# jasperlinthorst/reveal

Hardware: AMD Instinct MI355X
Metric: Mbp/s indexed+MUM-anchored (reveal rem) (higher is better)
Workload: dtype int32

## Files before the change

### include/reveal_amd.h

```cpp
#ifndef REVEAL_AMD_H
#define REVEAL_AMD_H
#include <stdint.h>

#ifdef __cplusplus
extern "C" {
#endif

typedef struct rv_index rv_index;

const char *rv_last_error(void);
int  rv_abi_version(void);
int  rv_sa_bits(void);
int  rv_device_count(void);

rv_index *rv_new(int device);
void rv_free(rv_index *h);

int rv_add_sample(rv_index *h);
int rv_add_sequence(rv_index *h, const char *seq, int64_t len, int64_t *begin, int64_t *end);
int rv_reset(rv_index *h);
int rv_reserve_text(rv_index *h, int64_t bytes);
int64_t rv_n(const rv_index *h);
int rv_nsamples(const rv_index *h);
int rv_nnodes(const rv_index *h);
// ... 42 lines not shown
    int64_t steps;
    int64_t splits;
    int64_t anchored_bp;
    int32_t levels;
    int32_t maxdepth;
    int64_t scanned_ranks;
    double  t_scan, t_host, t_split, t_bubble;
} rv_align_stats;
int rv_align_builtin(rv_index *h, int minl, int minn, rv_align_stats *st);

int rv_align_builtin_until(rv_index *h, int minl, int minn, int stop_subs, rv_align_stats *st);
int rv_align_builtin_resume(rv_index *h, rv_align_stats *st);
int rv_align_builtin_continue(rv_index *h, int stop_subs, rv_align_stats *st);
int rv_frontier_counts(rv_index *h, int64_t *out);
int rv_frontier_export(rv_index *h, int64_t *meta, int64_t *node_first, int64_t *nodes);
int64_t rv_frontier_pack(rv_index *h, const int32_t *subs, int k, void *sa, void *lcp, void *bwt, int on_device);
int rv_frontier_import(rv_index *h, int minl, int minn, uint32_t maxlcp, int level, int nsubs, const int64_t *meta,
                       const int64_t *node_first, const int64_t *nodes, int64_t m,
                       const void *sa, const void *lcp, const void *bwt, int on_device);
int64_t rv_frontier_seeds_export(rv_index *h, const int32_t *subs, int k, int64_t *out, int64_t cap);
int rv_frontier_seeds_import(rv_index *h, int nsubs, const int64_t *words, int64_t nwords);
uint32_t rv_maxlcp(const rv_index *h);
int rv_cascade_info(const rv_index *h, int64_t *out);
int rv_capacity_events(const rv_index *h, int64_t *out);
const char *rv_cascade_why(const rv_index *h);
int64_t rv_anchor_count(rv_index *h, int64_t *members);
int rv_fetch_anchors(rv_index *h, uint32_t *l, int64_t *off, int64_t *pos);
int rv_set_result_buffers(rv_index *h, uint32_t *l, int64_t l_cap, int64_t *off, int64_t off_cap, int64_t *pos, int64_t pos_cap);
typedef struct {
    int64_t  key, n;
    int32_t  depth, nsamples, nnodes, picked;
    int64_t  nmums;
    uint32_t l; int32_t mn;
    int64_t  sp_min;
    uint64_t h_sa, h_lcp, h_mums;
} rv_trace;
int rv_set_trace(rv_index *h, int on);
int rv_set_preselect(rv_index *h, int64_t maxmums);
int rv_set_option(rv_index *h, const char *name, int64_t value);
int rv_get_option(rv_index *h, const char *name, int64_t *value);
int rv_set_launch_trace(int on);
int rv_option_count(void);
const char *rv_option_name(int k);
int64_t rv_trace_count(rv_index *h);
int rv_fetch_trace(rv_index *h, rv_trace *out, int64_t cap);

typedef struct rv_subindex rv_subindex;
rv_index *rv_clone(rv_index *h);
rv_subindex *rv_sx_main(rv_index *h);
rv_subindex *rv_sx_copy(rv_subindex *x);
void rv_sx_free(rv_subindex *x);
int rv_sx_info(const rv_subindex *x, rv_sub *out);
int rv_sx_nodes(const rv_subindex *x, int64_t *begin_end);
int64_t rv_sx_array(rv_subindex *x, int which, void *out, int64_t cap);
int64_t rv_sx_scan(rv_subindex *x, int minl, int minn, int64_t *members);
int rv_sx_fetch(rv_subindex *x, uint32_t *l, int32_t *n, int64_t *off, uint16_t *so, int64_t *pos);
int rv_sx_split(rv_subindex *x, const int64_t *lead, int nlead, const int64_t *trail, int ntrail,
                const int64_t *match, int nmatch, const int64_t *rest, int nrest, rv_subindex **out);
int rv_sx_extract(rv_subindex *x, int64_t *intervals, int niv);

int64_t rv_chain(int64_t m, int k, const uint32_t *len, const int32_t *nmem, const int64_t *crd, const int64_t *left,
                 const int64_t *right, int64_t wscore, int64_t wpen, int model, int64_t *out_idx, int64_t *out_score);

typedef struct { int64_t wscore, wpen, maxmums, seedsize; int gcmodel; int trim; double pcutoff; } rv_picker_args;
typedef struct {
    int picked; uint32_t pick_l; int32_t pick_n; int pick_members; uint16_t *pick_so; int64_t *pick_pos; int64_t member_cap;
    int64_t nleft, nright, nseed_members, seed_cap, seed_member_cap;
    uint32_t *seed_l; int32_t *seed_n; int64_t *seed_off; uint16_t *seed_so; int64_t *seed_pos; int64_t *seed_score; uint8_t *seed_right;
} rv_picker_out;
int rv_set_picker(rv_index *h, int kind, const rv_picker_args *args);
int rv_picker_info(const rv_index *h, int64_t *out);
int rv_pick_chain(const rv_picker_args *args, int nsub, int64_t m, const uint32_t *l, const int32_t *n, const int64_t *off, const uint16_t *so,
                  const int64_t *pos, int nsamples, const int64_t *seq_begin, const int64_t *iv_begin, const int64_t *iv_end, int minlength,
                  rv_picker_out *out);

typedef struct rv_graph rv_graph;
rv_graph *rv_graph_import(int64_t nnodes, const int64_t *node_b, const int64_t *node_e, const int8_t *node_aligned, const int8_t *node_sent,
                          const int64_t *off_ptr, const int32_t *off_sid, const int64_t *off_val,
                          int64_t nedges, const int32_t *edge_u, const int32_t *edge_v, const int64_t *edge_ptr, const int32_t *edge_paths,
                          const int64_t *pred_ptr, const int32_t *pred_edge, int npaths, const uint8_t *star, const int64_t *id2end,
                          int nstart, const int32_t *start_nodes, int literal_segments);
int rv_graph_pick(rv_graph *g, const rv_picker_args *args, int nsub, int64_t m, const uint32_t *l, const int32_t *n, const int64_t *off, const uint16_t *so, const int64_t *pos,
                  const int64_t *left, const int64_t *right, int minlength, rv_picker_out *out);
int rv_graph_align(rv_graph *g, const int64_t *nodes, int64_t nn, const int64_t *left, const int64_t *right, uint32_t l, const int64_t *pos, int npos,
                   int64_t *counts, int64_t *out6);
int rv_graph_align_fetch(rv_graph *g, int64_t *out);
int rv_set_graph_picker(rv_index *h, rv_graph *g, const rv_picker_args *args);
rv_graph *rv_graph_new(void);
int rv_graph_add_linear(rv_graph *g, int64_t b, int64_t e, int star);
int64_t rv_graph_read_gfa(rv_graph *g, rv_index *h, int64_t *text_n, const char *data, int64_t len, const char **names);
typedef struct GfaParsed rv_gfa_parsed;
rv_gfa_parsed *rv_gfa_parse(const char *data, int64_t len);
int64_t rv_graph_adopt(rv_graph *g, rv_index *h, int64_t *text_n, rv_gfa_parsed *parsed, const char **names);
void rv_gfa_parsed_free(rv_gfa_parsed *parsed);
int rv_graph_seal(rv_graph *g);
int rv_graph_paths(const rv_graph *g, int64_t *id2end);
int rv_graph_node_kinds(const rv_graph *g, int8_t *out);
int rv_graph_literal(const rv_graph *g);
int rv_graph_finish(rv_graph *g);
rv_graph *rv_graph_replay_begin(int nseq, const int64_t *begin, const int64_t *end);
int rv_set_replay_graph(rv_index *h, rv_graph *g);
rv_graph *rv_graph_replay(int nseq, const int64_t *begin, const int64_t *end, int64_t na, const uint32_t *an_l, const int64_t *an_off, const int64_t *an_pos);
const char *rv_graph_error(const rv_graph *g);
int rv_graph_sizes(const rv_graph *g, int64_t *out);
int rv_graph_export(const rv_graph *g, int64_t *node_b, int64_t *node_e, int8_t *node_aligned, int64_t *off_ptr, int32_t *off_sid, int64_t *off_val,
                    int64_t *succ_ptr, int32_t *succ_to, int32_t *succ_edge, int64_t *pred_ptr, int32_t *pred_from, int32_t *pred_edge, int64_t *edge_ptr, int32_t *edge_paths);
int rv_graph_prune(rv_graph *g, const char *T);
int64_t rv_graph_gfa(rv_graph *g, const char *T, int npaths, const char *const *names, const char *cmdline, const char **out);
void rv_graph_free(rv_graph *g);

enum { RV_K_SCAN_PAIR = 0, RV_K_SCAN_MULTI = 1, RV_K_SA_SORT = 2, RV_K_LCP = 3, RV_K_SPLIT = 4, RV_K_LABEL = 5,
       RV_K_BUBBLE = 6,
       RV_K_RADIX_SCATTER = 7, RV_K_RADIX_HIST = 8, RV_K_TEXT_ROUND = 9,
       RV_K_CASCADE = 10,
       RV_K_DIAG_TABLE = 11,
       RV_K_INIT_KEYS = 12,
       RV_K_PUBLISH = 13,
       RV_K_COUNT = 14 };
int rv_prof_enable(rv_index *h, int on);
int rv_prof_reset(rv_index *h);
int rv_prof_get(rv_index *h, int k, int64_t *launches, double *ms, double *bytes);
typedef struct rv_batch rv_batch;
rv_batch *rv_batch_new(void);
int rv_batch_add(rv_batch *b, rv_index *h);
int rv_batch_run(rv_batch *b, int minl, int minn, int construct, rv_align_stats *stats, int *status);
int rv_batch_info(const rv_batch *b, int64_t *out);
void rv_batch_free(rv_batch *b);
typedef struct rv_many rv_many;
rv_many *rv_many_new(int device);
void rv_many_free(rv_many *m);
int rv_many_option(rv_many *m, const char *name, int64_t value);
int64_t rv_many_add(rv_many *m, const char *const *seqs, const int64_t *lens, int k);
int rv_many_clear(rv_many *m);
int rv_many_run(rv_many *m, int minl, int minn, rv_align_stats *total);
int64_t rv_many_anchor_count(rv_many *m, int64_t *first, int64_t *members);
int rv_many_fetch(rv_many *m, uint32_t *l, int64_t *off, int64_t *pos);
int64_t rv_many_text(rv_many *m, int64_t job, char *out, int64_t cap);
int rv_many_info(const rv_many *m, int64_t *out);
int64_t rv_many_arrays(rv_many *m, int64_t job, int which, void *out, int64_t cap);
void *rv_dev_alloc(int device, int64_t bytes);
int rv_dev_free(int device, void *p);
int rv_ipc_export(int device, const void *p, uint8_t handle[64]);
void *rv_ipc_open(int device, const uint8_t handle[64]);
int rv_ipc_close(int device, void *p);
int rv_dev_copy(int device, void *dst, const void *src, int64_t bytes);
int rv_measure_bandwidth(int device, int64_t bytes, int iters, double *read_gbs, double *copy_gbs);
int rv_sa_stats(rv_index *h, int *sigma, int *bits, int *k0, int *rounds, int64_t *sorted_elems, int *radix_passes);
int rv_sa_diag_table(rv_index *h);
int rv_sa_tail(rv_index *h, int64_t *out);

int rv_test_exclusive_sum_u32(const uint32_t *in, uint32_t *out, int64_t n);
int rv_test_inclusive_max_u32(const uint32_t *in, uint32_t *out, int64_t n);
int rv_test_radix_sort(uint64_t *keys, uint32_t *vals, int64_t n, int bit_lo, int bit_hi);
int rv_test_radix_time(int64_t n, int bits, int dist, int flags, int iters, double *ms, int64_t *bad);

#ifdef __cplusplus
}
#endif
#endif
```

### reveal_amd/_index.py

```python
import ctypes
import mmap
import os
import sys
import numpy as np

from . import _lib
from ._lib import RV_T, RV_SA, RV_SAI, RV_LCP, RV_SO, RV_NSEP


def _page_array(count, dtype):
    nbytes = max(int(count), 1) * np.dtype(dtype).itemsize
    m = mmap.mmap(-1, (nbytes + mmap.PAGESIZE - 1) // mmap.PAGESIZE * mmap.PAGESIZE)
    return np.frombuffer(m, dtype=dtype, count=max(int(count), 1))


def _pairs(iv, sa64):
    a = np.ascontiguousarray(np.array([(int(b), int(e)) for b, e in iv], dtype=np.int64).reshape(-1, 2))
    return a, len(a)


_OPTION_DEFAULTS = {}


def make_index_type(sa64, error):

    class index(object):

        def __init__(self, sa="", lcp="", cache=0):
            self._lib = _lib.get(sa64)
            self._dll = self._lib.dll
            self._h = None
            self._safile, self._lcpfile, self._cache = sa or "", lcp or "", int(cache)
            self._samples, self._nodes, self.skipmums = [], set(), []
            self._leftnode = self._rightnode = None
            self._depth = 0
            self._constructed = False
            self._main = self
            self._slot = None
            self._sx = None
            self._n_sub = None
            self._nsamples_sub = None
            self._h = self._dll.rv_new(_lib.device())
            if not self._h:
                raise error(self._lib.err())
            self.options_from_env()

        def set_option(self, name, value=1):
            if self._dll.rv_set_option(self._main._h, name.encode(), int(value)) != 0:
                self._fail()

        def get_option(self, name):
            v = ctypes.c_int64(0)
            if self._dll.rv_get_option(self._main._h, name.encode(), ctypes.byref(v)) != 0:
                self._fail()
            return v.value

        def options_from_env(self):
            for k in range(self._dll.rv_option_count()):
                name = self._dll.rv_option_name(k).decode()
                v = os.environ.get(name)
                if v is None:
                    d = _OPTION_DEFAULTS.get((sa64, name))
                    if d is None:
                        d = _OPTION_DEFAULTS[(sa64, name)] = self.get_option(name)
                    elif self.get_option(name) != d:
                        self.set_option(name, d)
                    continue
                try:
                    iv = int(v) if v.strip() else 1
                except ValueError:
                    iv = 1
                _OPTION_DEFAULTS.setdefault((sa64, name), self.get_option(name))
                self.set_option(name, iv)

        @property
        def _main(self):
            m = self.__dict__.get("_main_ref")
            return self if m is None else m

        @_main.setter
        def _main(self, v):
            self.__dict__["_main_ref"] = None if v is self else v

        def __del__(self):
            try:
                if getattr(self, "_sx", None):
                    self._dll.rv_sx_free(self._sx)
                    self._sx = None
                if self._h and self._main is self:
                    self._dll.rv_free(self._h)
                    self._h = None
            except Exception:
                pass

        def _fail(self, exc=None):
            raise (exc or error)(self._lib.err())

        def addsample(self, *args):
            if len(args) < 1:
                raise error("Specify name of sample as argument.")
            if not isinstance(args[0], str):
                raise error("Sample name has to be a string.")
            self._samples.append(args[0])
            self._dll.rv_add_sample(self._h)
            self._constructed = False
            return None

        def addsequence(self, seq):
            if isinstance(seq, str):
                seq = seq.encode()
            elif not isinstance(seq, (bytes, bytearray)):
                raise TypeError("argument 1 must be str or bytes")
            b, e = ctypes.c_int64(0), ctypes.c_int64(0)
            if self._dll.rv_add_sequence(self._h, bytes(seq), len(seq), ctypes.byref(b), ctypes.byref(e)) != 0:
                self._fail()
            intv = (b.value, e.value)
            self._nodes.add(intv)
            self._constructed = False
            return intv

        def reset(self, reserve=0):
            if self._main is not self or self._slot is not None:
                raise error("reset() is for a main index outside align()")
            if self._sx:
                self._dll.rv_sx_free(self._sx)
                self._sx = None
            if self._dll.rv_reset(self._h) != 0:
                self._fail()
            if reserve and self._dll.rv_reserve_text(self._h, int(reserve)) != 0:
                self._fail()
            self._samples, self._nodes, self.skipmums = [], set(), []
            self._leftnode = self._rightnode = None
            self._depth = 0
            self._constructed = False
            self._pending = False
            self._n_sub = self._nsamples_sub = None

        def upload(self):
            if self._dll.rv_upload(self._h) != 0:
                self._fail()

        def upload_again(self):
            if self._dll.rv_upload_again(self._h) != 0:
                self._fail()

        def prof(self, enable=None, reset=False, only=None):
            ids = {"scan_pair": _lib.K_SCAN_PAIR, "scan_multi": _lib.K_SCAN_MULTI, "sa_build": _lib.K_SA_SORT, "lcp": _lib.K_LCP,
                   "split": _lib.K_SPLIT, "label": _lib.K_LABEL, "bubble": _lib.K_BUBBLE, "radix_scatter": _lib.K_RADIX_SCATTER,
                   "radix_hist": _lib.K_RADIX_HIST, "text_round": _lib.K_TEXT_ROUND, "cascade": _lib.K_CASCADE, "diag_table": _lib.K_DIAG_TABLE,
                   "init_keys": _lib.K_INIT_KEYS, "publish": _lib.K_PUBLISH}
            if enable is not None:
                on = 0
                if enable:
                    on = 1 if only is None else sum(2 << ids[k] for k in only)
                self._dll.rv_prof_enable(self._h, on)
            if reset:
                self._dll.rv_prof_reset(self._h)
            out = {}
            for name, k in ids.items():
                n, ms, by = ctypes.c_int64(0), ctypes.c_double(0), ctypes.c_double(0)
                self._dll.rv_prof_get(self._h, k, ctypes.byref(n), ctypes.byref(ms), ctypes.byref(by))
                out[name] = (n.value, ms.value, by.value)
            return out

        def sa_stats(self):
            v = [ctypes.c_int(0) for _ in range(4)]
            se, rp = ctypes.c_int64(0), ctypes.c_int(0)
            self._dll.rv_sa_stats(self._h, *[ctypes.byref(x) for x in v], ctypes.byref(se), ctypes.byref(rp))
            tail = (ctypes.c_int64 * 2)()
            self._dll.rv_sa_tail(self._h, tail)
            return dict(sigma=v[0].value, bits=v[1].value, k0=v[2].value, rounds=v[3].value, sorted_elems=se.value, radix_passes=rp.value,
                        diag_table=int(self._dll.rv_sa_diag_table(self._h)), far_pairs=int(tail[0]), lcp_list=int(tail[1]))

        def construct(self, rc=0):
            if self._sx:
                self._dll.rv_sx_free(self._sx)
                self._sx = None
            r = self._dll.rv_construct(self._h, int(rc), self._safile.encode(), self._lcpfile.encode(), self._cache)
            if r != 0:
                self._fail()
            self._constructed = True
            self._rc = 1 if int(rc) == 1 else 0
            self._depth = 0
            self._main = self
            return None

        def _sx_info(self):
            info = _lib.RvSub()
            self._dll.rv_sx_info(self._sx, ctypes.byref(info))
            return info

        @property
        def n(self):
            if self._sx:
                return self._sx_info().n
            return self._n_sub if self._n_sub is not None else self._dll.rv_n(self._h)

        @property
        def depth(self):
            return self._depth

        @property
        def nsamples(self):
            if self._sx and self._depth > 0:
                return self._sx_info().nsamples
            return self._nsamples_sub if self._nsamples_sub is not None else self._dll.rv_nsamples(self._h)

        @property
        def samples(self):
            return self._main._samples

        @property
        def nodes(self):
            if self.__dict__.get("_nodes_stale"):
                self._sync_nodes()
            return self._nodes

        @property
        def leftnode(self):
            return self._leftnode

        @property
        def rightnode(self):
            return self._rightnode

        @property
        def nsep(self):
            ns = self._dll.rv_nsamples(self._h)
            out = np.zeros(max(ns - 1, 1), dtype=np.int64)
            k = self._dll.rv_get_array(self._h, RV_NSEP, out.ctypes.data, len(out))
            return [int(x) for x in out[:max(k, 0)]]

        def _array(self, which, dtype, count, exc=TypeError):
            out = np.zeros(max(count, 1), dtype=dtype)
            if self._sx and which in (RV_SA, RV_LCP):
                k = self._dll.rv_sx_array(self._sx, which, out.ctypes.data, len(out))
            elif self._slot is not None and which in (RV_SA, RV_LCP):
                k = self._dll.rv_sub_array(self._h, self._slot, which, out.ctypes.data, len(out))
            else:
                k = self._dll.rv_get_array(self._h, which, out.ctypes.data, len(out))
            if k < 0:
                raise exc(self._lib.err())
            return out[:k]

        def _main_n(self):
            return self._dll.rv_n(self._h)

        @property
        def SA(self):
            return self._array(RV_SA, self._lib.sa_t, self.n).tolist()

        @property
        def LCP(self):
            return self._array(RV_LCP, self._lib.lcp_t, self.n).tolist()

        @property
        def SAi(self):
            return self._array(RV_SAI, self._lib.sa_t, self._main_n()).tolist()

        @property
        def SO(self):
            return self._array(RV_SO, np.uint16, self._main_n()).tolist()

        @property
        def T(self):
            return self._array(RV_T, np.uint8, self._main_n(), exc=error).tobytes().decode("latin-1")

        def array(self, name):
            which = {"SA": RV_SA, "LCP": RV_LCP, "SAi": RV_SAI, "SO": RV_SO, "T": RV_T}[name]
            dt = {RV_SA: self._lib.sa_t, RV_LCP: self._lib.lcp_t, RV_SAI: self._lib.sa_t, RV_SO: np.uint16, RV_T: np.uint8}[which]
            return self._array(which, dt, self.n if which in (RV_SA, RV_LCP) else self._main_n())

        def _sx_mums(self, minl, minn):
            mem = ctypes.c_int64(0)
            cnt = self._dll.rv_sx_scan(self._sx, int(minl), int(minn), ctypes.byref(mem))
            if cnt < 0:
                self._fail()
            l = np.zeros(max(cnt, 1), dtype=np.uint32); n = np.zeros(max(cnt, 1), dtype=np.int32)
            off = np.zeros(cnt + 1, dtype=np.int64)
            so = np.zeros(max(mem.value, 1), dtype=np.uint16); pos = np.zeros(max(mem.value, 1), dtype=np.int64)
            if self._dll.rv_sx_fetch(self._sx, l.ctypes.data, n.ctypes.data, off.ctypes.data, so.ctypes.data, pos.ctypes.data) != 0:
                self._fail()
            return _csr_to_tuples(cnt, l, n, off, so, pos)

        def getmums(self, minl=0):
            if self._sx:
                if self._dll.rv_nsamples(self._h) != 2:
                    raise error("getmums on a sub-index needs a two-sample main index")
                rc = 1 if getattr(self._main, "_rc", 0) else 0
                out = [(l, (spd[0][1], spd[1][1]), rc) for l, _, spd in self._sx_mums(minl, 0)]
                if rc:
                    nsep0, nT = self.nsep[0], self._main_n()
                    out = [(l, (a, nsep0 + (nT - b - l)), rc) for l, (a, b), _ in out]
                return out
            cnt = self._dll.rv_getmums(self._h, int(minl))
            if cnt < 0:
                self._fail(TypeError if cnt == -2 else error)
            l = np.zeros(max(cnt, 1), dtype=np.uint32)
            a = np.zeros(max(cnt, 1), dtype=np.int64)
            b = np.zeros(max(cnt, 1), dtype=np.int64)
            if self._dll.rv_fetch_mums(self._h, l.ctypes.data, a.ctypes.data, b.ctypes.data, len(l)) != 0:
                self._fail()
            rc = 1 if getattr(self, "_rc", 0) else 0
            return [(int(l[k]), (int(a[k]), int(b[k])), rc) for k in range(cnt)]

        def _multi(self, minlength, minn, mems):
            if self._sx:
                if mems or self._dll.rv_nsamples(self._h) <= 2:
                    raise error("only getmultimums of an index with more than two samples is available on a sub-index")
                return self._sx_mums(minlength, minn)
            members = ctypes.c_int64(0)
            cnt = self._dll.rv_getmultimums(self._h, int(minlength), int(minn), mems, ctypes.byref(members))
            if cnt < 0:
                self._fail(TypeError if cnt == -2 else error)
            l = np.zeros(max(cnt, 1), dtype=np.uint32); n = np.zeros(max(cnt, 1), dtype=np.int32)
            off = np.zeros(cnt + 1, dtype=np.int64)
            so = np.zeros(max(members.value, 1), dtype=np.uint16); pos = np.zeros(max(members.value, 1), dtype=np.int64)
            if self._dll.rv_fetch_multi(self._h, l.ctypes.data, n.ctypes.data, off.ctypes.data, so.ctypes.data, pos.ctypes.data) != 0:
                self._fail()
            return _csr_to_tuples(cnt, l, n, off, so, pos)

        def getmultimums(self, minlength=0, minn=2):
            return self._multi(minlength, minn, 0)

        def getmultimems(self, minlength=0, minn=2):
# ... 404 lines not shown
```

### reveal_amd/_lib.py

```python
import ctypes
import importlib.util
import os
import sys
import numpy as np

_HERE = os.path.dirname(os.path.abspath(__file__))

RV_T, RV_SA, RV_SAI, RV_LCP, RV_SO, RV_NSEP, RV_NODES = range(7)
K_SCAN_PAIR, K_SCAN_MULTI, K_SA_SORT, K_LCP, K_SPLIT, K_LABEL, K_BUBBLE, K_RADIX_SCATTER, K_RADIX_HIST, K_TEXT_ROUND, K_CASCADE, K_DIAG_TABLE, K_INIT_KEYS, K_PUBLISH = range(14)

CAPACITY_EVENTS = ("pair_ovf", "pair_out", "pair_pick_ovf", "pair_second_copy", "multi_rec", "multi_mem", "multi_cand",
                   "mems_rec", "mems_mem", "mems_long")
CAP_SITES = {"multi_cand": 1, "cas_wit": 2, "cas_tables": 4, "casm_matches": 8, "casm_wit": 16, "casm_tables": 32,
             "mems_rec": 64, "mems_mem": 128, "mems_long": 256}

c_i64p = ctypes.POINTER(ctypes.c_int64)
V = ctypes.c_void_p


class RvSub(ctypes.Structure):
    _fields_ = [("n", ctypes.c_int64), ("depth", ctypes.c_int32), ("nsamples", ctypes.c_int32),
                ("nnodes", ctypes.c_int32), ("parent", ctypes.c_int32), ("kind", ctypes.c_int32),
                ("reserved", ctypes.c_int32), ("nmums", ctypes.c_int64), ("nmembers", ctypes.c_int64)]


class RvAlignStats(ctypes.Structure):
    _fields_ = [("steps", ctypes.c_int64), ("splits", ctypes.c_int64), ("anchored_bp", ctypes.c_int64),
                ("levels", ctypes.c_int32), ("maxdepth", ctypes.c_int32), ("scanned_ranks", ctypes.c_int64),
                ("t_scan", ctypes.c_double), ("t_host", ctypes.c_double), ("t_split", ctypes.c_double),
                ("t_bubble", ctypes.c_double)]


TRACE_DTYPE = np.dtype([("key", np.int64), ("n", np.int64), ("depth", np.int32), ("nsamples", np.int32),
                        ("nnodes", np.int32), ("picked", np.int32), ("nmums", np.int64), ("l", np.uint32),
                        ("mn", np.int32), ("sp_min", np.int64), ("h_sa", np.uint64), ("h_lcp", np.uint64),
                        ("h_mums", np.uint64)], align=True)

_I, _L, _D = ctypes.c_int, ctypes.c_int64, ctypes.c_double
SYMBOLS = {
    "rv_last_error": (ctypes.c_char_p, []),
    "rv_abi_version": (_I, []),
    "rv_sa_bits": (_I, []),
    "rv_device_count": (_I, []),
    "rv_new": (V, [_I]),
    "rv_free": (None, [V]),
    "rv_add_sample": (_I, [V]),
    "rv_add_sequence": (_I, [V, ctypes.c_char_p, _L, c_i64p, c_i64p]),
    "rv_reset": (_I, [V]),
    "rv_reserve_text": (_I, [V, _L]),
    "rv_n": (_L, [V]),
    "rv_nsamples": (_I, [V]),
    "rv_nnodes": (_I, [V]),
    "rv_node_list": (_I, [V, V]),
    "rv_construct": (_I, [V, _I, ctypes.c_char_p, ctypes.c_char_p, _I]),
    "rv_upload": (_I, [V]),
    "rv_upload_again": (_I, [V]),
    "rv_get_array": (_L, [V, _I, V, _L]),
    "rv_getmums": (_L, [V, _I]),
    "rv_fetch_mums": (_I, [V, V, V, V, _L]),
    "rv_getmultimums": (_L, [V, _I, _I, _I, c_i64p]),
    "rv_fetch_multi": (_I, [V, V, V, V, V, V]),
    "rv_align_begin": (_I, [V, _I, _I]),
    "rv_frontier_size": (_I, [V]),
    "rv_frontier_scan": (_I, [V]),
    "rv_sub_skip_scan": (_I, [V, _I]),
    "rv_sub_info": (_I, [V, _I, ctypes.POINTER(RvSub)]),
    "rv_sub_nodes": (_I, [V, _I, V]),
    "rv_sub_mums": (_I, [V, _I, V, V, V, V, V]),
    "rv_sub_array": (_L, [V, _I, _I, V, _L]),
    "rv_sub_split": (_I, [V, _I, ctypes.c_uint32, _I, V, V, _I, V, _I, V, _I, V, _I]),
    "rv_frontier_commit": (_I, [V, V]),
    "rv_align_end": (_I, [V]),
    "rv_align_builtin": (_I, [V, _I, _I, ctypes.POINTER(RvAlignStats)]),
    "rv_align_builtin_until": (_I, [V, _I, _I, _I, ctypes.POINTER(RvAlignStats)]),
    "rv_align_builtin_resume": (_I, [V, ctypes.POINTER(RvAlignStats)]),
    "rv_align_builtin_continue": (_I, [V, _I, ctypes.POINTER(RvAlignStats)]),
    "rv_frontier_counts": (_I, [V, V]),
    "rv_frontier_export": (_I, [V, V, V, V]),
    "rv_frontier_pack": (_L, [V, V, _I, V, V, V, _I]),
    "rv_frontier_import": (_I, [V, _I, _I, ctypes.c_uint32, _I, _I, V, V, V, _L, V, V, V, _I]),
    "rv_frontier_seeds_export": (_L, [V, V, _I, V, _L]),
    "rv_frontier_seeds_import": (_I, [V, _I, V, _L]),
    "rv_maxlcp": (ctypes.c_uint32, [V]),
    "rv_cascade_info": (ctypes.c_int, [V, V]),
    "rv_cascade_why": (ctypes.c_char_p, [V]),
    "rv_capacity_events": (_I, [V, V]),
    "rv_anchor_count": (_L, [V, c_i64p]),
    "rv_fetch_anchors": (_I, [V, V, V, V]),
    "rv_set_result_buffers": (_I, [V, V, _L, V, _L, V, _L]),
    "rv_set_trace": (_I, [V, _I]),
    "rv_set_preselect": (_I, [V, _L]),
    "rv_set_option": (_I, [V, ctypes.c_char_p, _L]),
    "rv_set_launch_trace": (_I, [_I]),
    "rv_batch_new": (V, []),
    "rv_batch_add": (_I, [V, V]),
    "rv_batch_run": (_I, [V, _I, _I, _I, V, V]),
    "rv_batch_info": (_I, [V, V]),
    "rv_batch_free": (None, [V]),
    "rv_dev_alloc": (V, [_I, _L]),
    "rv_dev_free": (_I, [_I, V]),
    "rv_ipc_export": (_I, [_I, V, V]),
    "rv_ipc_open": (V, [_I, V]),
    "rv_ipc_close": (_I, [_I, V]),
    "rv_dev_copy": (_I, [_I, V, V, _L]),
    "rv_get_option": (_I, [V, ctypes.c_char_p, c_i64p]),
    "rv_option_count": (_I, []),
    "rv_option_name": (ctypes.c_char_p, [_I]),
    "rv_trace_count": (_L, [V]),
    "rv_fetch_trace": (_I, [V, V, _L]),
    "rv_clone": (V, [V]),
    "rv_sx_main": (V, [V]),
    "rv_sx_copy": (V, [V]),
    "rv_sx_free": (None, [V]),
    "rv_sx_info": (_I, [V, ctypes.POINTER(RvSub)]),
    "rv_sx_nodes": (_I, [V, V]),
    "rv_sx_array": (_L, [V, _I, V, _L]),
    "rv_sx_scan": (_L, [V, _I, _I, c_i64p]),
    "rv_sx_fetch": (_I, [V, V, V, V, V, V]),
    "rv_sx_split": (_I, [V, V, _I, V, _I, V, _I, V, _I, V]),
    "rv_sx_extract": (_I, [V, V, _I]),
    "rv_chain": (_L, [_L, _I, V, V, V, V, V, _L, _L, _I, V, V]),
    "rv_prof_enable": (_I, [V, _I]),
    "rv_prof_reset": (_I, [V]),
    "rv_prof_get": (_I, [V, _I, c_i64p, ctypes.POINTER(_D), ctypes.POINTER(_D)]),
    "rv_measure_bandwidth": (_I, [_I, _L, _I, ctypes.POINTER(_D), ctypes.POINTER(_D)]),
    "rv_sa_stats": (_I, [V] + [ctypes.POINTER(_I)] * 4 + [c_i64p, ctypes.POINTER(_I)]),
    "rv_sa_diag_table": (_I, [V]),
    "rv_sa_tail": (_I, [V, c_i64p]),
    "rv_set_picker": (_I, [V, _I, V]),
    "rv_picker_info": (_I, [V, c_i64p]),
    "rv_pick_chain": (_I, [V, _I, _L, V, V, V, V, V, _I, V, V, V, _I, V]),
    "rv_graph_import": (V, [_L, V, V, V, V, V, V, V, _L, V, V, V, V, V, V, _I, V, V, _I, V, _I]),
    "rv_graph_pick": (_I, [V, V, _I, _L, V, V, V, V, V, V, V, _I, V]),
    "rv_graph_align": (_I, [V, V, _L, V, V, ctypes.c_uint32, V, _I, V, V]),
    "rv_graph_align_fetch": (_I, [V, V]),
    "rv_graph_finish": (_I, [V]),
    "rv_set_graph_picker": (_I, [V, V, V]),
    "rv_graph_new": (V, []),
    "rv_graph_replay_begin": (V, [_I, V, V]),
    "rv_set_replay_graph": (_I, [V, V]),
    "rv_graph_add_linear": (_I, [V, _L, _L, _I]),
    "rv_graph_read_gfa": (_L, [V, V, V, V, _L, V]),
    "rv_graph_paths": (_I, [V, V]),
    "rv_graph_seal": (_I, [V]),
    "rv_gfa_parse": (V, [V, _L]),
    "rv_graph_adopt": (_L, [V, V, V, V, V]),
    "rv_gfa_parsed_free": (None, [V]),
    "rv_add_sequences": (_I, [V, V, _L, V, _L]),
    "rv_graph_node_kinds": (_I, [V, V]),
    "rv_graph_literal": (_I, [V]),
    "rv_graph_replay": (V, [_I, V, V, _L, V, V, V]),
    "rv_graph_error": (ctypes.c_char_p, [V]),
    "rv_graph_sizes": (_I, [V, c_i64p]),
    "rv_graph_export": (_I, [V] * 15),
    "rv_graph_prune": (_I, [V, V]),
    "rv_graph_gfa": (_L, [V, V, _I, V, V, V]),
    "rv_graph_free": (None, [V]),
    "rv_many_new": (V, [_I]),
    "rv_many_free": (None, [V]),
    "rv_many_option": (_I, [V, ctypes.c_char_p, _L]),
    "rv_many_add": (_L, [V, V, V, _I]),
    "rv_many_clear": (_I, [V]),
    "rv_many_run": (_I, [V, _I, _I, ctypes.POINTER(RvAlignStats)]),
    "rv_many_anchor_count": (_L, [V, V, c_i64p]),
    "rv_many_fetch": (_I, [V, V, V, V]),
    "rv_many_text": (_L, [V, _L, V, _L]),
    "rv_many_info": (_I, [V, V]),
    "rv_many_arrays": (_L, [V, _L, _I, V, _L]),
    "rv_test_exclusive_sum_u32": (_I, [V, V, _L]),
    "rv_test_inclusive_max_u32": (_I, [V, V, _L]),
    "rv_test_radix_sort": (_I, [V, V, _L, _I, _I]),
    "rv_test_radix_time": (_I, [_L, _I, _I, _I, _I, ctypes.POINTER(_D), c_i64p]),
}


def _share_torch_runtime():
    if os.environ.get("RV_SYSTEM_HIP") or "torch" in sys.modules:
        return
    try:
        spec = importlib.util.find_spec("torch")
    except (ImportError, ValueError):
        spec = None
    if spec is None or not spec.origin:
        return
    path = os.path.join(os.path.dirname(spec.origin), "lib", "libamdhip64.so")
    if os.path.exists(path):
        ctypes.CDLL(path, mode=ctypes.RTLD_GLOBAL)


class Lib:
    def __init__(self, sa64=False):
        self.sa64 = sa64
        _share_torch_runtime()
        name = "libreveal_amd64.so" if sa64 else "libreveal_amd.so"
        self.path = os.path.join(os.environ.get("RV_LIB_DIR") or _HERE, name)
        if not os.path.exists(self.path):
            raise ImportError("%s is missing: build it with `python -c 'import __graft_entry__ as g; g.build()'` "
                              "(hipcc --offload-arch=gfx950); reveal_amd has no CPU fallback" % self.path)
        self.dll = ctypes.CDLL(self.path)
        for sym, (res, args) in SYMBOLS.items():
            fn = getattr(self.dll, sym)
            fn.restype, fn.argtypes = res, args
        self.sa_t = np.int64 if sa64 else np.int32
        self.lcp_t = np.uint32 if sa64 else np.int32
        assert self.dll.rv_sa_bits() == (64 if sa64 else 32)
        v = os.environ.get("RV_LAUNCH_TRACE")
        if v is not None and v.strip() not in ("", "0"):
            self.dll.rv_set_launch_trace(1)

    def err(self):
        return (self.dll.rv_last_error() or b"").decode(errors="replace")


_libs = {}
_device = 0


def set_device(i):
    global _device
    _device = int(i)


def device():
    return _device


def measure_bandwidth(nbytes=1 << 30, iters=10):
    lib = get(False)
    r, c = _D(0), _D(0)
    if lib.dll.rv_measure_bandwidth(device(), int(nbytes), int(iters), ctypes.byref(r), ctypes.byref(c)) != 0:
        raise RuntimeError(lib.err())
    return r.value, c.value


def set_launch_trace(on=True):
    return [bool(get(w).dll.rv_set_launch_trace(1 if on else 0)) for w in (False, True)]


def get(sa64=False):
    if sa64 not in _libs:
        _libs[sa64] = Lib(sa64)
    return _libs[sa64]
```

### reveal_amd/csrc/rv_api.hip

```cpp
#include "rv_index.h"
#include "rv_cascade.h"
#include <limits>
#include <stdarg.h>
#include <stdio.h>
#include <string.h>
#include <limits.h>
#include <algorithm>
#include <thread>

static thread_local char g_err[1024] = "";

void rv_set_error(const char *fmt, ...) {
    va_list ap;
    va_start(ap, fmt);
    vsnprintf(g_err, sizeof g_err, fmt, ap);
    va_end(ap);
}

static std::vector<rv_index *> &live_handles() { static std::vector<rv_index *> v; return v; }
std::mutex &rv_trim_mutex() { static std::mutex *m = new std::mutex(); return *m; }
bool rv_oom_trim() {
    size_t got = 0;
    bool log = false;
    int caller_dev = 0;
// ... 988 lines not shown
            h->batch = in ? b->g : nullptr; h->batch_settled = false;
            members += in ? 1 : 0;
        }
        rv_batch_group_begin(b->g, members);
        std::vector<int> rc((size_t)n, 0);
        auto work = [&](int i) {
            rv_index *h = b->hs[(size_t)i];
            int r = 0;
            if (hipSetDevice(h->device) != hipSuccess) { rv_set_error("hipSetDevice failed"); r = -1; }
            if (r == 0 && construct) r = rv_construct(h, 0, "", "", 0);
            if (r == 0) r = rv_align_builtin(h, minl, minn, stats ? &stats[i] : nullptr);
            if (h->batch && !h->batch_settled) { h->batch_settled = true; rv_batch_group_leave(h->batch); }
            if (r != 0) b->errs[(size_t)i] = rv_last_error();
            rc[(size_t)i] = r;
        };
        std::vector<std::thread> th;
        int started = n;
        for (int i = 1; i < n; i++) {
            try { th.emplace_back(work, i); }
            catch (...) { started = i; break; }
        }
        if (started < n) for (int i = started; i < n; i++) { rv_index *h = b->hs[(size_t)i]; if (h->batch) { h->batch_settled = true; rv_batch_group_leave(h->batch); h->batch = nullptr; } }
        work(0);
        for (auto &t : th) t.join();
        for (int i = started; i < n; i++) work(i);
        int bad = -1;
        for (int i = 0; i < n; i++) { b->hs[(size_t)i]->batch = nullptr; if (status) status[i] = rc[(size_t)i]; if (rc[(size_t)i] != 0 && bad < 0) bad = i; }
        if (bad >= 0) { rv_set_error("rv_batch_run: job %d: %s", bad, b->errs[(size_t)bad].c_str()); return -1; }
        return 0;
    } catch (const std::exception &e) {
        for (rv_index *h : b->hs) h->batch = nullptr;
        rv_set_error("rv_batch_run: %s", e.what());
        return -1;
    }
}

void *rv_dev_alloc(int device, int64_t bytes) {
    void *p = nullptr;
    if (bytes < 0 || hipSetDevice(device) != hipSuccess) { rv_set_error("rv_dev_alloc: bad device or size"); return nullptr; }
    const hipError_t e = hipMalloc(&p, (size_t)std::max<int64_t>(bytes, 256));
    if (e != hipSuccess) { (void)hipGetLastError(); rv_set_error("rv_dev_alloc(%lld bytes): %s", (long long)bytes, hipGetErrorString(e)); return nullptr; }
    return p;
}
int rv_dev_free(int device, void *p) {
    if (!p) return 0;
    RV_HIP(hipSetDevice(device));
    RV_HIP(hipFree(p));
    return 0;
}
int rv_ipc_export(int device, const void *p, uint8_t handle[64]) {
    static_assert(sizeof(hipIpcMemHandle_t) == 64, "hipIpcMemHandle_t is 64 bytes");
    RV_HIP(hipSetDevice(device));
    hipIpcMemHandle_t hd;
    RV_HIP(hipIpcGetMemHandle(&hd, const_cast<void *>(p)));
    memcpy(handle, &hd, 64);
    return 0;
}
void *rv_ipc_open(int device, const uint8_t handle[64]) {
    if (hipSetDevice(device) != hipSuccess) { rv_set_error("rv_ipc_open: bad device"); return nullptr; }
    hipIpcMemHandle_t hd;
    memcpy(&hd, handle, 64);
    void *p = nullptr;
    const hipError_t e = hipIpcOpenMemHandle(&p, hd, hipIpcMemLazyEnablePeerAccess);
    if (e != hipSuccess) { (void)hipGetLastError(); rv_set_error("rv_ipc_open: %s", hipGetErrorString(e)); return nullptr; }
    return p;
}
int rv_ipc_close(int device, void *p) {
    if (!p) return 0;
    RV_HIP(hipSetDevice(device));
    RV_HIP(hipIpcCloseMemHandle(p));
    return 0;
}
int rv_dev_copy(int device, void *dst, const void *src, int64_t bytes) {
    if (bytes <= 0) return 0;
    RV_HIP(hipSetDevice(device));
    RV_HIP(hipMemcpy(dst, src, (size_t)bytes, hipMemcpyDefault));
    RV_HIP(hipStreamSynchronize(nullptr));
    return 0;
}

int rv_measure_bandwidth(int device, int64_t bytes, int iters, double *read_gbs, double *copy_gbs) {
    if (bytes < (1 << 20) || iters < 1) { rv_set_error("rv_measure_bandwidth: bytes >= 1 MiB and iters >= 1 needed"); return -1; }
    RV_HIP(hipSetDevice(device));
    const int64_t n16 = bytes / 16;
    void *a = nullptr, *b = nullptr; unsigned *sink = nullptr;
    hipStream_t q = nullptr; hipEvent_t e0 = nullptr, e1 = nullptr;
    RV_HIP(hipMalloc(&a, (size_t)n16 * 16)); RV_HIP(hipMalloc(&b, (size_t)n16 * 16)); RV_HIP(hipMalloc((void **)&sink, 64));
    RV_HIP(hipStreamCreateWithFlags(&q, hipStreamNonBlocking));
    RV_HIP(hipEventCreate(&e0)); RV_HIP(hipEventCreate(&e1));
    RV_HIP(hipMemsetAsync(a, 1, (size_t)n16 * 16, q)); RV_HIP(hipMemsetAsync(b, 2, (size_t)n16 * 16, q));
    const unsigned grid = 256 * 16;
    double out[2] = {0, 0};
    for (int pass = 0; pass < 2; pass++) {
        for (int r = -1; r < iters; r++) {
            if (r == 0) RV_HIP(hipEventRecord(e0, q));
            if (pass == 0) hipLaunchKernelGGL(k_bw_read, dim3(grid), dim3(256), 0, q, (const bw_v4 *)a, n16, sink);
            else hipLaunchKernelGGL(k_bw_copy, dim3(grid), dim3(256), 0, q, (const bw_v4 *)a, (bw_v4 *)b, n16);
        }
        RV_HIP(hipEventRecord(e1, q));
        RV_HIP(hipEventSynchronize(e1));
        float ms = 0.f;
        RV_HIP(hipEventElapsedTime(&ms, e0, e1));
        out[pass] = (double)n16 * 16 * (pass ? 2 : 1) * iters / ((double)ms * 1e6);
    }
    if (read_gbs) *read_gbs = out[0];
    if (copy_gbs) *copy_gbs = out[1];
    (void)hipEventDestroy(e0); (void)hipEventDestroy(e1); (void)hipStreamDestroy(q);
    (void)hipFree(a); (void)hipFree(b); (void)hipFree(sink);
    return 0;
}

static int test_ws(Workspace &ws) {
    if (rv_device_count() <= 0) { rv_set_error("no HIP device"); return -1; }
    RV_HIP(hipSetDevice(0));
    RV_HIP(hipStreamCreateWithFlags(&ws.stream, hipStreamNonBlocking));
    return 0;
}
static void test_ws_done(Workspace &ws) { ws.release(); (void)hipStreamDestroy(ws.stream); }

static int test_scan(const uint32_t *in, uint32_t *out, int64_t n, bool maxscan) {
    Workspace ws;
    RV_TRY(test_ws(ws));
    DBuf a, b;
    int r = 0;
    if (a.reserve((size_t)n * 4 + 64) || b.reserve((size_t)n * 4 + 64)) r = -1;
    if (!r && hipMemcpy(a.p, in, (size_t)n * 4, hipMemcpyHostToDevice) != hipSuccess) r = -1;
    if (!r) r = maxscan ? rv_inclusive_max_u32(ws, a.as<u32>(), b.as<u32>(), n) : rv_exclusive_sum_u32(ws, a.as<u32>(), b.as<u32>(), n);
    if (!r && hipStreamSynchronize(ws.stream) != hipSuccess) { rv_set_error("sync failed: %s", hipGetErrorString(hipGetLastError())); r = -1; }
    if (!r && hipMemcpy(out, b.p, (size_t)n * 4, hipMemcpyDeviceToHost) != hipSuccess) r = -1;
    a.release(); b.release();
    test_ws_done(ws);
    return r;
}
int rv_test_exclusive_sum_u32(const uint32_t *in, uint32_t *out, int64_t n) { return test_scan(in, out, n, false); }
int rv_test_inclusive_max_u32(const uint32_t *in, uint32_t *out, int64_t n) { return test_scan(in, out, n, true); }

int rv_test_radix_sort(uint64_t *keys, uint32_t *vals, int64_t n, int bit_lo, int bit_hi) {
    Workspace ws;
    RV_TRY(test_ws(ws));
    DBuf k0, k1, v0, v1;
    int r = 0, in1 = 0;
    if (k0.reserve((size_t)n * 8 + 64) || k1.reserve((size_t)n * 8 + 64) || v0.reserve((size_t)n * 4 + 64) || v1.reserve((size_t)n * 4 + 64)) r = -1;
    if (!r && hipMemcpy(k0.p, keys, (size_t)n * 8, hipMemcpyHostToDevice) != hipSuccess) r = -1;
    if (!r && hipMemcpy(v0.p, vals, (size_t)n * 4, hipMemcpyHostToDevice) != hipSuccess) r = -1;
    if (!r) r = rv_radix_sort_pairs<u32>(ws, k0.as<u64>(), v0.as<u32>(), k1.as<u64>(), v1.as<u32>(), n, bit_lo, bit_hi, &in1);
    if (!r && hipStreamSynchronize(ws.stream) != hipSuccess) { rv_set_error("sync failed: %s", hipGetErrorString(hipGetLastError())); r = -1; }
    if (!r && hipMemcpy(keys, in1 ? k1.p : k0.p, (size_t)n * 8, hipMemcpyDeviceToHost) != hipSuccess) r = -1;
    if (!r && hipMemcpy(vals, in1 ? v1.p : v0.p, (size_t)n * 4, hipMemcpyDeviceToHost) != hipSuccess) r = -1;
    k0.release(); k1.release(); v0.release(); v1.release();
    test_ws_done(ws);
    return r;
}

}
namespace {
__device__ inline u64 rt_mix(u64 x) { x ^= x >> 33; x *= 0xff51afd7ed558ccdull; x ^= x >> 33; x *= 0xc4ceb9fe1a85ec53ull; x ^= x >> 33; return x; }
__global__ __launch_bounds__(256) void k_rt_fill(u64 *keys, u32 *vals, int64_t n, int bits, int dist) {
    const int64_t i = (int64_t)blockIdx.x * 256 + threadIdx.x;
    if (i >= n) return;
    u64 r = rt_mix((u64)i * 0x9E3779B97F4A7C15ull + 12345);
    u64 k = 0;
    if (dist == 0) k = r;
    else if (dist == 1) { u64 r2 = rt_mix(r); for (int j = 0; j < 17; j++) { k = k * 5 + 1 + (r2 & 3); r2 >>= 2; } }
    const u64 mask = bits >= 64 ? ~0ull : (1ull << bits) - 1;
    keys[i] = (k & mask) | (r & ~mask & 0x00ffffffffffffffull);
    vals[i] = (u32)i;
}
__global__ __launch_bounds__(256) void k_rt_check(const u64 *keys, const u32 *vals, int64_t n, int bits, unsigned long long *bad) {
    const int64_t i = (int64_t)blockIdx.x * 256 + threadIdx.x;
    if (i + 1 >= n) return;
    const u64 mask = bits >= 64 ? ~0ull : (1ull << bits) - 1;
    const u64 a = keys[i] & mask, b = keys[i + 1] & mask;
    if (a > b || (a == b && vals[i] > vals[i + 1])) atomicAdd(bad, 1ull);
}
}
extern "C" {
int rv_test_radix_time(int64_t n, int bits, int dist, int flags, int iters, double *ms, int64_t *bad) {
    Workspace ws;
    RV_TRY(test_ws(ws));
    ws.opt.rs_bits = (flags & 1) ? 10 : 8; ws.opt.rs_xcd = (flags & 2) ? 1 : 0; ws.opt.rs_cnt16 = (flags & 4) ? 1 : 0; ws.opt.rs_no_digit_bytes = (flags & 8) ? 1 : 0;
    DBuf k0, k1, v0, v1, db;
    int r = 0, in1 = 0;
    hipEvent_t e0 = nullptr, e1 = nullptr;
    if (k0.reserve((size_t)n * 8 + 64) || k1.reserve((size_t)n * 8 + 64) || v0.reserve((size_t)n * 4 + 64) || v1.reserve((size_t)n * 4 + 64) || db.reserve(64)) r = -1;
    if (!r && (hipEventCreate(&e0) != hipSuccess || hipEventCreate(&e1) != hipSuccess)) r = -1;
    for (int it = 0; !r && it < iters; it++) {
        hipLaunchKernelGGL(k_rt_fill, dim3((unsigned)ceil_div(n, 256)), dim3(256), 0, ws.stream, k0.as<u64>(), v0.as<u32>(), n, bits, dist);
        (void)hipEventRecord(e0, ws.stream);
        r = rv_radix_sort_pairs<u32>(ws, k0.as<u64>(), v0.as<u32>(), k1.as<u64>(), v1.as<u32>(), n, 0, bits, &in1);
        (void)hipEventRecord(e1, ws.stream);
        if (!r && hipEventSynchronize(e1) != hipSuccess) { rv_set_error("sync failed: %s", hipGetErrorString(hipGetLastError())); r = -1; }
        float t = 0;
        if (!r) { (void)hipEventElapsedTime(&t, e0, e1); ms[it] = t; }
    }
    if (!r) {
        (void)hipMemsetAsync(db.p, 0, 8, ws.stream);
        hipLaunchKernelGGL(k_rt_check, dim3((unsigned)ceil_div(n, 256)), dim3(256), 0, ws.stream, (const u64 *)(in1 ? k1.p : k0.p), (const u32 *)(in1 ? v1.p : v0.p), n, bits,
                           db.as<unsigned long long>());
        unsigned long long b = 0;
        if (hipMemcpyAsync(&b, db.p, 8, hipMemcpyDeviceToHost, ws.stream) != hipSuccess || hipStreamSynchronize(ws.stream) != hipSuccess) r = -1;
        *bad = (int64_t)b;
    }
    if (e0) (void)hipEventDestroy(e0);
    if (e1) (void)hipEventDestroy(e1);
    k0.release(); k1.release(); v0.release(); v1.release(); db.release();
    test_ws_done(ws);
    return r;
}

}
```

### reveal_amd/csrc/rv_common.h

```cpp
#pragma once
#include <algorithm>
#include <mutex>
#include <thread>
#include <vector>
#include <utility>
#include <hip/hip_runtime.h>
#include <stdint.h>
#include <string.h>
#include <stddef.h>
#include <vector>
#include <string>

#ifdef RV_SA64
typedef int64_t  sa_t;
typedef uint32_t lcp_t;
#else
typedef int32_t  sa_t;
typedef int32_t  lcp_t;
#endif

typedef unsigned long long u64;
typedef unsigned int       u32;

void rv_set_error(const char *fmt, ...);

#define RV_HIP(x)                                                                              \
    do {                                                                                       \
        hipError_t e_ = (x);                                                                   \
        if (e_ != hipSuccess) {                                                                \
            rv_set_error("%s:%d %s: %s", __FILE__, __LINE__, #x, hipGetErrorString(e_));       \
            return -1;                                                                         \
        }                                                                                      \
    } while (0)
#define RV_TRY(x)                                                                              \
    do {                                                                                       \
        int r_ = (x);                                                                          \
        if (r_ != 0) return r_;                                                                \
    } while (0)
#define RV_OPTION_LIST(X) \
    X(bubble_par_min, "RV_BUBBLE_PAR_MIN", -1) \
    X(presel_log, "RV_PRESEL_LOG", 0) \
    X(presel_host, "RV_PRESEL_HOST", 0) \
    X(leaf_acap, "RV_LEAF_ACAP", 256) \
    X(bubble_lds_always, "RV_BUBBLE_LDS_ALWAYS", 0) \
    X(no_early_bubble, "RV_NO_EARLY_BUBBLE", 0) \
    X(early_bubble_many, "RV_EARLY_BUBBLE_MANY", 0) \
    X(no_early_split, "RV_NO_EARLY_SPLIT", 0) \
    X(keep_dead, "RV_KEEP_DEAD", 0) \
    X(bubble_no_lds, "RV_BUBBLE_NO_LDS", 0) \
    X(bubble_no_join, "RV_BUBBLE_NO_JOIN", 0) \
    X(bubble_no_merge, "RV_BUBBLE_NO_MERGE", 0) \
    X(tables_memcpy, "RV_TABLES_MEMCPY", 0) \
    X(bubble_parent_scratch, "RV_BUBBLE_PARENT_SCRATCH", 0) \
    X(level_log, "RV_LEVEL_LOG", 0) \
    X(pb_two_pass, "RV_PB_TWO_PASS", 0) \
    X(no_leaf, "RV_NO_LEAF", 0) \
    X(leaf_prof, "RV_LEAF_PROF", 0) \
    X(no_cascade, "RV_NO_CASCADE", 0) \
    X(cascade_second, "RV_CASCADE_SECOND", 0) \
    X(cascade_danger, "RV_CASCADE_DANGER", 1) \
    X(cascade_second_off, "RV_CASCADE_SECOND_OFF", 0) \
    X(sync_block, "RV_SYNC_BLOCK", 0) \
    X(pb_refresh_tmin, "RV_PB_REFRESH_TMIN", 0) \
    X(cascade_log, "RV_CASCADE_LOG", 0) \
    X(cascade_danger_min, "RV_CASCADE_DANGER_MIN", 0) \
    X(cascade_batch, "RV_CASCADE_BATCH", 8) \
    X(lcp_by_rank, "RV_LCP_BY_RANK", 0) \
    X(no_tiny_sa, "RV_NO_TINY_SA", 0) \
    X(no_short_alphabet, "RV_NO_SHORT_ALPHABET", 0) \
    X(no_fused_lcp, "RV_NO_FUSED_LCP", 0) \
    X(no_diag, "RV_NO_DIAG", 0) \
    X(no_packed_text, "RV_NO_PACKED_TEXT", 0) \
    X(no_heads_fusion, "RV_NO_HEADS_FUSION", 0) \
    X(no_twin_collapse, "RV_NO_TWIN_COLLAPSE", 0) \
    X(no_far_twins, "RV_NO_FAR_TWINS", 0) \
    X(no_lcp_list, "RV_NO_LCP_LIST", 0) \
    X(no_text_jump, "RV_NO_TEXT_JUMP", 0) \
    X(far_table, "RV_FAR_TABLE", 0) \
    X(no_slow_class, "RV_NO_SLOW_CLASS", 0) \
    X(no_dwalk_blocks, "RV_NO_DWALK_BLOCKS", 0) \
    X(no_pub_twins, "RV_NO_PUB_TWINS", 0) \
    X(sa_no_text, "RV_SA_NO_TEXT", 0) \
    X(text_mode, "RV_TEXT_MODE", -1) \
    X(carry_ch, "RV_CARRY_CH", -1) \
    X(rs_bits, "RV_RS_BITS", 8) \
    X(rs_xcd, "RV_RS_XCD", 1) \
    X(rs_cnt16, "RV_RS_CNT16", 1) \
    X(rs_no_digit_bytes, "RV_RS_NO_DIGIT_BYTES", 0) \
    X(diag_table, "RV_DIAG_TABLE", -1) \
    X(no_cascade_chain, "RV_NO_CASCADE_CHAIN", 0) \
    X(casm_rank_count, "RV_CASM_RANK_COUNT", 0) \
    X(casm_big_min, "RV_CASM_BIG_MIN", -1) \
    X(casm_no_big, "RV_CASM_NO_BIG", 0) \
    X(casm_big_root, "RV_CASM_BIG_ROOT", 1 << 22) \
    X(casm_big_total, "RV_CASM_BIG_TOTAL", 1 << 26) \
    X(lock_any, "RV_LOCK_ANY", 0) \
    X(presel_dev_min, "RV_PRESEL_DEV_MIN", 65536) \
    X(scan_v1, "RV_SCAN_V1", 0) \
    X(pick_threads, "RV_PICK_THREADS", 0) \
    X(cascade_prio, "RV_CASCADE_PRIO", 0) \
    X(cas_witness_pass, "RV_CAS_WITNESS_PASS", 0) \
    X(cap_limit, "RV_CAP_LIMIT", 0) \
    X(cap_sites, "RV_CAP_SITES", -1)
struct RvOptions {
#define RV_X_(f, name, def) int64_t f = def;
    RV_OPTION_LIST(RV_X_)
#undef RV_X_
    int64_t *find(const char *name) {
#define RV_X_(f, nm, def) if (strcmp(name, nm) == 0) return &f;
        RV_OPTION_LIST(RV_X_)
#undef RV_X_
        return nullptr;
    }
};
extern int g_rv_launch_trace;
static inline bool rv_launch_trace_on() { return g_rv_launch_trace != 0; }
#define RV_LAUNCH_CHECK()                                                                      \
    do {                                                                                       \
        RV_HIP(hipGetLastError());                                                             \
        if (rv_launch_trace_on()) {                                                            \
            fprintf(stderr, "launch %s:%d\n", __FILE__, __LINE__);                             \
            fflush(stderr);                                                                    \
            RV_HIP(hipDeviceSynchronize());                                                    \
        }                                                                                      \
    } while (0)

static inline int64_t ceil_div(int64_t a, int64_t b) { return (a + b - 1) / b; }

#define RV_BWT_SIDE 0x80u
#define RV_BWT_CHAR 0x7fu

#ifdef __HIPCC__
__device__ inline u32 rv_wave_min_u32(u32 v) {
    const int inf = -1;
    int x = (int)v, y;
#define RV_DPP_MIN(ctrl, rmask)                                                        \
    y = __builtin_amdgcn_update_dpp(inf, x, ctrl, rmask, 0xf, false);                  \
    x = (int)(((u32)y < (u32)x) ? (u32)y : (u32)x);
    RV_DPP_MIN(0xB1, 0xf)
    RV_DPP_MIN(0x4E, 0xf)
    RV_DPP_MIN(0x141, 0xf)
    RV_DPP_MIN(0x140, 0xf)
    RV_DPP_MIN(0x142, 0xa)
    RV_DPP_MIN(0x143, 0xc)
#undef RV_DPP_MIN
    return (u32)__builtin_amdgcn_readlane(x, 63);
}
#endif

#ifdef __HIPCC__
template <int CTRL, int ROWMASK> __device__ inline u32 rv_dpp_u32(u32 x) { return (u32)__builtin_amdgcn_update_dpp(0, (int)x, CTRL, ROWMASK, 0xf, false); }
#define RV_WAVE_SCAN_STEPS(STEP)                                                     \
    STEP(0x111, 0xf, (lane & 15) >= 1)                                               \
    STEP(0x112, 0xf, (lane & 15) >= 2)                                               \
    STEP(0x114, 0xf, (lane & 15) >= 4)                                               \
    STEP(0x118, 0xf, (lane & 15) >= 8)                                               \
    STEP(0x142, 0xa, (lane & 31) >= 16)                                              \
    STEP(0x143, 0xc, lane >= 32)
__device__ inline u64 rv_wave_max_u64(u64 v) {
#define RV_STEP_(CTRL, RM, TAKE) { const u64 t = ((u64)rv_dpp_u32<CTRL, RM>((u32)(v >> 32)) << 32) | rv_dpp_u32<CTRL, RM>((u32)v); v = t > v ? t : v; }
    RV_WAVE_SCAN_STEPS(RV_STEP_)
#undef RV_STEP_
    return ((u64)(u32)__builtin_amdgcn_readlane((int)(u32)(v >> 32), 63) << 32) | (u32)__builtin_amdgcn_readlane((int)(u32)v, 63);
}
__device__ inline u64 rv_wave_seg_max_u64(u32 seg, u64 v) {
    const int lane = threadIdx.x & 63;
    u32 lo = (u32)v, hi = (u32)(v >> 32);
#define RV_STEP_(CTRL, RM, TAKE) { const u32 os = rv_dpp_u32<CTRL, RM>(seg), ol = rv_dpp_u32<CTRL, RM>(lo), oh = rv_dpp_u32<CTRL, RM>(hi); \
                                   const bool up = (TAKE) && os == seg && (oh > hi || (oh == hi && ol > lo)); lo = up ? ol : lo; hi = up ? oh : hi; }
    RV_WAVE_SCAN_STEPS(RV_STEP_)
#undef RV_STEP_
    return ((u64)hi << 32) | lo;
}
__device__ inline u32 rv_wave_seg_max_u32(u32 seg, u32 v) {
    const int lane = threadIdx.x & 63;
#define RV_STEP_(CTRL, RM, TAKE) { const u32 os = rv_dpp_u32<CTRL, RM>(seg), ov = rv_dpp_u32<CTRL, RM>(v); v = ((TAKE) && os == seg && ov > v) ? ov : v; }
    RV_WAVE_SCAN_STEPS(RV_STEP_)
#undef RV_STEP_
    return v;
}
__device__ inline u32 rv_wave_incl_sum_u32(u32 v) {
    const int lane = threadIdx.x & 63;
#define RV_STEP_(CTRL, RM, TAKE) { const u32 t = rv_dpp_u32<CTRL, RM>(v); v += (TAKE) ? t : 0u; }
    RV_WAVE_SCAN_STEPS(RV_STEP_)
#undef RV_STEP_
    return v;
}
#endif

bool rv_oom_trim();

inline hipError_t rv_event_wait(hipEvent_t ev) {
    hipError_t e;
    for (int spins = 0; (e = hipEventQuery(ev)) == hipErrorNotReady; spins++) {
        if (spins < 64) { __builtin_ia32_pause(); continue; }
        if (spins < 640) { std::this_thread::yield(); continue; }
        return hipEventSynchronize(ev);
    }
    return e;
}

struct DBuf {
    void  *p = nullptr;
    size_t cap = 0;
    int reserve(size_t bytes) {
        if (bytes <= cap) return 0;
        if (p) { (void)hipFree(p); p = nullptr; cap = 0; }
        size_t want = bytes + (bytes >= ((size_t)256 << 20) ? bytes / 64 : bytes / 8) + 256;
        hipError_t e = hipMalloc(&p, want);
        if (e == hipErrorOutOfMemory) {
            (void)hipGetLastError();
            if (rv_oom_trim()) e = hipMalloc(&p, want);
            if (e == hipErrorOutOfMemory) { (void)hipGetLastError(); want = bytes + 256; e = hipMalloc(&p, want); }
        }
        if (e != hipSuccess) { p = nullptr; rv_set_error("%s:%d hipMalloc(%zu bytes): %s", __FILE__, __LINE__, want, hipGetErrorString(e)); return -1; }
        cap = want;
        return 0;
    }
    void release() { if (p) (void)hipFree(p); p = nullptr; cap = 0; }
    template <class T> T *as() const { return (T *)p; }
};

struct RvPools {
    std::mutex mu;
    std::vector<std::pair<int, hipStream_t>> streams;
    struct Pin { int dev; void *p; size_t cap; };
    std::vector<Pin> pinned;
    size_t pinned_bytes = 0;
};
inline RvPools &rv_pools() { static RvPools *p = new RvPools(); return *p; }
inline hipError_t rv_stream_get(hipStream_t *s) {
    int dev = 0; (void)hipGetDevice(&dev);
    {
        RvPools &P = rv_pools();
        std::lock_guard<std::mutex> g(P.mu);
        for (size_t k = P.streams.size(); k-- > 0;)
            if (P.streams[k].first == dev) { *s = P.streams[k].second; P.streams.erase(P.streams.begin() + (ptrdiff_t)k); return hipSuccess; }
    }
    return hipStreamCreateWithFlags(s, hipStreamNonBlocking);
}
inline void rv_stream_put(hipStream_t s) {
    if (!s) return;
    (void)hipStreamSynchronize(s);
    int dev = 0; (void)hipGetDevice(&dev);
    RvPools &P = rv_pools();
    {
        std::lock_guard<std::mutex> g(P.mu);
        if (P.streams.size() < 64) { P.streams.push_back({dev, s}); return; }
    }
    (void)hipStreamDestroy(s);
}
inline hipError_t rv_pinned_get(size_t bytes, void **p, size_t *cap) {
    int dev = 0; (void)hipGetDevice(&dev);
    {
        RvPools &P = rv_pools();
        std::lock_guard<std::mutex> g(P.mu);
        size_t best = (size_t)-1;
        for (size_t k = 0; k < P.pinned.size(); k++)
            if (P.pinned[k].dev == dev && P.pinned[k].cap >= bytes && P.pinned[k].cap <= 4 * bytes + (1u << 20) && (best == (size_t)-1 || P.pinned[k].cap < P.pinned[best].cap)) best = k;
        if (best != (size_t)-1) { *p = P.pinned[best].p; *cap = P.pinned[best].cap; P.pinned_bytes -= *cap; P.pinned.erase(P.pinned.begin() + (ptrdiff_t)best); return hipSuccess; }
    }
    const hipError_t e = hipHostMalloc(p, bytes, hipHostMallocDefault);
    if (e == hipSuccess) *cap = bytes;
    return e;
}
inline void rv_pinned_put(void *p, size_t cap) {
    if (!p) return;
    int dev = 0; (void)hipGetDevice(&dev);
    RvPools &P = rv_pools();
    {
        std::lock_guard<std::mutex> g(P.mu);
        if (cap <= ((size_t)64 << 20) && P.pinned_bytes + cap <= ((size_t)512 << 20) && P.pinned.size() < 256) { P.pinned.push_back({dev, p, cap}); P.pinned_bytes += cap; return; }
    }
    (void)hipHostFree(p);
}

struct HBuf {
    void  *p = nullptr;
    size_t cap = 0;
    int reserve(size_t bytes) {
        if (bytes <= cap) return 0;
        if (p) { (void)hipDeviceSynchronize(); rv_pinned_put(p, cap); p = nullptr; cap = 0; }
        size_t want = bytes + bytes / 2 + 4096;
        RV_HIP(rv_pinned_get(want, &p, &cap));
        return 0;
    }
    void release() { if (p) rv_pinned_put(p, cap); p = nullptr; cap = 0; }
    template <class T> T *as() const { return (T *)p; }
};

enum RvCapEvent { RV_CE_PAIR_OVF = 0, RV_CE_PAIR_OUT, RV_CE_PAIR_PICK_OVF, RV_CE_PAIR_SECOND_COPY, RV_CE_MULTI_REC, RV_CE_MULTI_MEM, RV_CE_MULTI_CAND,
                  RV_CE_MEMS_REC, RV_CE_MEMS_MEM, RV_CE_MEMS_LONG, RV_CE_COUNT };
enum RvCapSite { RV_CS_MULTI_CAND = 1, RV_CS_CAS_WIT = 2, RV_CS_CAS_TABLES = 4, RV_CS_CASM_MATCHES = 8, RV_CS_CASM_WIT = 16, RV_CS_CASM_TABLES = 32,
                 RV_CS_MEMS_REC = 64, RV_CS_MEMS_MEM = 128, RV_CS_MEMS_LONG = 256 };
struct Workspace {
    hipStream_t stream = nullptr;
    RvOptions opt;
    int64_t cap_events[RV_CE_COUNT] = {0};
    u32 pair_ovf_cap = 0, multi_cand_cap = 0;
    template <class T> T cap_first(int site, T cap, T least = 1) const {
        if (opt.cap_limit <= 0 || !(opt.cap_sites & (int64_t)site)) return cap;
        const T lim = (T)std::max<int64_t>(opt.cap_limit, (int64_t)least);
        return cap < lim ? cap : lim;
    }
    DBuf scan_tmp[4];
    DBuf rs_hist;
    DBuf rs_digits;
    DBuf misc[20];
    DBuf sa[32];
    HBuf hpin;
    hipEvent_t ev_rb = nullptr;
    void *prof_ctx = nullptr;
    int (*prof_begin_fn)(void *, hipStream_t, int, double) = nullptr;
    void (*prof_end_fn)(void *, hipStream_t, int) = nullptr;
    int prof_begin(int k, double bytes) { return prof_begin_fn ? prof_begin_fn(prof_ctx, stream, k, bytes) : -1; }
    void prof_end(int id) { if (prof_end_fn && id >= 0) prof_end_fn(prof_ctx, stream, id); }
    bool sa_in_use = false;
    size_t trim_sa() {
        size_t got = 0;
        for (auto &b : sa) { got += b.cap; b.release(); }
        return got;
    }
    void release() {
        hpin.release();
        if (ev_rb) { (void)hipEventDestroy(ev_rb); ev_rb = nullptr; }
        for (auto &b : scan_tmp) b.release();
        rs_hist.release(); rs_digits.release();
        for (auto &b : misc) b.release();
        for (auto &b : sa) b.release();
    }
};

std::mutex &rv_trim_mutex();
struct SaScratchInUse {
    Workspace &w; bool was;
    SaScratchInUse(Workspace &x) : w(x) { std::lock_guard<std::mutex> g(rv_trim_mutex()); was = w.sa_in_use; w.sa_in_use = true; }
    ~SaScratchInUse() { std::lock_guard<std::mutex> g(rv_trim_mutex()); w.sa_in_use = was; }
};

int rv_exclusive_sum_u32(Workspace &ws, const u32 *in, u32 *out, int64_t n);
int rv_exclusive_sum_u64(Workspace &ws, const u64 *in, u64 *out, int64_t n);
int rv_inclusive_max_u32(Workspace &ws, const u32 *in, u32 *out, int64_t n);
int rv_inclusive_max_u64(Workspace &ws, const u64 *in, u64 *out, int64_t n);

int rv_radix_passes(const Workspace &ws, int nbits);
template <class V>
int rv_radix_sort_pairs(Workspace &ws, u64 *k0, V *v0, u64 *k1, V *v1, int64_t n,
                        int bit_lo, int bit_hi, int *result_in_1, bool first_digits = false);
uint8_t *rv_radix_first_digits(Workspace &ws, int64_t n, int bit_lo, int bit_hi);

int rv_read_back(Workspace &ws, void *dst, const void *dsrc, size_t bytes);
int rv_read_back2(Workspace &ws, void *dst_a, const void *dsrc_a, size_t bytes_a, void *dst_b, const void *dsrc_b, size_t bytes_b);

int rv_h2d_copy(Workspace &ws, const void *pinned_src, void *dst, size_t bytes);

struct RvSaStats {
    int    sigma, bits, k0;
    int    rounds;
    int64_t sorted_elems;
    int    radix_passes;
    int    diag_table;
    int64_t far_pairs;
    int64_t lcp_list;
};
int rv_build_sa(Workspace &ws, const uint8_t *T, int64_t n, sa_t *SA, RvSaStats *st,
                lcp_t *LCP = nullptr, uint8_t *BWT = nullptr, sa_t side_sep = 0, u32 *d_maxlcp = nullptr, bool *fused_done = nullptr,
                const int64_t *seps = nullptr, int nseps = 0);
int rv_build_inverse(Workspace &ws, const sa_t *SA, sa_t *SAi, int64_t n);
int rv_build_inverse_checked(Workspace &ws, const sa_t *SA, sa_t *SAi, int64_t n);
int rv_build_lcp(Workspace &ws, const uint8_t *T, const sa_t *SA, bool by_rank, lcp_t *LCP, int64_t n, u32 *d_maxlcp, uint8_t *BWT, sa_t side_sep);
int rv_build_bwt(Workspace &ws, const uint8_t *T, const sa_t *SA, int64_t n, uint8_t *BWT, sa_t side_sep);
```

### reveal_amd/csrc/rv_construct.hip

```cpp
#include "rv_common.h"
#include <string.h>
#include <stdlib.h>
#include <algorithm>
#include <limits>

#ifdef RV_SA64
typedef u64 sav_t;
#else
typedef u32 sav_t;
#endif

namespace {

constexpr int TB = 256;

__device__ inline u64 swar_eq(u64 v, uint8_t c) {
    const u64 t = v ^ (0x0101010101010101ull * c);
    return ~(((t & 0x7f7f7f7f7f7f7f7full) + 0x7f7f7f7f7f7f7f7full) | t) & 0x8080808080808080ull;
}
__device__ inline u64 swar_acgt(u64 v) { return swar_eq(v, 'A') | swar_eq(v, 'C') | swar_eq(v, 'G') | swar_eq(v, 'T'); }
__device__ inline u32 swar_code2(u64 v) {
    u64 y = ((v >> 1) ^ (v >> 2)) & 0x0303030303030303ull;
    y = (y | (y >> 6)) & 0x000f000f000f000full;
    y = (y | (y >> 12)) & 0x000000ff000000ffull;
// ... 182 lines not shown
        const int64_t z0 = ys < dt.S2 ? ys + dt.D + (int64_t)dd : ys - dt.D - (int64_t)dd;
        const bool other_side = ys < dt.S2 ? z0 >= dt.S2 : z0 + DT_TILE - 1 < dt.S2 - 1;
        if (dd == DT_NONE) { ms = me = 0xffffu; prev = DT_NONE; }
        else if (one_side && ys + DT_TILE <= n && z0 >= 0 && z0 + DT_TILE <= n && other_side) {
            const int off = (int)(z0 & (DT_TILE - 1));
            const bool v0 = dt.dtab[z0 >> DT_SHIFT] == dd, v1 = off ? dt.dtab[(z0 >> DT_SHIFT) + 1] == dd : v0;
            const u32 lowm = off ? ((1u << (DT_TILE - off)) - 1u) : 0xffffu;
            const u32 valid = (v0 ? lowm : 0u) | (v1 ? (~lowm & 0xffffu) : 0u);
            u64 a[2], b[2];
            __builtin_memcpy(a, T + ys, 16);
            __builtin_memcpy(b, T + z0, 16);
#pragma unroll
            for (int k = 0; k < 2; k++)
#pragma unroll
                for (int j = 0; j < 8; j++) {
                    const u32 ca = (u32)(a[k] >> (8 * j)) & 0xffu, cb = (u32)(b[k] >> (8 * j)) & 0xffu;
                    const bool ea = !((ca == 'A') | (ca == 'C') | (ca == 'G') | (ca == 'T')), eb = !((cb == 'A') | (cb == 'C') | (cb == 'G') | (cb == 'T'));
                    const int bit = 8 * k + j;
                    me |= (u32)(ea | eb) << bit; ms |= (u32)((ca != cb) | ea | eb) << bit; ml |= (u32)(ca < cb) << bit;
                }
            u32 forced = 0;
            if ((valid & 1u) && prev != dd) forced |= 1u;
            if (off && !v0 && v1) forced |= 1u << (DT_TILE - off);
            ms |= (~valid & 0xffffu) | forced; me |= (~valid & 0xffffu) | forced; ml &= valid & ~forced;
            prev = (valid >> (DT_TILE - 1)) & 1u ? dd : DT_NONE;
        } else {
            for (int bit = 0; bit < DT_TILE; bit++) {
                const int64_t y = ys + bit;
                int64_t z = 0;
                const int32_t l = dtab_link(dt, y, n, &z);
                if (l == DT_NONE || l != prev) { me |= 1u << bit; ms |= 1u << bit; prev = l; continue; }
                const u32 ca = T[y], cb = T[z];
                const bool ea = !((ca == 'A') | (ca == 'C') | (ca == 'G') | (ca == 'T')), eb = !((cb == 'A') | (cb == 'C') | (cb == 'G') | (cb == 'T'));
                me |= (u32)(ea | eb) << bit; ms |= (u32)((ca != cb) | ea | eb) << bit; ml |= (u32)((ca < cb) & !(ea | eb)) << bit;
            }
        }
        ws |= (u64)ms << (sub * DT_TILE); we |= (u64)me << (sub * DT_TILE); wl |= (u64)ml << (sub * DT_TILE);
    }
    stop[w] = ws; exc[w] = we; lt[w] = wl;
}
constexpr sav_t TW_FLAG = (sav_t)1 << (sizeof(sav_t) * 8 - 1);
__device__ inline u64 tw_window_clear(u64 prev, u64 lo, u64 hi, int K) {
    u64 a = lo, b = hi;
    int m = 1;
    while (2 * m <= K) { a |= (a >> m) | (b << (64 - m)); b |= b >> m; m *= 2; }
    if (m < K) { const int d = K - m; a |= (a >> d) | (b << (64 - d)); }
    return ~(a | (lo << 1) | (prev >> 63));
}
__device__ inline u64 tw_range(int64_t w, int64_t a, int64_t b) {
    const int64_t lo = a - 64 * w, hi = b - 64 * w;
    if (hi <= 0 || lo >= 64) return 0ull;
    const u64 from = lo <= 0 ? ~0ull : (~0ull << lo), to = hi >= 64 ? ~0ull : ((1ull << hi) - 1ull);
    return from & to;
}
__device__ inline u64 tw_mask(u64 prev, u64 lo, u64 hi, int64_t w, int K, int64_t D, int64_t n, int tab) {
    const int64_t e = 2 * D - 1 < n ? 2 * D - 1 : n;
    return tw_window_clear(prev, lo, hi, K) & (tab ? (tw_range(w, 0, D - 1) | tw_range(w, D, n)) : (tw_range(w, 1, D - 1) | tw_range(w, D + 1, e)));
}
__global__ __launch_bounds__(TB) void k_tw_count(const u64 *__restrict__ stop, int64_t nwords, int K, int64_t D, int64_t n, u32 *__restrict__ tilecnt, int64_t ntiles, int tab) {
    const int64_t w = (int64_t)blockIdx.x * TB + threadIdx.x;
    u32 c = 0;
    if (w < nwords) {
        const u64 prev = w > 0 ? stop[w - 1] : ~0ull, lo = stop[w], hi = w + 1 < nwords ? stop[w + 1] : ~0ull;
        c = (u32)__popcll(tw_range(w, D, n) & ~tw_mask(prev, lo, hi, w, K, D, n, tab));
    }
#pragma unroll
    for (int d = 8; d >= 1; d >>= 1) c += __shfl_down(c, d, 16);
    const int64_t tile = w >> 4;
    if ((threadIdx.x & 15) == 0 && tile < ntiles) tilecnt[tile] = c;
    if (w == 0) tilecnt[ntiles] = 0;
}
struct KeyLayout { int at_shift, at_bits, nd_shift, nd_bits; u64 sortmask; };
struct KeyPack { int g, fb, nf, gl, fbl, bits; u32 rad, fmask, lmask, lscale , fdiv ;
                 u32 lastmul , dmul[4]; };
constexpr int KP_MAXG = 5;
constexpr u32 KP_MAXFIELD = 4096;
__device__ inline u32 key_common_digits(u64 x, u64 y, const KeyPack &kp) {
    const u64 d = x ^ y;
    if (d == 0ull) return (u32)((kp.nf - 1) * kp.g + kp.gl);
    const int top = 63 - __builtin_clzll(d);
    const bool last = top < kp.fbl;
    const u32 f = last ? (u32)(kp.nf - 1) : ((u32)(kp.bits - 1 - top) * kp.fdiv) >> 16;
    const int sh = last ? 0 : kp.bits - (int)(f + 1u) * kp.fb;
    const u32 fm = last ? kp.lmask : kp.fmask, sc = last ? kp.lscale : 1u;
    const u32 a = __umul24((u32)(x >> sh) & fm, sc), b = __umul24((u32)(y >> sh) & fm, sc);
    u32 c = f * (u32)kp.g;
#pragma unroll
    for (int i = 1; i < KP_MAXG; i++)
        if (i < kp.g) c += ((a * kp.dmul[i - 1]) >> 20) == ((b * kp.dmul[i - 1]) >> 20) ? 1u : 0u;
    return c;
}
constexpr int ND_WORDS = 40;
constexpr int IK_AHEAD = 96;
constexpr int IK_WORDS = (KEY_TILE + IK_AHEAD) / 4;
constexpr int IK_FPOS = KEY_TILE + 64;
__device__ inline u32 ik_first_stop(const u32 *s_sc, int k, int K, u32 at_none) {
    const int w = k >> 5, sh = k & 31;
    if (K <= 32) {
        const u32 win = __funnelshift_r(s_sc[w], s_sc[w + 1], (u32)sh) & (K >= 32 ? ~0u : (1u << K) - 1u);
        return win ? (u32)__builtin_ctz(win) : at_none;
    }
    u64 win = (((u64)s_sc[w + 1] << 32) | s_sc[w]) >> sh;
    if (sh) win |= (u64)s_sc[w + 2] << (64 - sh);
    win &= K >= 64 ? ~0ull : (1ull << K) - 1ull;
    return win ? (u32)__builtin_ctzll(win) : at_none;
}
template <int G, int N> __device__ inline void ik_fields(const volatile uint16_t *s_tf, int p, const KeyPack &kp, u32 (&lo)[N], u32 (&hi)[N]) {
#pragma unroll
    for (int r = 0; r < N; r++) lo[r] = hi[r] = 0u;
    int sh = kp.bits;
    for (int f = 0; f + 1 < kp.nf; f++, p += G) {
        sh -= kp.fb;
        u32 v[N];
#pragma unroll
        for (int r = 0; r < N; r++) v[r] = s_tf[p + r];
        if (sh >= 32) {
#pragma unroll
            for (int r = 0; r < N; r++) hi[r] |= v[r] << (sh - 32);
        } else {
#pragma unroll
            for (int r = 0; r < N; r++) lo[r] |= v[r] << sh;
            if (sh + kp.fb > 32) {
#pragma unroll
                for (int r = 0; r < N; r++) hi[r] |= v[r] >> (32 - sh);
            }
        }
    }
#pragma unroll
    for (int r = 0; r < N; r++) lo[r] |= ((u32)s_tf[p + r] * kp.lastmul) >> 20;
}
struct IkFetch { u32 raw0, raw1, pb; u64 ds, de, dl; };
__device__ inline u32 ik_text_word(const uint8_t *__restrict__ T, int64_t n, int64_t i, bool whole) {
    if (whole) return *reinterpret_cast<const u32 *>(T + i);
    u32 raw = 0;
    for (int r = 0; r < 4; r++) if (i + r < n) raw |= (u32)T[i + r] << (8 * r);
    return raw;
}
__device__ inline void ik_fetch(IkFetch &f, const uint8_t *__restrict__ T, int64_t n, const DiagBits &dg, bool hint, int64_t tile, bool aligned) {
    const int64_t base = tile * KEY_TILE;
    const bool whole = aligned && base + KEY_TILE + IK_AHEAD <= n;
    f.raw0 = ik_text_word(T, n, base + 4 * (int64_t)threadIdx.x, whole);
    f.raw1 = (int)threadIdx.x < IK_WORDS - TB ? ik_text_word(T, n, base + 4 * (int64_t)(TB + threadIdx.x), whole) : 0u;
    f.pb = (threadIdx.x == 0 && base > 0) ? (u32)T[base - 1] : (u32)'$';
    f.ds = ~0ull; f.de = ~0ull; f.dl = 0ull;
    if (hint && (int)threadIdx.x <= ND_WORDS) {
        const int64_t w = base / 64 - 1 + threadIdx.x, nwords = (n + 63) / 64;
        if (w >= 0 && w < nwords) { f.ds = dg.stop[w]; if (threadIdx.x) { f.de = dg.exc[w]; f.dl = dg.lt[w]; } }
    }
}
template <int G>
__global__ __launch_bounds__(TB) void k_init_keys(const uint8_t *__restrict__ T, int64_t n, const uint8_t *__restrict__ lut, int K, KeyPack kp,
                                                  u64 *__restrict__ keys, sav_t *__restrict__ vals, int pay, u32 stop0, u32 stop1,
                                                  KeyLayout ly, DiagBits dg, const u32 *__restrict__ tw_off , int64_t ntiles,
                                                  uint8_t *__restrict__ dig0 ) {
    __shared__ u32 code32[IK_WORDS + 2];
    __shared__ u32 s_sc[IK_WORDS / 8 + 3];
    __shared__ uint8_t slut[256], sstop[256];
    __shared__ __align__(8) uint16_t s_tf[IK_FPOS];
    __shared__ u64 s_stop0[ND_WORDS + 1], s_exc[ND_WORDS], s_lt[ND_WORDS];
    __shared__ u64 s_tw[KEY_TILE / 64], s_keep[KEY_TILE / 64];
    __shared__ u32 s_kpre[KEY_TILE / 64 + 1];
    __shared__ uint16_t s_list[KEY_TILE];
    __shared__ u32 s_nm[64];
    __shared__ u32 s_raw32[KEY_TILE / 4 + 1];
    u64 *const s_stop = s_stop0 + 1;
    uint8_t *const s_raw = reinterpret_cast<uint8_t *>(s_raw32);
    const bool hint = ly.nd_bits > 0;
    const bool aligned = (reinterpret_cast<uintptr_t>(T) & 3u) == 0;
    auto tile_of = [&](int64_t x) { return x; };
    IkFetch fx;
    int64_t x = blockIdx.x;
    if (x < ntiles) ik_fetch(fx, T, n, dg, hint, tile_of(x), aligned);
    {
        const u32 c = lut[threadIdx.x];
        slut[threadIdx.x] = (uint8_t)c;
        sstop[threadIdx.x] = ((c == stop0) | (c == stop1) | (c == 0u)) ? 1 : 0;
        if (threadIdx.x < 2) code32[IK_WORDS + threadIdx.x] = 0u;
        if (threadIdx.x < 3) s_sc[IK_WORDS / 8 + threadIdx.x] = ~0u;
    }
    __syncthreads();
    const u32 at_none = (1u << ly.at_bits) - 1u;
    const int nd_none = hint ? (int)((1u << ly.nd_bits) - 1u) : 0;
    for (; x < ntiles; x += gridDim.x) {
    const int64_t tile = tile_of(x);
    const int64_t base = tile * KEY_TILE;
#pragma unroll
    for (int turn = 0; turn < 2; turn++) {
        const int wq = (int)threadIdx.x + turn * TB;
        if (wq >= IK_WORDS) break;
        const u32 raw = turn ? fx.raw1 : fx.raw0;
        u32 c4 = 0, sb = 0;
#pragma unroll
        for (int r = 0; r < 4; r++) {
            const u32 b = (raw >> (8 * r)) & 0xffu;
            c4 |= (u32)slut[b] << (8 * r);
            sb |= (u32)sstop[b] << r;
        }
        code32[wq] = c4;
        if (turn == 0) s_raw32[1 + wq] = raw;
        int v = (int)(sb << (4 * (wq & 7)));
        v |= __builtin_amdgcn_update_dpp(0, v, 0xB1, 0xf, 0xf, false);
        v |= __builtin_amdgcn_update_dpp(0, v, 0x4E, 0xf, 0xf, false);
        v |= __builtin_amdgcn_update_dpp(0, v, 0x141, 0xf, 0xf, false);
        if ((wq & 7) == 0) s_sc[wq >> 3] = (u32)v;
    }
    if (threadIdx.x == 0) s_raw[3] = (uint8_t)fx.pb;
    if (hint && (int)threadIdx.x <= ND_WORDS) {
        s_stop0[threadIdx.x] = fx.ds;
        if (threadIdx.x) { s_exc[threadIdx.x - 1] = fx.de; s_lt[threadIdx.x - 1] = fx.dl; }
    }
    if (x + gridDim.x < ntiles) ik_fetch(fx, T, n, dg, hint, tile_of(x + gridDim.x), aligned);
    __syncthreads();
    for (int wq = threadIdx.x; wq < IK_FPOS / 4; wq += TB) {
        const u64 cw = ((u64)code32[wq + 1] << 32) | code32[wq];
        u32 f4[4];
#pragma unroll
        for (int j = 0; j < 4; j++) {
            u32 h = 0;
#pragma unroll
            for (int e = 0; e < G; e++) h = __umul24(h, kp.rad) + ((u32)(cw >> (8 * (j + e))) & 0xffu);
            f4[j] = h;
        }
        *reinterpret_cast<uint2 *>(s_tf + 4 * wq) = make_uint2(f4[0] | (f4[1] << 16), f4[2] | (f4[3] << 16));
    }
    if (hint && (threadIdx.x >> 6) == 1) {
        const int w = (int)threadIdx.x - 64;
        u32 v = ~0u;
        if (w < ND_WORDS && s_stop[w] != 0ull) {
            const int b = __builtin_ctzll(s_stop[w]);
            v = ((u32)(64 * w + b) << 2) | ((u32)((s_lt[w] >> b) & 1ull) << 1) | (u32)((s_exc[w] >> b) & 1ull);
        }
#pragma unroll
        for (int d = 1; d < 64; d <<= 1) { const u32 o = __shfl_down(v, d, 64); if (w + d < 64 && o < v) v = o; }
        s_nm[w] = v;
    }
    if (tw_off && threadIdx.x < KEY_TILE / 64) {
        const int xw = threadIdx.x;
        const int64_t w = base / 64 + xw;
        const u64 t = tw_mask(s_stop0[xw], s_stop[xw], s_stop[xw + 1], w, K, dg.D, n, dg.tab);
        const u64 keep = tw_range(w, dg.D, n) & ~t;
        s_tw[xw] = t; s_keep[xw] = keep;
        const u32 c = (u32)__popcll(keep);
        u32 inc = c;
#pragma unroll
        for (int d = 1; d < KEY_TILE / 64; d <<= 1) { const u32 up = __shfl_up(inc, d, KEY_TILE / 64); if (xw >= d) inc += up; }
        s_kpre[xw] = inc - c;
        if (xw == KEY_TILE / 64 - 1) s_kpre[KEY_TILE / 64] = inc;
    }
    __syncthreads();
    if (tw_off && base >= dg.D) {
        {
            const int t = (int)threadIdx.x, xw = t >> 4, b = (t & 15) * 4;
            const u64 kw = s_keep[xw];
            u32 nib = (u32)(kw >> b) & 15u;
            if (nib) {
                u32 at = s_kpre[xw] + (u32)__popcll(kw & ((1ull << b) - 1ull));
                while (nib) { s_list[at++] = (uint16_t)(4 * t + __builtin_ctz(nib)); nib &= nib - 1u; }
            }
        }
        __syncthreads();
        const u32 total = s_kpre[KEY_TILE / 64];
        const int64_t obase = dg.D + (int64_t)tw_off[tile];
        for (u32 j = threadIdx.x; j < total; j += TB) {
            const int k = (int)s_list[j];
            const int64_t i = base + k;
            u32 lo[1], hi[1];
            ik_fields<G, 1>(s_tf, k, kp, lo, hi);
            u64 key = ((u64)hi[0] << 32) | lo[0];
            if (pay) key |= ((u64)s_raw[k + 3] << 56) | ((u64)ik_first_stop(s_sc, k, K, at_none) << ly.at_shift);
            if (hint) {
                const int wi = k >> 6, sft = k & 63;
                const u64 A = s_stop[wi] >> sft;
                const u32 nx = s_nm[wi + 1];
                const bool has = A != 0ull;
                const int d = has ? __builtin_ctzll(A) : (int)(nx >> 2) - k;
                const int at = (sft + d) & 63;
                const u32 f = has ? ((u32)((s_lt[wi] >> at) & 1ull) << 1) | (u32)((s_exc[wi] >> at) & 1ull) : nx & 3u;
                const bool known = (d < nd_none) & !(f & 1u);
                key |= (u64)(known ? (u32)d | ((f >> 1) << ly.nd_bits) : (u32)nd_none) << ly.nd_shift;
            }
            keys[obase + j] = key; vals[obase + j] = (sav_t)i;
            if (dig0) dig0[obase + j] = (uint8_t)key;
        }
    } else {
    constexpr int PER = KEY_TILE / TB;
    static_assert(PER == 4, "four bytes in front of four positions");
    const int k0 = (int)threadIdx.x * PER;
    const int64_t i0 = base + k0;
    u64 okey[PER];
    {
        u32 lo[PER], hi[PER];
        ik_fields<G, PER>(s_tf, k0, kp, lo, hi);
#pragma unroll
        for (int r = 0; r < PER; r++) okey[r] = ((u64)hi[r] << 32) | lo[r];
    }
    if (pay) {
        const u32 prevb = (u32)s_raw[k0 + 3] | (s_raw32[threadIdx.x + 1] << 8);
        const bool clear = K <= 29 && (__funnelshift_r(s_sc[k0 >> 5], s_sc[(k0 >> 5) + 1], (u32)(k0 & 31)) & ((1u << (K + 3)) - 1u)) == 0u;
#pragma unroll
        for (int r = 0; r < PER; r++)
            okey[r] |= ((u64)((prevb >> (8 * r)) & 0xffu) << 56) | ((u64)(clear ? at_none : ik_first_stop(s_sc, k0 + r, K, at_none)) << ly.at_shift);
    }
    if (hint) {
        const int wi = k0 >> 6, sft = k0 & 63;
        const u64 A = s_stop[wi] >> sft, E = s_exc[wi] >> sft, Lt = s_lt[wi] >> sft;
        const u32 nx = s_nm[wi + 1];
        const u64 Ah = A >> 3;
        const bool hh = Ah != 0ull;
        const int dh = hh ? 3 + __builtin_ctzll(Ah) : (int)(nx >> 2) - k0;
        const u32 fh = hh ? ((u32)((Lt >> (dh & 63)) & 1ull) << 1) | (u32)((E >> (dh & 63)) & 1ull) : nx & 3u;
        const u32 a3 = (u32)A & 7u, e3 = (u32)E & 7u, l3 = (u32)Lt & 7u;
#pragma unroll
        for (int r = 0; r < PER; r++) {
            const u32 t = a3 >> r;
            const int m = t ? r + __builtin_ctz(t) : dh;
            const u32 f = t ? (((l3 >> m) & 1u) << 1) | ((e3 >> m) & 1u) : fh;
            const int nd = m - r;
            const bool known = (nd < nd_none) & !(f & 1u);
            okey[r] |= (u64)(known ? (u32)nd | ((f >> 1) << ly.nd_bits) : (u32)nd_none) << ly.nd_shift;
        }
    }
    if (!tw_off || i0 + PER <= dg.D) {
        const u32 twn = tw_off ? (u32)(s_tw[k0 >> 6] >> (k0 & 63)) & 15u : 0u;
        sav_t oval[PER];
#pragma unroll
        for (int r = 0; r < PER; r++) oval[r] = (sav_t)(i0 + r) | (((twn >> r) & 1u) ? TW_FLAG : (sav_t)0);
        if (i0 + PER <= n) {
            ulonglong2 *kd2 = reinterpret_cast<ulonglong2 *>(keys + i0);
            kd2[0] = make_ulonglong2(okey[0], okey[1]); kd2[1] = make_ulonglong2(okey[2], okey[3]);
            if constexpr (sizeof(sav_t) == 4) *reinterpret_cast<uint4 *>(vals + i0) = make_uint4((u32)oval[0], (u32)oval[1], (u32)oval[2], (u32)oval[3]);
            else {
                ulonglong2 *vd2 = reinterpret_cast<ulonglong2 *>(vals + i0);
                vd2[0] = make_ulonglong2((u64)oval[0], (u64)oval[1]); vd2[1] = make_ulonglong2((u64)oval[2], (u64)oval[3]);
            }
            if (dig0) *reinterpret_cast<u32 *>(dig0 + i0) = ((u32)okey[0] & 0xffu) | (((u32)okey[1] & 0xffu) << 8) | (((u32)okey[2] & 0xffu) << 16) | ((u32)okey[3] << 24);
        } else {
#pragma unroll
            for (int r = 0; r < PER; r++) if (i0 + r < n) { keys[i0 + r] = okey[r]; vals[i0 + r] = oval[r]; if (dig0) dig0[i0 + r] = (uint8_t)okey[r]; }
        }
    } else {
#pragma unroll
        for (int r = 0; r < PER; r++) {
            const int k = k0 + r;
            const int64_t i = base + k;
            if (i >= n) continue;
            const int xw = k >> 6, b = k & 63;
            const bool twin = (s_tw[xw] >> b) & 1ull;
            if (i < dg.D) { keys[i] = okey[r]; vals[i] = (sav_t)i | (twin ? TW_FLAG : (sav_t)0); if (dig0) dig0[i] = (uint8_t)okey[r]; }
            else if (!twin) {
                const int64_t o = dg.D + (int64_t)tw_off[tile] + s_kpre[xw] + (u32)__popcll(s_keep[xw] & ((b == 0) ? 0ull : (~0ull >> (64 - b))));
                keys[o] = okey[r]; vals[o] = (sav_t)i;
                if (dig0) dig0[o] = (uint8_t)okey[r];
            }
        }
    }
    }
    __syncthreads();
    }
}

constexpr int HINT_K = 16;
struct KeyDigits { int K; u32 stop0, stop1; KeyPack kp; KeyLayout ly; int64_t D; int ns; int64_t sep[HINT_K - 1], Ds[HINT_K];
                   const int32_t *dtab; };
__device__ inline u32 key_first_stop(u64 key, const KeyDigits &kd) {
    const u32 none = (1u << kd.ly.at_bits) - 1u;
    const u32 at = (u32)(key >> kd.ly.at_shift) & none;
    return at == none ? 0xFFFFFFFFu : at;
}
__device__ inline bool key_hint(u64 key, const KeyDigits &kd, u32 *nd, bool *lt) {
    const u32 none = (1u << kd.ly.nd_bits) - 1u;
    const u32 v = (u32)(key >> kd.ly.nd_shift) & none;
    *nd = v; *lt = (key >> (kd.ly.nd_shift + kd.ly.nd_bits)) & 1ull;
    return kd.ly.nd_bits > 0 && v != none;
}
__device__ inline int hint_sample(const KeyDigits &kd, int64_t p) {
    int s = 0;
    for (int q = 0; q < kd.ns - 1; q++) s += kd.sep[q] < p ? 1 : 0;
    return s;
}
__device__ inline bool hint_cmp(const KeyDigits &kd, int64_t u, u64 key_u, int64_t v, u64 key_v, int *c, u32 *l, bool linked = false) {
    if (kd.ly.nd_bits <= 0) return false;
    const int su = hint_sample(kd, u), sv = hint_sample(kd, v);
    if (su >= HINT_K || sv >= HINT_K) return false;
    if (kd.dtab) {
        if (su == sv) return false;
        if (!linked) {
            const int64_t a = su == 0 ? u : v, b = su == 0 ? v : u;
            const int32_t dd = kd.dtab[b >> DT_SHIFT];
            if (dd == DT_NONE || b - kd.D - (int64_t)dd != a) return false;
        }
    } else {
    const int64_t bu = u - (su ? kd.Ds[su] : 0), bv = v - (sv ? kd.Ds[sv] : 0);
    if (bu != bv || su == sv) return false;
    }
    u32 au = 0, av = 0; bool ltu = false, ltv = false;
    const bool ku = su ? key_hint(key_u, kd, &au, &ltu) : false, kv = sv ? key_hint(key_v, kd, &av, &ltv) : false;
    if (su == 0) { if (!kv) return false; *c = ltv ? 1 : -1; *l = av; return true; }
    if (sv == 0) { if (!ku) return false; *c = ltu ? -1 : 1; *l = au; return true; }
    if (!ku || !kv) return false;
    if (ltu != ltv) { *c = ltu ? -1 : 1; *l = au < av ? au : av; return true; }
    if (au == av) return false;
    *l = au < av ? au : av;
    *c = ((au < av) == ltu) ? -1 : 1;
    return true;
}

__device__ inline bool hint_cmp2(const KeyDigits &kd, int64_t u, u64 key_u, int64_t v, u64 key_v, int *c, u32 *l) {
    const bool su = u > kd.sep[0], sv = v > kd.sep[0];
    if (su == sv) return false;
    const int64_t a = su ? v : u, b = su ? u : v;
    if (kd.dtab) {
        const int32_t dd = kd.dtab[b >> DT_SHIFT];
        if (dd == DT_NONE || b - kd.D - (int64_t)dd != a) return false;
    } else if (b - kd.D != a) return false;
    u32 nd = 0; bool lt = false;
    if (!key_hint(su ? key_u : key_v, kd, &nd, &lt)) return false;
    *c = (lt == su) ? -1 : 1; *l = nd;
    return true;
}

__global__ __launch_bounds__(TB) void k_heads(const u64 *__restrict__ keys, int64_t n, uint8_t *__restrict__ head, u32 *__restrict__ seed,
                                              lcp_t *__restrict__ LCP, KeyDigits kd, u32 *__restrict__ d_maxlcp) {
    const int64_t j = (int64_t)blockIdx.x * TB + threadIdx.x;
    const u64 mask = LCP ? kd.ly.sortmask : ~0ull;
    const bool in = j < n;
    const u64 kb = in ? keys[j] & mask : 0ull, ka = (in && j > 0) ? keys[j - 1] & mask : 0ull;
    const bool hd = in && ((j == 0) || ka != kb);
    if (in) { head[j] = hd; seed[j] = hd ? (u32)j : 0u; }
    u32 l = 0;
    if (LCP && hd) {
        if (j > 0) {
            const u64 dm = kd.ly.sortmask;
            l = key_common_digits(ka & dm, kb & dm, kd.kp);
            const u32 st = key_first_stop(keys[j], kd);
            l = l < st ? l : st;
        }
        LCP[j] = (lcp_t)l;
    }
    if (LCP && d_maxlcp) {
        const u32 wm = (u32)rv_wave_max_u64((u64)l);
        if ((threadIdx.x & 63) == 0 && wm > *reinterpret_cast<volatile u32 *>(d_maxlcp)) atomicMax(d_maxlcp, wm);
    }
}

__global__ __launch_bounds__(TB) void k_publish0(const sav_t *__restrict__ vals, int64_t n, sa_t *__restrict__ SA,
                                                 const u64 *__restrict__ keys, uint8_t *__restrict__ BWT, sa_t side_sep,
                                                 KeyDigits kd, lcp_t *__restrict__ LCP, uint8_t *__restrict__ head, u32 *__restrict__ d_maxlcp, u32 *__restrict__ grp) {
    const int64_t j = (int64_t)blockIdx.x * TB + threadIdx.x;
    u32 lmax = 0;
    __shared__ u64 s_key[TB + 4];
    __shared__ sav_t s_val[TB + 2];
    const bool hint = BWT && kd.ly.nd_bits > 0;
    if (hint) {
        const int64_t j0 = (int64_t)blockIdx.x * TB;
        for (int k = threadIdx.x; k < TB + 4; k += TB) { const int64_t i = j0 - 2 + k; s_key[k] = (i >= 0 && i < n) ? keys[i] : 0ull; }
        for (int k = threadIdx.x; k < TB + 2; k += TB) { const int64_t i = j0 - 1 + k; s_val[k] = (i >= 0 && i < n) ? vals[i] : (sav_t)0; }
        __syncthreads();
    }
    if (j < n) {
        const int t = threadIdx.x;
        const sav_t s = hint ? s_val[t + 1] : vals[j];
        int64_t rank = j;
        const u64 key = hint ? s_key[t + 2] : (BWT ? keys[j] : 0ull);
        if (hint) {
            const u64 mk = kd.ly.sortmask;
            const u64 k0 = key & mk;
            const u64 km2 = j >= 2 ? s_key[t] & mk : ~k0, km1 = j >= 1 ? s_key[t + 1] & mk : ~k0;
            const u64 kp1r = j + 1 < n ? s_key[t + 3] : ~key, kp2 = j + 2 < n ? s_key[t + 4] & mk : ~k0;
            const u64 km1r = j >= 1 ? s_key[t + 1] : ~key;
            const u64 kp1 = j + 1 < n ? kp1r & mk : ~k0;
            const bool first = (km1 != k0) & (kp1 == k0) & (kp2 != k0);
            const bool second = (km1 == k0) & (kp1 != k0) & (km2 != k0);
            if (first | second) {
                const sav_t ps = first ? s_val[t + 2] : s_val[t];
                const u64 pkey = first ? kp1r : km1r;
                int c; u32 nd;
                if (hint_cmp(kd, (int64_t)s, key, (int64_t)ps, pkey, &c, &nd)) {
                    const bool i_smaller = c < 0;
                    const int64_t base = first ? j : j - 1;
                    rank = base + (i_smaller ? 0 : 1);
                    if (rank != base) {
                        const u32 st = key_first_stop(key, kd);
                        const u32 l = nd < st ? nd : st;
                        LCP[rank] = (lcp_t)l;
                        lmax = l;
                        grp[rank] = (u32)rank;
                    }
                    if (second) head[j] = 1;
                }
            }
        }
        SA[rank] = (sa_t)s;
        if (BWT) BWT[rank] = (uint8_t)((u32)(key >> 56) | ((sa_t)s > side_sep ? RV_BWT_SIDE : 0u));
    }
    if (BWT && kd.ly.nd_bits > 0) {
        const u32 wm = (u32)rv_wave_max_u64((u64)lmax);
        if ((threadIdx.x & 63) == 0 && wm > __atomic_load_n(d_maxlcp, __ATOMIC_RELAXED)) atomicMax(d_maxlcp, wm);
    }
}
constexpr int HP_ITEMS = 4;
__global__ __launch_bounds__(TB) void k_heads_publish(const u64 *__restrict__ keys, const sav_t *__restrict__ vals, int64_t n, uint8_t *__restrict__ head,
                                                      u32 *__restrict__ seed, lcp_t *__restrict__ LCP, sa_t *__restrict__ SA, uint8_t *__restrict__ BWT, sa_t side_sep,
                                                      KeyDigits kd, u32 *__restrict__ d_maxlcp, int twins) {
    __shared__ u64 s_key[HP_ITEMS * TB + 4];
    __shared__ sav_t s_val[HP_ITEMS * TB + 2];
// ... 1477 lines not shown
    if (sigma >= 255) radix = 256;
    if (sigma >= 255) for (int c = 0; c < 256; c++) lut[c] = (uint8_t)c;
    const bool short_alphabet = sigma >= 2 && sigma < 255 && T != nullptr && hist[(uint8_t)'$'] > 0 && lut[(uint8_t)'$'] == 1 && hist[256] == 0 && !ws.opt.no_short_alphabet;
    bool ends_with_sep = false;
    if (short_alphabet) ends_with_sep = hist[257] == (u32)(uint8_t)'$';
    if (short_alphabet && ends_with_sep) {
        for (int c = 0; c < 256; c++) lut[c] = hist[c] ? (uint8_t)(lut[c] - 1) : (uint8_t)0;
        radix = (u32)sigma;
    }
    int K = 1;
    int bits = 0;
    KeyPack kp;
    {
        const double base = sigma > 2 ? (double)(sigma - 1) : 2.0;
        const double want = (double)n * ((seps && nseps > 1) ? 16.0 : 1.0);
        int best_g = 0, best_K = 0, best_bits = 0;
        u64 rg = 1;
        for (int g = 1; g <= KP_MAXG; g++) {
            rg *= radix;
            if (rg > KP_MAXFIELD && g > 1) break;
            const int fb = bitlen(rg - 1);
            auto bits_of = [&](int k) { u64 rl = 1; for (int e = 0; e < k % g; e++) rl *= radix; return (k / g) * fb + (k % g ? bitlen(rl - 1) : 0); };
            bool exact = true;
            for (int i = 1; i < g && exact; i++) {
                u64 d = 1; for (int e = 0; e < g - i; e++) d *= radix;
                const u32 m = (u32)(((1ull << 20) + d - 1) / d);
                for (u64 f = 0; f < rg && exact; f++) exact = ((f * m) >> 20) == f / d && f * m < (1ull << 32);
            }
            if (!exact) continue;
            int k = 1; double cap = base;
            while (cap < want && bits_of(k + 1) <= 62) { cap *= base; k++; }
            const int passes = rv_radix_passes(ws, bits_of(k));
            while (bits_of(k + 1) <= 62 && rv_radix_passes(ws, bits_of(k + 1)) == passes) k++;
            const int b = bits_of(k);
            if (k > best_K || (k == best_K && b < best_bits)) { best_g = g; best_K = k; best_bits = b; }
        }
        K = best_K; bits = best_bits;
        u64 rgb = 1; for (int e = 0; e < best_g; e++) rgb *= radix;
        kp.g = best_g; kp.fb = bitlen(rgb - 1); kp.nf = (K + best_g - 1) / best_g; kp.gl = K - (kp.nf - 1) * best_g;
        u64 rl = 1; for (int e = 0; e < kp.gl; e++) rl *= radix;
        kp.fbl = bitlen(rl - 1); kp.bits = bits; kp.rad = radix; kp.fmask = (1u << kp.fb) - 1u; kp.lmask = (1u << kp.fbl) - 1u;
        kp.lscale = (u32)(rgb / rl); kp.fdiv = (1u << 16) / (u32)kp.fb + 1u;
        kp.lastmul = kp.gl == best_g ? (1u << 20) : (u32)(((1ull << 20) + kp.lscale - 1) / kp.lscale);
        for (int i = 1; i < KP_MAXG; i++) {
            u64 d = 1; for (int e = 0; e < best_g - i; e++) d *= radix;
            kp.dmul[i - 1] = i < best_g ? (u32)(((1ull << 20) + d - 1) / d) : 0u;
        }
    }
    s.sigma = sigma; s.bits = bits; s.k0 = K;
    RV_HIP(hipMemcpyAsync(d_lut.p, lut, 256, hipMemcpyHostToDevice, q));
    bool fused = LCP && BWT && d_maxlcp && bits <= 48 && !ws.opt.no_fused_lcp;
    KeyDigits kd;
    kd.ly.sortmask = bits >= 64 ? ~0ull : (1ull << bits) - 1;
    kd.ly.at_bits = K <= 30 ? 5 : 8; kd.ly.at_shift = 56 - kd.ly.at_bits;
    kd.ly.nd_shift = (bits + 7) / 8 * 8; kd.ly.nd_bits = 0;
    kd.D = (side_sep > 0 && (int64_t)side_sep < n - 1) ? (int64_t)side_sep + 1 : 0;
    kd.ns = 0;
    for (int q2 = 0; q2 < HINT_K - 1; q2++) kd.sep[q2] = std::numeric_limits<int64_t>::max();
    for (int q2 = 0; q2 < HINT_K; q2++) kd.Ds[q2] = 0;
    if (seps && nseps > 0 && kd.D > 0) {
        kd.ns = (nseps + 1 < HINT_K + 1) ? nseps + 1 : HINT_K + 1;
        if (kd.ns > HINT_K) kd.ns = HINT_K;
        for (int q2 = 0; q2 < kd.ns - 1; q2++) kd.sep[q2] = seps[q2];
        for (int q2 = 1; q2 < kd.ns; q2++) kd.Ds[q2] = seps[q2 - 1] + 1;
        if (nseps + 1 > HINT_K) kd.ns = 0;
    }
    const bool want_hint = fused && kd.D > 0 && kd.ns >= 2 && kd.ly.at_shift - kd.ly.nd_shift >= 8 && !ws.opt.no_diag && !ws.opt.no_packed_text;
    if (want_hint) kd.ly.nd_bits = std::min(kd.ly.at_shift - kd.ly.nd_shift - 1, 11);
    kd.K = K; kd.kp = kp; kd.stop0 = lut[(uint8_t)'$']; kd.stop1 = lut[(uint8_t)'N'];
    if (fused) RV_HIP(hipMemsetAsync(d_maxlcp, 0, sizeof(u32), q));

    DBuf &bk0 = ws.sa[0], &bk1 = ws.sa[1], &bv0 = ws.sa[2], &bv1 = ws.sa[3], &bhead = ws.sa[4], &bseed = ws.sa[5], &bgrp = ws.sa[6], &bisa = ws.sa[7],
         &bP0 = ws.sa[8], &bP1 = ws.sa[9], &bG0 = ws.sa[10], &bG1 = ws.sa[11], &btile = ws.sa[12], &bbig = ws.sa[13], &bQb = ws.sa[14], &bPb = ws.sa[15];
    auto freeall = [&]() {};
#define SA_TRY(x) do { int r__ = (x); if (r__) { freeall(); return r__; } } while (0)
#define SA_HIP(x) do { hipError_t e__ = (x); if (e__ != hipSuccess) { rv_set_error("%s:%d %s", __FILE__, __LINE__, hipGetErrorString(e__)); freeall(); return -1; } } while (0)
    SA_TRY(bk0.reserve((size_t)n * 8)); SA_TRY(bk1.reserve((size_t)n * 8));
    SA_TRY(bv0.reserve((size_t)n * sizeof(sav_t))); SA_TRY(bv1.reserve((size_t)n * sizeof(sav_t)));
    SA_TRY(bhead.reserve((size_t)n + 16));
    auto need_seed_grp = [&](int64_t cnt) -> int {
        RV_TRY(bseed.reserve((size_t)std::max<int64_t>(cnt, 1) * (sizeof(sav_t) > 4 ? sizeof(sav_t) : 4)));
        return bgrp.reserve((size_t)std::max<int64_t>(cnt, 1) * 4);
    };
    SA_TRY(bisa.reserve((size_t)n * 4));
    const unsigned nblk = (unsigned)ceil_div(n, TB);

    DiagBits dg; dg.stop = dg.exc = dg.lt = nullptr; dg.D = kd.D; dg.tab = 0;
    kd.dtab = nullptr;
    const int64_t nw = (n + 63) / 64;
    DiagSamples dsm; dsm.ns = kd.ns;
    for (int q2 = 0; q2 < HINT_K - 1; q2++) dsm.sep[q2] = kd.sep[q2];
    for (int q2 = 0; q2 < HINT_K; q2++) dsm.Ds[q2] = kd.Ds[q2];
    if (kd.ly.nd_bits > 0) {
        DBuf &bds = ws.sa[20], &bde = ws.sa[21], &bdl = ws.sa[22];
        SA_TRY(bds.reserve((size_t)nw * 8)); SA_TRY(bde.reserve((size_t)nw * 8)); SA_TRY(bdl.reserve((size_t)nw * 8));
        hipLaunchKernelGGL(k_diag_bits, dim3((unsigned)ceil_div(nw, TB)), dim3(TB), 0, q, T, n, dsm, bds.as<u64>(), bde.as<u64>(), bdl.as<u64>(), nw);
        SA_HIP(hipGetLastError());
        dg.stop = bds.as<u64>(); dg.exc = bde.as<u64>(); dg.lt = bdl.as<u64>();
    }
    const bool collapse = fused && kd.ly.nd_bits > 0 && kd.ns == 2 && K < 64 && kd.D > 1 && n > kd.D + 1 && !ws.opt.no_heads_fusion && !ws.opt.no_twin_collapse
                          && (sizeof(sav_t) > 4 || n < ((int64_t)1 << 31));
    int64_t nsort = n;
    const u32 *tw_off = nullptr;
    if (collapse) {
        const int64_t ntiles = ceil_div(n, KEY_TILE);
        DBuf &btw = ws.sa[23];
        SA_TRY(btw.reserve((size_t)(std::max<int64_t>(ntiles, ceil_div(n, TB)) + 1) * 4 + 64));
        u32 *tc = btw.as<u32>();
        auto count_kept = [&](int tab, u32 *kept_out) -> int {
            hipLaunchKernelGGL(k_tw_count, dim3((unsigned)ceil_div(nw, TB)), dim3(TB), 0, q, (const u64 *)dg.stop, nw, K, kd.D, n, tc, ntiles, tab);
            RV_LAUNCH_CHECK();
            RV_TRY(rv_exclusive_sum_u32(ws, tc, tc, ntiles + 1));
            return rv_read_back(ws, kept_out, tc + ntiles, 4);
        };
        u32 kept = 0;
        SA_TRY(count_kept(0, &kept));
        const int dt_mode = (int)ws.opt.diag_table;
        const int64_t n2 = n - kd.D;
        if (dt_mode != 0 && n >= 4096 && (dt_mode == 1 || (int64_t)kept * 10 > n2 * 3)) {
            const int64_t mseeds = nw * SEED_SLOTS;
            DBuf &bdt = ws.sa[25];
            const int64_t ndt = (n >> DT_SHIFT) + 1;
            SA_TRY(bdt.reserve((size_t)ndt * 8 + 64));
            int32_t *raw = bdt.as<int32_t>(), *tab = raw + ndt;
            const int did = ws.prof_begin(11 , (double)n + (double)mseeds * 12.0);
            hipLaunchKernelGGL(k_seed_sample, dim3((unsigned)ceil_div(nw, TB)), dim3(TB), 0, q, T, n, bk0.as<u64>(), bv0.as<sav_t>(), nw);
            SA_HIP(hipGetLastError());
            int sin1 = 0;
            SA_TRY(rv_radix_sort_pairs<sav_t>(ws, bk0.as<u64>(), bv0.as<sav_t>(), bk1.as<u64>(), bv1.as<sav_t>(), mseeds, 0, 40, &sin1));
            SA_HIP(hipMemsetAsync(raw, 0x7f, (size_t)ndt * 4, q));
            hipLaunchKernelGGL(k_seed_pairs, dim3((unsigned)ceil_div(mseeds, TB)), dim3(TB), 0, q, (const u64 *)(sin1 ? bk1.as<u64>() : bk0.as<u64>()),
                               (const sav_t *)(sin1 ? bv1.as<sav_t>() : bv0.as<sav_t>()), mseeds, kd.D, kd.D, raw);
            SA_HIP(hipGetLastError());
            hipLaunchKernelGGL(k_dtab_fill, dim3((unsigned)ceil_div(ndt, TB)), dim3(TB), 0, q, T, n, kd.D, kd.D, (const int32_t *)raw, tab, ndt);
            SA_HIP(hipGetLastError());
            DiagTab dt; dt.dtab = tab; dt.S2 = kd.D; dt.D = kd.D;
            hipLaunchKernelGGL(k_diag_bits_tab, dim3((unsigned)ceil_div(nw, TB)), dim3(TB), 0, q, T, n, dt, ws.sa[20].as<u64>(), ws.sa[21].as<u64>(), ws.sa[22].as<u64>(), nw);
            SA_HIP(hipGetLastError());
            ws.prof_end(did);
            u32 kept_tab = 0;
            SA_TRY(count_kept(1, &kept_tab));
            if (dt_mode == 1 || (int64_t)kept_tab * 5 < (int64_t)kept * 4) { kept = kept_tab; kd.dtab = tab; dg.tab = 1; }
            else {
                hipLaunchKernelGGL(k_diag_bits, dim3((unsigned)ceil_div(nw, TB)), dim3(TB), 0, q, T, n, dsm, ws.sa[20].as<u64>(), ws.sa[21].as<u64>(), ws.sa[22].as<u64>(), nw);
                SA_HIP(hipGetLastError());
                SA_TRY(count_kept(0, &kept));
            }
        }
        nsort = kd.D + (int64_t)kept;
        tw_off = tc;
        s.diag_table = dg.tab;
    }
    uint8_t *dig0 = nullptr;
    {
        const int64_t iktiles = ceil_div(n, KEY_TILE);
        const dim3 ig((unsigned)std::min<int64_t>(iktiles, 256 * 8));
        dig0 = rv_radix_first_digits(ws, nsort, 0, bits);
#define RV_IK_(G) hipLaunchKernelGGL(k_init_keys<G>, ig, dim3(TB), 0, q, T, n, d_lut.as<uint8_t>(), K, kp, bk0.as<u64>(), bv0.as<sav_t>(), fused ? 1 : 0, \
                                     kd.stop0, kd.stop1, kd.ly, dg, tw_off, iktiles, dig0)
        const int ikid = ws.prof_begin(12 , (double)n + (double)nsort * (8.0 + sizeof(sav_t) + 1.0));
        switch (kp.g) { case 1: RV_IK_(1); break; case 2: RV_IK_(2); break; case 3: RV_IK_(3); break; case 4: RV_IK_(4); break; default: RV_IK_(5); break; }
        ws.prof_end(ikid);
#undef RV_IK_
    }
    SA_HIP(hipGetLastError());
    int in1 = 0;
    SA_TRY(rv_radix_sort_pairs<sav_t>(ws, bk0.as<u64>(), bv0.as<sav_t>(), bk1.as<u64>(), bv1.as<sav_t>(), nsort, 0, bits, &in1, dig0 != nullptr));
    s.radix_passes += rv_radix_passes(ws, bits); s.sorted_elems += nsort;
    u64 *ks = in1 ? bk1.as<u64>() : bk0.as<u64>();
    sav_t *vs = in1 ? bv1.as<sav_t>() : bv0.as<sav_t>();
    u64 *kt = in1 ? bk0.as<u64>() : bk1.as<u64>();
    sav_t *vt = in1 ? bv0.as<sav_t>() : bv1.as<sav_t>();

    uint8_t *head = bhead.as<uint8_t>();
    if (!collapse) SA_TRY(need_seed_grp(n));
    u32 *seed = bseed.as<u32>(), *grp = bgrp.as<u32>(), *ISA = bisa.as<u32>();
    const u64 *keys_by_rank = ks;
    const sav_t *vals_by_rank = vs;
    if (collapse) {
        const int64_t nb = ceil_div(nsort, TC_TILE);
        u32 *bc = ws.sa[23].as<u32>();
        hipLaunchKernelGGL(k_tw_flags, dim3((unsigned)nb), dim3(TB), 0, q, (const sav_t *)vs, nsort, bc);
        SA_HIP(hipGetLastError());
        SA_TRY(rv_exclusive_sum_u32(ws, bc, bc, nb));
        sav_t *vexp = reinterpret_cast<sav_t *>(bisa.p);
        if (sizeof(sav_t) > 4) { SA_TRY(ws.sa[24].reserve((size_t)n * sizeof(sav_t))); vexp = ws.sa[24].as<sav_t>(); }
        const int pbid = ws.prof_begin(13 , (double)nsort * 2.0 * (8.0 + sizeof(sav_t)) + (double)n * (1.0 + sizeof(sa_t) + sizeof(lcp_t) + 1.0));
        hipLaunchKernelGGL(k_heads_publish_tc, dim3((unsigned)nb), dim3(TB), 0, q, (const u64 *)ks, (const sav_t *)vs, nsort, (const u32 *)bc, head, LCP, SA, BWT,
                           side_sep, kd, d_maxlcp, ws.opt.no_pub_twins ? 0 : 1, kt, vexp);
        ws.prof_end(pbid);
        SA_HIP(hipGetLastError());
        keys_by_rank = kt; vals_by_rank = vexp;
    } else if (fused && kd.ly.nd_bits > 0 && !ws.opt.no_heads_fusion) {
        hipLaunchKernelGGL(k_heads_publish, dim3((unsigned)ceil_div(n, (int64_t)HP_ITEMS * TB)), dim3(TB), 0, q, (const u64 *)ks, (const sav_t *)vs, n, head, seed, LCP, SA, BWT, side_sep, kd, d_maxlcp,
                           ws.opt.no_pub_twins ? 0 : 1);
        SA_HIP(hipGetLastError());
        SA_TRY(rv_inclusive_max_u32(ws, seed, grp, n));
    } else {
        hipLaunchKernelGGL(k_heads, dim3(nblk), dim3(TB), 0, q, (const u64 *)ks, n, head, seed, fused ? LCP : (lcp_t *)nullptr, kd, fused ? d_maxlcp : (u32 *)nullptr);
        SA_HIP(hipGetLastError());
        SA_TRY(rv_inclusive_max_u32(ws, seed, grp, n));
        {
            KeyDigits kp = kd;
            if (ws.opt.no_pub_twins) kp.ly.nd_bits = 0;
            hipLaunchKernelGGL(k_publish0, dim3(nblk), dim3(TB), 0, q, (const sav_t *)vs, n, SA, (const u64 *)ks, fused ? BWT : (uint8_t *)nullptr, side_sep,
                               kp, fused ? LCP : (lcp_t *)nullptr, head, d_maxlcp, grp);
        }
        SA_HIP(hipGetLastError());
    }
    bool isa_built = false;
    const sav_t *cur_S = nullptr; const u32 *cur_G = nullptr; int64_t cur_m = 0;
    auto need_isa = [&]() -> int {
        if (isa_built) return 0;
        hipLaunchKernelGGL(k_isa_identity, dim3(nblk), dim3(TB), 0, q, (const sa_t *)SA, n, ISA);
        RV_LAUNCH_CHECK();
        if (cur_m > 0) {
            hipLaunchKernelGGL(k_round_isa, dim3((unsigned)ceil_div(cur_m, TB)), dim3(TB), 0, q, cur_S, cur_G, cur_m, ISA);
            RV_LAUNCH_CHECK();
        }
        isa_built = true;
        return 0;
    };

    int64_t ntile = ceil_div(n, CP_TILE);
    SA_TRY(btile.reserve(std::max((size_t)(ntile + 1) * 8 + 64, (size_t)RT_REGIONS * 4)));
    u32 *tile = btile.as<u32>();
    auto count_unsorted = [&](const uint8_t *hd, int64_t len, int64_t *m_out) -> int {
        const int64_t nt = ceil_div(len, CP_TILE);
        hipLaunchKernelGGL(k_cp_count, dim3((unsigned)nt), dim3(TB), 0, q, hd, len, tile);
        RV_LAUNCH_CHECK();
        RV_TRY(rv_exclusive_sum_u32(ws, tile, tile, nt + 1));
        u32 tot = 0;
        RV_TRY(rv_read_back(ws, &tot, tile + nt, 4));
        *m_out = tot;
        return 0;
    };
    auto emit_unsorted = [&](const uint8_t *hd, int64_t len, const u32 *pos_in, const sav_t *suf_in, const u32 *grp_in, u32 *P, sav_t *S, u32 *G,
                             const uint8_t *cls_in = nullptr, uint8_t *cls_out = nullptr, int cls_is = 0) -> int {
        const int64_t nt = ceil_div(len, CP_TILE);
        hipLaunchKernelGGL(k_cp_emit, dim3((unsigned)nt), dim3(TB), 0, q, hd, len, (const u32 *)tile, pos_in, suf_in, grp_in, P, S, G, cls_in, cls_out, cls_is);
        RV_LAUNCH_CHECK();
        return 0;
    };
    int64_t m = 0;
    if (collapse) {
        u32 *tlast = tile + (ntile + 1);
        hipLaunchKernelGGL(k_cp_count_g, dim3((unsigned)ntile), dim3(TB), 0, q, (const uint8_t *)head, n, tile, tlast);
        SA_HIP(hipGetLastError());
        SA_TRY(rv_exclusive_sum_u32(ws, tile, tile, ntile + 1));
        SA_TRY(rv_inclusive_max_u32(ws, tlast, tlast, ntile));
        u32 tot = 0;
        SA_TRY(rv_read_back(ws, &tot, tile + ntile, 4));
        m = tot;
        SA_TRY(bP0.reserve((size_t)std::max<int64_t>(m, 1) * 4)); SA_TRY(bG0.reserve((size_t)std::max<int64_t>(m, 1) * 4));
        SA_TRY(need_seed_grp(m));
        seed = bseed.as<u32>(); grp = bgrp.as<u32>();
        if (m > 0) {
            hipLaunchKernelGGL(k_cp_emit_g, dim3((unsigned)ntile), dim3(TB), 0, q, (const uint8_t *)head, n, (const u32 *)tile, (const u32 *)tlast, vals_by_rank,
                               bP0.as<u32>(), vt, bG0.as<u32>());
            SA_HIP(hipGetLastError());
        }
    } else {
        SA_TRY(count_unsorted(head, n, &m));
        SA_TRY(bP0.reserve((size_t)std::max<int64_t>(m, 1) * 4)); SA_TRY(bG0.reserve((size_t)std::max<int64_t>(m, 1) * 4));
        if (m > 0) SA_TRY(emit_unsorted(head, n, nullptr, vals_by_rank, grp, bP0.as<u32>(), vt, bG0.as<u32>()));
    }
    const int64_t m_list0 = m;
    u32 *P = bP0.as<u32>(), *G = bG0.as<u32>(), *Pn = nullptr, *Gn = nullptr;
    sav_t *S = vt;
    sav_t *Sfree = vs;
    u64 *kA = ks, *kB = kt;
    if (m > 0) { SA_TRY(bbig.reserve((size_t)m + 16)); SA_TRY(bQb.reserve((size_t)m * 4)); SA_TRY(bPb.reserve((size_t)m * 4)); }

    const int lowbits = bitlen((u64)n), highbits = bitlen((u64)(n > 1 ? n - 1 : 1));
    int64_t h = K;
    const bool can_far = fused && kd.ly.nd_bits > 0 && kd.ns == 2 && dg.stop != nullptr && !ws.opt.no_far_twins;
    const bool can_list = fused && !ws.opt.no_lcp_list;
    bool text_round_ran = false, far_ran = false, partial = false;
    DBuf &btodo = ws.sa[26];
    int64_t ntodo = 0;
    auto todo_add = [&](const u32 *ranks, int64_t cnt) -> int {
        if (cnt <= 0) return 0;
        if ((size_t)(ntodo + cnt) * 4 > btodo.cap) {
            DBuf nb;
            RV_TRY(nb.reserve((size_t)(ntodo + cnt) * 4 * 2 + 1024));
            if (ntodo) RV_HIP(hipMemcpyAsync(nb.p, btodo.p, (size_t)ntodo * 4, hipMemcpyDeviceToDevice, q));
            RV_HIP(hipStreamSynchronize(q));
            btodo.release();
            btodo = nb;
        }
        RV_HIP(hipMemcpyAsync(btodo.as<u32>() + ntodo, ranks, (size_t)cnt * 4, hipMemcpyDeviceToDevice, q));
        ntodo += cnt;
        return 0;
    };
    auto leave_fused = [&](const u32 *ranks, int64_t cnt) -> int {
        if (!fused) return 0;
        if (!can_list) { fused = false; return 0; }
        partial = true;
        return todo_add(ranks, cnt);
    };
    bool list_in_todo = false;
    DBuf &bcls0 = ws.sa[30], &bcls1 = ws.sa[31];
    uint8_t *cls = nullptr, *cls_next = nullptr;
    while (m > 0) {
        if (h >= 2 * n + 2 + 2 * TEXT_LIM) { rv_set_error("SA build: did not converge"); freeall(); return -1; }
        s.rounds++;
        const unsigned mb = (unsigned)ceil_div(m, TB);
        uint8_t *bigflag = bbig.as<uint8_t>();
        cur_S = S; cur_G = G; cur_m = m;
        const bool far_round = text_round_ran && !far_ran && can_far;
        const bool text_round = !far_round && s.rounds == 1 && h <= 64 && !ws.opt.sa_no_text;
        bool text_big = false;
        if (far_round) {
            far_ran = true;
            DBuf &bR = ws.sa[27], &bM = ws.sa[28];
            const int64_t nw1 = ceil_div(kd.D - 1, (int64_t)64);
            SA_TRY(bR.reserve(std::max((size_t)nw * 4 + 64, (size_t)(nw1 * 64 + 64) * 4))); SA_TRY(bM.reserve((size_t)nw * 4 + 64));
            hipLaunchKernelGGL(k_far_rev, dim3((unsigned)ceil_div(nw, TB)), dim3(TB), 0, q, (const u64 *)dg.stop, nw, bR.as<u32>());
            SA_HIP(hipGetLastError());
            SA_TRY(rv_inclusive_max_u32(ws, bR.as<u32>(), bM.as<u32>(), nw));
            FarTwins ft; ft.stop = dg.stop; ft.exc = dg.exc; ft.lt = dg.lt; ft.M = bM.as<u32>(); ft.nw = nw; ft.n = n; ft.S2 = kd.D; ft.D = kd.D; ft.dtab = kd.dtab;
// ... 136 lines not shown
```

### reveal_amd/csrc/rv_prims.hip

```cpp
#include "rv_common.h"
#include <string.h>

namespace {

constexpr int SCAN_THREADS = 256;
constexpr int SCAN_ITEMS   = 8;
constexpr int SCAN_TILE    = SCAN_THREADS * SCAN_ITEMS;

template <class T> struct OpSum {
    __device__ static T id() { return (T)0; }
    __device__ static T f(T a, T b) { return a + b; }
};
template <class T> struct OpMax {
    __device__ static T id() { return (T)0; }
    __device__ static T f(T a, T b) { return a > b ? a : b; }
};

template <class T> __device__ inline T shfl_up_t(T v, int d) { return __shfl_up(v, d, 64); }
template <> __device__ inline u64 shfl_up_t<u64>(u64 v, int d) {
    u32 lo = __shfl_up((u32)v, d, 64), hi = __shfl_up((u32)(v >> 32), d, 64);
    return ((u64)hi << 32) | lo;
}

template <class T, class Op>
__device__ inline T block_exclusive(T x, T *lds , T *total) {
    const int lane = threadIdx.x & 63, w = threadIdx.x >> 6;
    T inc = x;
#pragma unroll
    for (int d = 1; d < 64; d <<= 1) {
        T t = shfl_up_t<T>(inc, d);
        if (lane >= d) inc = Op::f(t, inc);
    }
    T exc = shfl_up_t<T>(inc, 1);
    if (lane == 0) exc = Op::id();
    if (lane == 63) lds[w] = inc;
    __syncthreads();
    T base = Op::id(), tot = Op::id();
#pragma unroll
    for (int k = 0; k < SCAN_THREADS / 64; k++) {
        T v = lds[k];
        if (k < w) base = Op::f(base, v);
        tot = Op::f(tot, v);
    }
    __syncthreads();
    *total = tot;
    return Op::f(base, exc);
}

template <class T, class Op>
__global__ __launch_bounds__(SCAN_THREADS) void k_tile_reduce(const T *__restrict__ in, T *__restrict__ totals, int64_t n) {
    __shared__ T lds[4];
    const int64_t base = (int64_t)blockIdx.x * SCAN_TILE + (int64_t)threadIdx.x * SCAN_ITEMS;
    T acc = Op::id();
    if (base + SCAN_ITEMS <= n) {
        T v[SCAN_ITEMS];
        __builtin_memcpy(v, in + base, sizeof v);
#pragma unroll
        for (int i = 0; i < SCAN_ITEMS; i++) acc = Op::f(acc, v[i]);
    } else {
#pragma unroll
        for (int i = 0; i < SCAN_ITEMS; i++)
            if (base + i < n) acc = Op::f(acc, in[base + i]);
    }
    T tot;
    (void)block_exclusive<T, Op>(acc, lds, &tot);
    if (threadIdx.x == 0) totals[blockIdx.x] = tot;
}

template <class T, class Op, bool INCL>
__global__ __launch_bounds__(SCAN_THREADS) void k_tile_scan(const T *in, T *out, const T *__restrict__ tile_prefix, int64_t n) {
    __shared__ T lds[4];
    const int64_t base = (int64_t)blockIdx.x * SCAN_TILE + (int64_t)threadIdx.x * SCAN_ITEMS;
    T v[SCAN_ITEMS];
    const bool whole = base + SCAN_ITEMS <= n;
    if (whole) __builtin_memcpy(v, in + base, sizeof v);
    else {
#pragma unroll
        for (int i = 0; i < SCAN_ITEMS; i++) v[i] = (base + i < n) ? in[base + i] : Op::id();
    }
    T acc = Op::id();
#pragma unroll
    for (int i = 0; i < SCAN_ITEMS; i++) acc = Op::f(acc, v[i]);
    T tot;
    T pre = block_exclusive<T, Op>(acc, lds, &tot);
    if (tile_prefix) pre = Op::f(tile_prefix[blockIdx.x], pre);
    if (whole) {
        T o[SCAN_ITEMS];
#pragma unroll
        for (int i = 0; i < SCAN_ITEMS; i++) { const T nx = Op::f(pre, v[i]); o[i] = INCL ? nx : pre; pre = nx; }
        __builtin_memcpy(out + base, o, sizeof o);
        return;
    }
#pragma unroll
    for (int i = 0; i < SCAN_ITEMS; i++) {
        T nx = Op::f(pre, v[i]);
        if (base + i < n) out[base + i] = INCL ? nx : pre;
        pre = nx;
    }
}

template <class T, class Op, bool INCL>
int scan_rec(Workspace &ws, const T *in, T *out, int64_t n, int level) {
    if (n <= 0) return 0;
    const int64_t nt = ceil_div(n, SCAN_TILE);
    if (nt == 1) {
        hipLaunchKernelGGL((k_tile_scan<T, Op, INCL>), dim3(1), dim3(SCAN_THREADS), 0, ws.stream, in, out, (const T *)nullptr, n);
        RV_LAUNCH_CHECK();
        return 0;
    }
    if (level >= 4) { rv_set_error("scan: too many levels"); return -1; }
    RV_TRY(ws.scan_tmp[level].reserve((size_t)nt * sizeof(T)));
    T *tot = ws.scan_tmp[level].as<T>();
    hipLaunchKernelGGL((k_tile_reduce<T, Op>), dim3((unsigned)nt), dim3(SCAN_THREADS), 0, ws.stream, in, tot, n);
    RV_LAUNCH_CHECK();
    RV_TRY((scan_rec<T, Op, false>(ws, tot, tot, nt, level + 1)));
    hipLaunchKernelGGL((k_tile_scan<T, Op, INCL>), dim3((unsigned)nt), dim3(SCAN_THREADS), 0, ws.stream, in, out, (const T *)tot, n);
    RV_LAUNCH_CHECK();
    return 0;
}

}

int rv_exclusive_sum_u32(Workspace &ws, const u32 *in, u32 *out, int64_t n) { return scan_rec<u32, OpSum<u32>, false>(ws, in, out, n, 0); }
int rv_exclusive_sum_u64(Workspace &ws, const u64 *in, u64 *out, int64_t n) { return scan_rec<u64, OpSum<u64>, false>(ws, in, out, n, 0); }
int rv_inclusive_max_u32(Workspace &ws, const u32 *in, u32 *out, int64_t n) { return scan_rec<u32, OpMax<u32>, true>(ws, in, out, n, 0); }
int rv_inclusive_max_u64(Workspace &ws, const u64 *in, u64 *out, int64_t n) { return scan_rec<u64, OpMax<u64>, true>(ws, in, out, n, 0); }

namespace {

#ifndef RV_RS_THREADS
#define RV_RS_THREADS 256
#endif
constexpr int RS_THREADS = RV_RS_THREADS;
#ifndef RV_RS_ITEMS
#define RV_RS_ITEMS 16
#endif
constexpr int RS_ITEMS   = RV_RS_ITEMS;
constexpr int RS_TILE    = RS_THREADS * RS_ITEMS;
constexpr int RS_WAVES   = RS_THREADS / 64;

constexpr unsigned RS_XCDS = 8;
template <bool XCD> __device__ inline u32 rs_tile_of(u32 nb) {
    if (!XCD) return blockIdx.x;
    const u32 chunk = (nb + RS_XCDS - 1) / RS_XCDS;
    return (blockIdx.x % RS_XCDS) * chunk + blockIdx.x / RS_XCDS;
}

template <int BITS, bool XCD>
__global__ __launch_bounds__(RS_THREADS) void k_rs_hist(const u64 *__restrict__ keys, int64_t n, int shift, u32 dmask, u32 *__restrict__ blockhist, u32 nblocks) {
    constexpr int NB = 1 << BITS;
    __shared__ u32 h[NB];
    const u32 tile = rs_tile_of<XCD>(nblocks);
    if (tile >= nblocks) return;
    for (int k = threadIdx.x; k < NB; k += RS_THREADS) h[k] = 0;
    __syncthreads();
    const int64_t base = (int64_t)tile * RS_TILE;
    u64 key[RS_ITEMS];
#pragma unroll
    for (int r = 0; r < RS_ITEMS; r++) {
        const int64_t i = base + (int64_t)r * RS_THREADS + threadIdx.x;
        key[r] = i < n ? keys[i] : 0ull;
    }
#pragma unroll
    for (int r = 0; r < RS_ITEMS; r++) {
        const int64_t i = base + (int64_t)r * RS_THREADS + threadIdx.x;
        if (i < n) atomicAdd(&h[(u32)(key[r] >> shift) & dmask], 1u);
    }
    __syncthreads();
    for (int k = threadIdx.x; k < NB; k += RS_THREADS) blockhist[(size_t)k * nblocks + tile] = h[k];
}

template <bool XCD>
__global__ __launch_bounds__(RS_THREADS) void k_rs_hist_bytes(const uint8_t *__restrict__ digits, int64_t n, u32 *__restrict__ blockhist, u32 nblocks) {
    static_assert(RS_ITEMS == 16, "sixteen digit bytes per thread");
    __shared__ u32 h[256];
    const u32 tile = rs_tile_of<XCD>(nblocks);
    if (tile >= nblocks) return;
    h[threadIdx.x] = 0;
    __syncthreads();
    const int64_t i0 = (int64_t)tile * RS_TILE + (int64_t)threadIdx.x * 16;
    if (i0 + 16 <= n) {
        const uint4 v = *reinterpret_cast<const uint4 *>(digits + i0);
        const u32 w[4] = {v.x, v.y, v.z, v.w};
#pragma unroll
        for (int k = 0; k < 4; k++)
#pragma unroll
            for (int b = 0; b < 4; b++) atomicAdd(&h[(w[k] >> (8 * b)) & 255u], 1u);
    } else {
        for (int64_t i = i0; i < n && i < i0 + 16; i++) atomicAdd(&h[digits[i]], 1u);
    }
    __syncthreads();
    blockhist[(size_t)threadIdx.x * nblocks + tile] = h[threadIdx.x];
}

template <class V, int BITS, bool XCD, class CNT>
__global__ __launch_bounds__(RS_THREADS) void k_rs_scatter(const u64 *__restrict__ kin, const V *__restrict__ vin,
                                                            u64 *__restrict__ kout, V *__restrict__ vout, int64_t n, int shift, u32 dmask,
                                                            const u32 *__restrict__ blockoff, u32 nblocks, uint8_t *__restrict__ dnext, int nshift, u32 nmask) {
    constexpr int NB = 1 << BITS;
    constexpr int BPT = NB / RS_THREADS;
    static_assert(NB % RS_THREADS == 0 && RS_TILE < 65536, "bins per thread, 16-bit counters");
    __shared__ CNT cnt[RS_WAVES][NB];
    __shared__ u32 gbase[NB];
    __shared__ CNT dstart[NB];
    __shared__ u32 wtot[RS_WAVES];
    __shared__ u64 skey[RS_TILE];
    __shared__ V sval[RS_TILE];
    const u32 tile = rs_tile_of<XCD>(nblocks);
    if (tile >= nblocks) return;
    const int lane = threadIdx.x & 63, w = threadIdx.x >> 6;
    for (int k = threadIdx.x; k < RS_WAVES * NB; k += RS_THREADS) (&cnt[0][0])[k] = 0;
    for (int k = threadIdx.x; k < NB; k += RS_THREADS) gbase[k] = blockoff[(size_t)k * nblocks + tile];
    __syncthreads();

    const int64_t wbase = (int64_t)tile * RS_TILE + (int64_t)w * (64 * RS_ITEMS);
    u64 key[RS_ITEMS];
    V val[RS_ITEMS];
    u32 rnk[RS_ITEMS];
    const u64 lt = (lane == 0) ? 0ull : (~0ull >> (64 - lane));
#pragma unroll
    for (int r = 0; r < RS_ITEMS; r++) {
        const int64_t i = wbase + (int64_t)r * 64 + lane;
        key[r] = i < n ? kin[i] : ~0ull;
    }
#pragma unroll
    for (int r = 0; r < RS_ITEMS; r++) {
        const int64_t i = wbase + (int64_t)r * 64 + lane;
        val[r] = i < n ? vin[i] : V(0);
    }
#pragma unroll
    for (int r = 0; r < RS_ITEMS; r++) {
        const int64_t i = wbase + (int64_t)r * 64 + lane;
        const bool valid = i < n;
        const u32 d = (u32)(key[r] >> shift) & dmask;
        u64 peers = __ballot(valid);
#pragma unroll
        for (int b = 0; b < BITS; b++) {
            const bool bit = (d >> b) & 1u;
            const u64 bal = __ballot(bit);
            peers &= bit ? bal : ~bal;
        }
        const u32 below = (u32)__popcll(peers & lt);
        const u32 old = cnt[w][d];
        __builtin_amdgcn_wave_barrier();
        if (valid && below == 0) cnt[w][d] = (CNT)(old + (u32)__popcll(peers));
        __builtin_amdgcn_wave_barrier();
        rnk[r] = old + below;
    }
    __syncthreads();
    u32 tot[BPT], mytot = 0;
#pragma unroll
    for (int b = 0; b < BPT; b++) {
        const int d = threadIdx.x * BPT + b;
        u32 run = 0;
#pragma unroll
        for (int k = 0; k < RS_WAVES; k++) { const u32 c = cnt[k][d]; cnt[k][d] = (CNT)run; run += c; }
        tot[b] = run; mytot += run;
    }
    {
        u32 inc = mytot;
#pragma unroll
        for (int dd = 1; dd < 64; dd <<= 1) { const u32 t = __shfl_up(inc, dd, 64); if (lane >= dd) inc += t; }
        if (lane == 63) wtot[w] = inc;
        __syncthreads();
        u32 before = inc - mytot;
#pragma unroll
        for (int k = 0; k < RS_WAVES; k++) if (k < w) before += wtot[k];
#pragma unroll
        for (int b = 0; b < BPT; b++) { dstart[threadIdx.x * BPT + b] = (CNT)before; before += tot[b]; }
    }
    __syncthreads();
#pragma unroll
    for (int r = 0; r < RS_ITEMS; r++) {
        const int64_t i = wbase + (int64_t)r * 64 + lane;
        if (i < n) {
            const u32 d = (u32)(key[r] >> shift) & dmask;
            const u32 li = (u32)dstart[d] + (u32)cnt[w][d] + rnk[r];
            skey[li] = key[r];
            sval[li] = val[r];
        }
    }
    __syncthreads();
    const int64_t tbase = (int64_t)tile * RS_TILE;
    const u32 nvalid = (u32)((n - tbase) < (int64_t)RS_TILE ? (n - tbase) : (int64_t)RS_TILE);
    for (u32 li = threadIdx.x; li < nvalid; li += RS_THREADS) {
        const u64 k = skey[li];
        const u32 d = (u32)(k >> shift) & dmask;
        const size_t dst = (size_t)gbase[d] + (li - (u32)dstart[d]);
        kout[dst] = k;
        vout[dst] = sval[li];
        if (dnext) dnext[dst] = (uint8_t)((u32)(k >> nshift) & nmask);
    }
}

template <class V, int BITS, bool XCD, class CNT>
static void rs_scatter_launch(hipStream_t q, u32 nb, const u64 *ki, const V *vi, u64 *ko, V *vo, int64_t n, int shift, u32 dmask, const u32 *bh,
                              uint8_t *dnext, int nshift, u32 nmask) {
    const u32 grid = XCD ? RS_XCDS * ((nb + RS_XCDS - 1) / RS_XCDS) : nb;
    hipLaunchKernelGGL((k_rs_scatter<V, BITS, XCD, CNT>), dim3(grid), dim3(RS_THREADS), 0, q, ki, vi, ko, vo, n, shift, dmask, bh, nb, dnext, nshift, nmask);
}

}

int rv_radix_passes(const Workspace &ws, int nbits) {
    const int w = ws.opt.rs_bits == 10 ? 10 : 8;
    return nbits <= 0 ? 0 : (nbits + w - 1) / w;
}

static bool rs_digit_bytes(const Workspace &ws, int64_t n, int bit_lo, int bit_hi) {
    return ws.opt.rs_bits != 10 && !ws.opt.rs_no_digit_bytes && n > 1 && n >= ((int64_t)1 << 20) && n < ((int64_t)1 << 32) && bit_hi - bit_lo > 8;
}
uint8_t *rv_radix_first_digits(Workspace &ws, int64_t n, int bit_lo, int bit_hi) {
    if (!rs_digit_bytes(ws, n, bit_lo, bit_hi) || ws.rs_digits.reserve((size_t)n + 64)) return nullptr;
    return ws.rs_digits.as<uint8_t>();
}

template <class V>
int rv_radix_sort_pairs(Workspace &ws, u64 *k0, V *v0, u64 *k1, V *v1, int64_t n, int bit_lo, int bit_hi, int *result_in_1, bool first_digits) {
    *result_in_1 = 0;
    if (n <= 1 || bit_hi <= bit_lo) return 0;
    if (n >= ((int64_t)1 << 32)) { rv_set_error("radix sort: n >= 2^32 not supported"); return -1; }
    const int width = ws.opt.rs_bits == 10 ? 10 : 8;
    const bool xcd = ws.opt.rs_xcd != 0, c16 = ws.opt.rs_cnt16 != 0;
    const u32 nb = (u32)ceil_div(n, RS_TILE);
    RV_TRY(ws.rs_hist.reserve(((size_t)1 << width) * nb * sizeof(u32)));
    u32 *bh = ws.rs_hist.as<u32>();
    const bool bytes = rs_digit_bytes(ws, n, bit_lo, bit_hi);
    if (first_digits && (!bytes || ws.rs_digits.cap < (size_t)n + 64)) { rv_set_error("radix sort: first digits announced but the byte path is off"); return -1; }
    if (bytes) RV_TRY(ws.rs_digits.reserve((size_t)n + 64));
    uint8_t *dig = bytes ? ws.rs_digits.as<uint8_t>() : nullptr;
    bool have_digits = first_digits;
    u64 *ki = k0, *ko = k1;
    V *vi = v0, *vo = v1;
    int flip = 0;
    for (int shift = bit_lo; shift < bit_hi; shift += width) {
        const int wbits = bit_hi - shift < width ? bit_hi - shift : width;
        const u32 dmask = (1u << wbits) - 1u;
        int pid = ws.prof_begin(8 , (have_digits ? 1.0 : 8.0) * (double)n);
        const u32 hgrid = xcd ? RS_XCDS * ((nb + RS_XCDS - 1) / RS_XCDS) : nb;
        if (have_digits) {
            if (xcd) hipLaunchKernelGGL((k_rs_hist_bytes<true>), dim3(hgrid), dim3(RS_THREADS), 0, ws.stream, (const uint8_t *)dig, n, bh, nb);
            else hipLaunchKernelGGL((k_rs_hist_bytes<false>), dim3(hgrid), dim3(RS_THREADS), 0, ws.stream, (const uint8_t *)dig, n, bh, nb);
        } else if (width == 10) { if (xcd) hipLaunchKernelGGL((k_rs_hist<10, true>), dim3(hgrid), dim3(RS_THREADS), 0, ws.stream, (const u64 *)ki, n, shift, dmask, bh, nb);
                           else hipLaunchKernelGGL((k_rs_hist<10, false>), dim3(hgrid), dim3(RS_THREADS), 0, ws.stream, (const u64 *)ki, n, shift, dmask, bh, nb); }
        else             { if (xcd) hipLaunchKernelGGL((k_rs_hist<8, true>), dim3(hgrid), dim3(RS_THREADS), 0, ws.stream, (const u64 *)ki, n, shift, dmask, bh, nb);
                           else hipLaunchKernelGGL((k_rs_hist<8, false>), dim3(hgrid), dim3(RS_THREADS), 0, ws.stream, (const u64 *)ki, n, shift, dmask, bh, nb); }
        RV_LAUNCH_CHECK();
        ws.prof_end(pid);
        RV_TRY(rv_exclusive_sum_u32(ws, bh, bh, ((int64_t)1 << width) * nb));
        const int nshift = shift + width;
        const bool more = nshift < bit_hi;
        const u32 nmask = more ? ((1u << (bit_hi - nshift < width ? bit_hi - nshift : width)) - 1u) : 0u;
        uint8_t *dn = (bytes && more) ? dig : nullptr;
        pid = ws.prof_begin(7 , (2.0 * (8.0 + sizeof(V)) + (dn ? 1.0 : 0.0)) * (double)n);
#define RS_GO(B_, X_, C_) rs_scatter_launch<V, B_, X_, C_>(ws.stream, nb, (const u64 *)ki, (const V *)vi, ko, vo, n, shift, dmask, (const u32 *)bh, dn, nshift, nmask)
        if (width == 10) { if (xcd) { if (c16) RS_GO(10, true, uint16_t); else RS_GO(10, true, u32); } else { if (c16) RS_GO(10, false, uint16_t); else RS_GO(10, false, u32); } }
        else             { if (xcd) { if (c16) RS_GO(8, true, uint16_t); else RS_GO(8, true, u32); } else { if (c16) RS_GO(8, false, uint16_t); else RS_GO(8, false, u32); } }
#undef RS_GO
        RV_LAUNCH_CHECK();
        ws.prof_end(pid);
        have_digits = dn != nullptr;
        u64 *tk = ki; ki = ko; ko = tk;
        V *tv = vi; vi = vo; vo = tv;
        flip ^= 1;
    }
    *result_in_1 = flip;
    return 0;
}

__global__ __launch_bounds__(256) void k_h2d_copy(const uint4 *__restrict__ src, uint4 *__restrict__ dst, size_t n16) {
    for (size_t i = (size_t)blockIdx.x * 256 + threadIdx.x; i < n16; i += (size_t)gridDim.x * 256) dst[i] = src[i];
}
int rv_read_back(Workspace &ws, void *dst, const void *dsrc, size_t bytes) {
    RV_TRY(ws.hpin.reserve(bytes < 4096 ? 4096 : bytes));
    if (!ws.ev_rb) RV_HIP(hipEventCreateWithFlags(&ws.ev_rb, hipEventDisableTiming));
    RV_HIP(hipMemcpyAsync(ws.hpin.p, dsrc, bytes, hipMemcpyDeviceToHost, ws.stream));
    RV_HIP(hipEventRecord(ws.ev_rb, ws.stream));
    const hipError_t e = rv_event_wait(ws.ev_rb);
    if (e != hipSuccess) { rv_set_error("rv_read_back: %s", hipGetErrorString(e)); return -1; }
    memcpy(dst, ws.hpin.p, bytes);
    return 0;
}

int rv_read_back2(Workspace &ws, void *dst_a, const void *dsrc_a, size_t bytes_a, void *dst_b, const void *dsrc_b, size_t bytes_b) {
    const size_t off = (bytes_a + 63) & ~(size_t)63;
    RV_TRY(ws.hpin.reserve(off + bytes_b < 4096 ? 4096 : off + bytes_b));
    if (!ws.ev_rb) RV_HIP(hipEventCreateWithFlags(&ws.ev_rb, hipEventDisableTiming));
    RV_HIP(hipMemcpyAsync(ws.hpin.p, dsrc_a, bytes_a, hipMemcpyDeviceToHost, ws.stream));
    RV_HIP(hipMemcpyAsync((uint8_t *)ws.hpin.p + off, dsrc_b, bytes_b, hipMemcpyDeviceToHost, ws.stream));
    RV_HIP(hipEventRecord(ws.ev_rb, ws.stream));
    const hipError_t e = rv_event_wait(ws.ev_rb);
    if (e != hipSuccess) { rv_set_error("rv_read_back2: %s", hipGetErrorString(e)); return -1; }
    memcpy(dst_a, ws.hpin.p, bytes_a);
    memcpy(dst_b, (const uint8_t *)ws.hpin.p + off, bytes_b);
    return 0;
}

int rv_h2d_copy(Workspace &ws, const void *pinned_src, void *dst, size_t bytes) {
    const size_t n16 = (bytes + 15) / 16;
    if (n16 == 0) return 0;
    size_t blocks = (n16 + 255) / 256;
    if (blocks > 512) blocks = 512;
    hipLaunchKernelGGL(k_h2d_copy, dim3((unsigned)blocks), dim3(256), 0, ws.stream, (const uint4 *)pinned_src, (uint4 *)dst, n16);
    RV_LAUNCH_CHECK();
    return 0;
}

template int rv_radix_sort_pairs<u32>(Workspace &, u64 *, u32 *, u64 *, u32 *, int64_t, int, int, int *, bool);
template int rv_radix_sort_pairs<u64>(Workspace &, u64 *, u64 *, u64 *, u64 *, int64_t, int, int, int *, bool);
```

Measured before the change: 25190.

## Defer lowest radix digit to a snapped final pass in suffix sort

```diff
diff --git a/include/reveal_amd.h b/include/reveal_amd.h
--- a/include/reveal_amd.h
+++ b/include/reveal_amd.h
@@ -218,7 +218,9 @@
 int rv_test_exclusive_sum_u32(const uint32_t *in, uint32_t *out, int64_t n);
 int rv_test_inclusive_max_u32(const uint32_t *in, uint32_t *out, int64_t n);
 int rv_test_radix_sort(uint64_t *keys, uint32_t *vals, int64_t n, int bit_lo, int bit_hi);
+int rv_test_radix_sort_fin(uint64_t *keys, uint32_t *vals, int64_t n, int bit_lo, int bit_hi, int S, int W, int G, int64_t min_n, int64_t *info);
 int rv_test_radix_time(int64_t n, int bits, int dist, int flags, int iters, double *ms, int64_t *bad);
+int rv_test_radix_time_fin(int64_t n, int bits, int dist, int flags, int iters, double *ms, int64_t *bad, int S, int W, int G, int64_t *info);
 
 #ifdef __cplusplus
 }
diff --git a/reveal_amd/_index.py b/reveal_amd/_index.py
--- a/reveal_amd/_index.py
+++ b/reveal_amd/_index.py
@@ -169,8 +169,12 @@
             self._dll.rv_sa_stats(self._h, *[ctypes.byref(x) for x in v], ctypes.byref(se), ctypes.byref(rp))
             tail = (ctypes.c_int64 * 2)()
             self._dll.rv_sa_tail(self._h, tail)
+            ev = np.zeros(len(_lib.CAPACITY_EVENTS), dtype=np.int64)
+            self._dll.rv_capacity_events(self._h, ev.ctypes.data)
+            ev = dict(zip(_lib.CAPACITY_EVENTS, ev))
             return dict(sigma=v[0].value, bits=v[1].value, k0=v[2].value, rounds=v[3].value, sorted_elems=se.value, radix_passes=rp.value,
-                        diag_table=int(self._dll.rv_sa_diag_table(self._h)), far_pairs=int(tail[0]), lcp_list=int(tail[1]))
+                        diag_table=int(self._dll.rv_sa_diag_table(self._h)), far_pairs=int(tail[0]), lcp_list=int(tail[1]),
+                        sort_deferred=int(ev["sort_deferred"]), sort_unsnapped=int(ev["sort_unsnapped"]), sort_fallback=int(ev["sort_fallback"]))
 
         def construct(self, rc=0):
             if self._sx:
diff --git a/reveal_amd/_lib.py b/reveal_amd/_lib.py
--- a/reveal_amd/_lib.py
+++ b/reveal_amd/_lib.py
@@ -10,7 +10,7 @@
 K_SCAN_PAIR, K_SCAN_MULTI, K_SA_SORT, K_LCP, K_SPLIT, K_LABEL, K_BUBBLE, K_RADIX_SCATTER, K_RADIX_HIST, K_TEXT_ROUND, K_CASCADE, K_DIAG_TABLE, K_INIT_KEYS, K_PUBLISH = range(14)
 
 CAPACITY_EVENTS = ("pair_ovf", "pair_out", "pair_pick_ovf", "pair_second_copy", "multi_rec", "multi_mem", "multi_cand",
-                   "mems_rec", "mems_mem", "mems_long")
+                   "mems_rec", "mems_mem", "mems_long", "sort_deferred", "sort_unsnapped", "sort_fallback")
 CAP_SITES = {"multi_cand": 1, "cas_wit": 2, "cas_tables": 4, "casm_matches": 8, "casm_wit": 16, "casm_tables": 32,
              "mems_rec": 64, "mems_mem": 128, "mems_long": 256}
 
@@ -170,7 +170,9 @@
     "rv_test_exclusive_sum_u32": (_I, [V, V, _L]),
     "rv_test_inclusive_max_u32": (_I, [V, V, _L]),
     "rv_test_radix_sort": (_I, [V, V, _L, _I, _I]),
+    "rv_test_radix_sort_fin": (_I, [V, V, _L, _I, _I, _I, _I, _I, _L, V]),
     "rv_test_radix_time": (_I, [_L, _I, _I, _I, _I, ctypes.POINTER(_D), c_i64p]),
+    "rv_test_radix_time_fin": (_I, [_L, _I, _I, _I, _I, ctypes.POINTER(_D), c_i64p, _I, _I, _I, V]),
 }
 
 
diff --git a/reveal_amd/csrc/rv_api.hip b/reveal_amd/csrc/rv_api.hip
--- a/reveal_amd/csrc/rv_api.hip
+++ b/reveal_amd/csrc/rv_api.hip
@@ -1164,6 +1164,25 @@
     return r;
 }
 
+int rv_test_radix_sort_fin(uint64_t *keys, uint32_t *vals, int64_t n, int bit_lo, int bit_hi, int S, int W, int G, int64_t min_n, int64_t *info) {
+    Workspace ws;
+    RV_TRY(test_ws(ws));
+    ws.opt.rs_fin_stride = S; ws.opt.rs_fin_window = W; ws.opt.rs_fin_group = G; ws.opt.rs_fin_min_n = min_n;
+    DBuf k0, k1, v0, v1;
+    int r = 0, in1 = 0;
+    if (k0.reserve((size_t)n * 8 + 64) || k1.reserve((size_t)n * 8 + 64) || v0.reserve((size_t)n * 4 + 64) || v1.reserve((size_t)n * 4 + 64)) r = -1;
+    if (!r && hipMemcpy(k0.p, keys, (size_t)n * 8, hipMemcpyHostToDevice) != hipSuccess) r = -1;
+    if (!r && hipMemcpy(v0.p, vals, (size_t)n * 4, hipMemcpyHostToDevice) != hipSuccess) r = -1;
+    if (!r) r = rv_radix_sort_pairs<u32>(ws, k0.as<u64>(), v0.as<u32>(), k1.as<u64>(), v1.as<u32>(), n, bit_lo, bit_hi, &in1, false, true);
+    if (!r && hipStreamSynchronize(ws.stream) != hipSuccess) { rv_set_error("sync failed: %s", hipGetErrorString(hipGetLastError())); r = -1; }
+    if (!r && hipMemcpy(keys, in1 ? k1.p : k0.p, (size_t)n * 8, hipMemcpyDeviceToHost) != hipSuccess) r = -1;
+    if (!r && hipMemcpy(vals, in1 ? v1.p : v0.p, (size_t)n * 4, hipMemcpyDeviceToHost) != hipSuccess) r = -1;
+    if (info) for (int k = 0; k < 4; k++) info[k] = ws.rs_info[k];
+    k0.release(); k1.release(); v0.release(); v1.release();
+    test_ws_done(ws);
+    return r;
+}
+
 }
 namespace {
 __device__ inline u64 rt_mix(u64 x) { x ^= x >> 33; x *= 0xff51afd7ed558ccdull; x ^= x >> 33; x *= 0xc4ceb9fe1a85ec53ull; x ^= x >> 33; return x; }
@@ -1186,10 +1205,12 @@
     if (a > b || (a == b && vals[i] > vals[i + 1])) atomicAdd(bad, 1ull);
 }
 }
-extern "C" {
-int rv_test_radix_time(int64_t n, int bits, int dist, int flags, int iters, double *ms, int64_t *bad) {
+static int radix_time(int64_t n, int bits, int dist, int flags, int iters, double *ms, int64_t *bad, int S, int W, int G, int64_t *info) {
     Workspace ws;
     RV_TRY(test_ws(ws));
+    if (S > 0) ws.opt.rs_fin_stride = S;
+    if (W > 0) ws.opt.rs_fin_window = W;
+    if (G > 0) ws.opt.rs_fin_group = G;
     ws.opt.rs_bits = (flags & 1) ? 10 : 8; ws.opt.rs_xcd = (flags & 2) ? 1 : 0; ws.opt.rs_cnt16 = (flags & 4) ? 1 : 0; ws.opt.rs_no_digit_bytes = (flags & 8) ? 1 : 0;
     DBuf k0, k1, v0, v1, db;
     int r = 0, in1 = 0;
@@ -1199,11 +1220,12 @@
     for (int it = 0; !r && it < iters; it++) {
         hipLaunchKernelGGL(k_rt_fill, dim3((unsigned)ceil_div(n, 256)), dim3(256), 0, ws.stream, k0.as<u64>(), v0.as<u32>(), n, bits, dist);
         (void)hipEventRecord(e0, ws.stream);
-        r = rv_radix_sort_pairs<u32>(ws, k0.as<u64>(), v0.as<u32>(), k1.as<u64>(), v1.as<u32>(), n, 0, bits, &in1);
+        r = rv_radix_sort_pairs<u32>(ws, k0.as<u64>(), v0.as<u32>(), k1.as<u64>(), v1.as<u32>(), n, 0, bits, &in1, false, (flags & 16) != 0);
         (void)hipEventRecord(e1, ws.stream);
         if (!r && hipEventSynchronize(e1) != hipSuccess) { rv_set_error("sync failed: %s", hipGetErrorString(hipGetLastError())); r = -1; }
         float t = 0;
         if (!r) { (void)hipEventElapsedTime(&t, e0, e1); ms[it] = t; }
+        if (!r && info) for (int k = 0; k < 4; k++) info[k] = ws.rs_info[k];
     }
     if (!r) {
         (void)hipMemsetAsync(db.p, 0, 8, ws.stream);
@@ -1219,5 +1241,10 @@
     test_ws_done(ws);
     return r;
 }
-
-}
+extern "C" {
+int rv_test_radix_time(int64_t n, int bits, int dist, int flags, int iters, double *ms, int64_t *bad) { return radix_time(n, bits, dist, flags, iters, ms, bad, 0, 0, 0, nullptr); }
+int rv_test_radix_time_fin(int64_t n, int bits, int dist, int flags, int iters, double *ms, int64_t *bad, int S, int W, int G, int64_t *info) {
+    return radix_time(n, bits, dist, flags, iters, ms, bad, S, W, G, info);
+}
+
+}
diff --git a/reveal_amd/csrc/rv_common.h b/reveal_amd/csrc/rv_common.h
--- a/reveal_amd/csrc/rv_common.h
+++ b/reveal_amd/csrc/rv_common.h
@@ -87,6 +87,12 @@
     X(rs_xcd, "RV_RS_XCD", 1) \
     X(rs_cnt16, "RV_RS_CNT16", 1) \
     X(rs_no_digit_bytes, "RV_RS_NO_DIGIT_BYTES", 0) \
+    X(rs_no_finish_low, "RV_RS_NO_FINISH_LOW", 0) \
+    X(rs_fin_min_n, "RV_RS_FIN_MIN_N", 1 << 20) \
+    X(rs_fin_stride, "RV_RS_FIN_STRIDE", 3712) \
+    X(rs_fin_window, "RV_RS_FIN_WINDOW", 384) \
+    X(rs_fin_group, "RV_RS_FIN_GROUP", 16) \
+    X(rs_fin_share, "RV_RS_FIN_SHARE", 4) \
     X(diag_table, "RV_DIAG_TABLE", -1) \
     X(no_cascade_chain, "RV_NO_CASCADE_CHAIN", 0) \
     X(casm_rank_count, "RV_CASM_RANK_COUNT", 0) \
@@ -290,7 +296,9 @@
 };
 
 enum RvCapEvent { RV_CE_PAIR_OVF = 0, RV_CE_PAIR_OUT, RV_CE_PAIR_PICK_OVF, RV_CE_PAIR_SECOND_COPY, RV_CE_MULTI_REC, RV_CE_MULTI_MEM, RV_CE_MULTI_CAND,
-                  RV_CE_MEMS_REC, RV_CE_MEMS_MEM, RV_CE_MEMS_LONG, RV_CE_COUNT };
+                  RV_CE_MEMS_REC, RV_CE_MEMS_MEM, RV_CE_MEMS_LONG,
+                  RV_CE_SORT_DEFERRED, RV_CE_SORT_UNSNAPPED, RV_CE_SORT_FALLBACK,
+                  RV_CE_COUNT };
 enum RvCapSite { RV_CS_MULTI_CAND = 1, RV_CS_CAS_WIT = 2, RV_CS_CAS_TABLES = 4, RV_CS_CASM_MATCHES = 8, RV_CS_CASM_WIT = 16, RV_CS_CASM_TABLES = 32,
                  RV_CS_MEMS_REC = 64, RV_CS_MEMS_MEM = 128, RV_CS_MEMS_LONG = 256 };
 struct Workspace {
@@ -306,6 +314,8 @@
     DBuf scan_tmp[4];
     DBuf rs_hist;
     DBuf rs_digits;
+    DBuf rs_fin[4];
+    int64_t rs_info[4] = {0, 0, 0, 0};
     DBuf misc[20];
     DBuf sa[32];
     HBuf hpin;
@@ -326,6 +336,7 @@
         if (ev_rb) { (void)hipEventDestroy(ev_rb); ev_rb = nullptr; }
         for (auto &b : scan_tmp) b.release();
         rs_hist.release(); rs_digits.release();
+        for (auto &b : rs_fin) b.release();
         for (auto &b : misc) b.release();
         for (auto &b : sa) b.release();
     }
@@ -346,8 +357,8 @@
 int rv_radix_passes(const Workspace &ws, int nbits);
 template <class V>
 int rv_radix_sort_pairs(Workspace &ws, u64 *k0, V *v0, u64 *k1, V *v1, int64_t n,
-                        int bit_lo, int bit_hi, int *result_in_1, bool first_digits = false);
-uint8_t *rv_radix_first_digits(Workspace &ws, int64_t n, int bit_lo, int bit_hi);
+                        int bit_lo, int bit_hi, int *result_in_1, bool first_digits = false, bool finish_low = false);
+uint8_t *rv_radix_first_digits(Workspace &ws, int64_t n, int bit_lo, int bit_hi, bool finish_low = false, int vbytes = 4, int *digit_shift = nullptr);
 
 int rv_read_back(Workspace &ws, void *dst, const void *dsrc, size_t bytes);
 int rv_read_back2(Workspace &ws, void *dst_a, const void *dsrc_a, size_t bytes_a, void *dst_b, const void *dsrc_b, size_t bytes_b);
diff --git a/reveal_amd/csrc/rv_construct.hip b/reveal_amd/csrc/rv_construct.hip
--- a/reveal_amd/csrc/rv_construct.hip
+++ b/reveal_amd/csrc/rv_construct.hip
@@ -358,7 +358,7 @@
 __global__ __launch_bounds__(TB) void k_init_keys(const uint8_t *__restrict__ T, int64_t n, const uint8_t *__restrict__ lut, int K, KeyPack kp,
                                                   u64 *__restrict__ keys, sav_t *__restrict__ vals, int pay, u32 stop0, u32 stop1,
                                                   KeyLayout ly, DiagBits dg, const u32 *__restrict__ tw_off , int64_t ntiles,
-                                                  uint8_t *__restrict__ dig0 ) {
+                                                  uint8_t *__restrict__ dig0 , int dsh) {
     __shared__ u32 code32[IK_WORDS + 2];
     __shared__ u32 s_sc[IK_WORDS / 8 + 3];
     __shared__ uint8_t slut[256], sstop[256];
@@ -486,7 +486,7 @@
                 key |= (u64)(known ? (u32)d | ((f >> 1) << ly.nd_bits) : (u32)nd_none) << ly.nd_shift;
             }
             keys[obase + j] = key; vals[obase + j] = (sav_t)i;
-            if (dig0) dig0[obase + j] = (uint8_t)key;
+            if (dig0) dig0[obase + j] = (uint8_t)(key >> dsh);
         }
     } else {
     constexpr int PER = KEY_TILE / TB;
@@ -539,10 +539,10 @@
                 ulonglong2 *vd2 = reinterpret_cast<ulonglong2 *>(vals + i0);
                 vd2[0] = make_ulonglong2((u64)oval[0], (u64)oval[1]); vd2[1] = make_ulonglong2((u64)oval[2], (u64)oval[3]);
             }
-            if (dig0) *reinterpret_cast<u32 *>(dig0 + i0) = ((u32)okey[0] & 0xffu) | (((u32)okey[1] & 0xffu) << 8) | (((u32)okey[2] & 0xffu) << 16) | ((u32)okey[3] << 24);
+            if (dig0) *reinterpret_cast<u32 *>(dig0 + i0) = ((u32)(okey[0] >> dsh) & 0xffu) | (((u32)(okey[1] >> dsh) & 0xffu) << 8) | (((u32)(okey[2] >> dsh) & 0xffu) << 16) | ((u32)(okey[3] >> dsh) << 24);
         } else {
 #pragma unroll
-            for (int r = 0; r < PER; r++) if (i0 + r < n) { keys[i0 + r] = okey[r]; vals[i0 + r] = oval[r]; if (dig0) dig0[i0 + r] = (uint8_t)okey[r]; }
+            for (int r = 0; r < PER; r++) if (i0 + r < n) { keys[i0 + r] = okey[r]; vals[i0 + r] = oval[r]; if (dig0) dig0[i0 + r] = (uint8_t)(okey[r] >> dsh); }
         }
     } else {
 #pragma unroll
@@ -552,11 +552,11 @@
             if (i >= n) continue;
             const int xw = k >> 6, b = k & 63;
             const bool twin = (s_tw[xw] >> b) & 1ull;
-            if (i < dg.D) { keys[i] = okey[r]; vals[i] = (sav_t)i | (twin ? TW_FLAG : (sav_t)0); if (dig0) dig0[i] = (uint8_t)okey[r]; }
+            if (i < dg.D) { keys[i] = okey[r]; vals[i] = (sav_t)i | (twin ? TW_FLAG : (sav_t)0); if (dig0) dig0[i] = (uint8_t)(okey[r] >> dsh); }
             else if (!twin) {
                 const int64_t o = dg.D + (int64_t)tw_off[tile] + s_kpre[xw] + (u32)__popcll(s_keep[xw] & ((b == 0) ? 0ull : (~0ull >> (64 - b))));
                 keys[o] = okey[r]; vals[o] = (sav_t)i;
-                if (dig0) dig0[o] = (uint8_t)okey[r];
+                if (dig0) dig0[o] = (uint8_t)(okey[r] >> dsh);
             }
         }
     }
@@ -2340,12 +2340,13 @@
         s.diag_table = dg.tab;
     }
     uint8_t *dig0 = nullptr;
+    int dig_shift = 0;
     {
         const int64_t iktiles = ceil_div(n, KEY_TILE);
         const dim3 ig((unsigned)std::min<int64_t>(iktiles, 256 * 8));
-        dig0 = rv_radix_first_digits(ws, nsort, 0, bits);
+        dig0 = rv_radix_first_digits(ws, nsort, 0, bits, true, (int)sizeof(sav_t), &dig_shift);
 #define RV_IK_(G) hipLaunchKernelGGL(k_init_keys<G>, ig, dim3(TB), 0, q, T, n, d_lut.as<uint8_t>(), K, kp, bk0.as<u64>(), bv0.as<sav_t>(), fused ? 1 : 0, \
-                                     kd.stop0, kd.stop1, kd.ly, dg, tw_off, iktiles, dig0)
+                                     kd.stop0, kd.stop1, kd.ly, dg, tw_off, iktiles, dig0, dig_shift)
         const int ikid = ws.prof_begin(12 , (double)n + (double)nsort * (8.0 + sizeof(sav_t) + 1.0));
         switch (kp.g) { case 1: RV_IK_(1); break; case 2: RV_IK_(2); break; case 3: RV_IK_(3); break; case 4: RV_IK_(4); break; default: RV_IK_(5); break; }
         ws.prof_end(ikid);
@@ -2353,8 +2354,9 @@
     }
     SA_HIP(hipGetLastError());
     int in1 = 0;
-    SA_TRY(rv_radix_sort_pairs<sav_t>(ws, bk0.as<u64>(), bv0.as<sav_t>(), bk1.as<u64>(), bv1.as<sav_t>(), nsort, 0, bits, &in1, dig0 != nullptr));
-    s.radix_passes += rv_radix_passes(ws, bits); s.sorted_elems += nsort;
+    SA_TRY(rv_radix_sort_pairs<sav_t>(ws, bk0.as<u64>(), bv0.as<sav_t>(), bk1.as<u64>(), bv1.as<sav_t>(), nsort, 0, bits, &in1, dig0 != nullptr, true));
+    s.radix_passes += (int)ws.rs_info[0]; s.sorted_elems += nsort;
+    ws.cap_events[RV_CE_SORT_UNSNAPPED] += ws.rs_info[1]; ws.cap_events[RV_CE_SORT_DEFERRED] += ws.rs_info[2]; ws.cap_events[RV_CE_SORT_FALLBACK] += ws.rs_info[3];
     u64 *ks = in1 ? bk1.as<u64>() : bk0.as<u64>();
     sav_t *vs = in1 ? bv1.as<sav_t>() : bv0.as<sav_t>();
     u64 *kt = in1 ? bk0.as<u64>() : bk1.as<u64>();
diff --git a/reveal_amd/csrc/rv_prims.hip b/reveal_amd/csrc/rv_prims.hip
--- a/reveal_amd/csrc/rv_prims.hip
+++ b/reveal_amd/csrc/rv_prims.hip
@@ -1,5 +1,6 @@
 #include "rv_common.h"
 #include <string.h>
+#include <type_traits>
 
 namespace {
 
@@ -193,10 +194,67 @@
     blockhist[(size_t)threadIdx.x * nblocks + tile] = h[threadIdx.x];
 }
 
-template <class V, int BITS, bool XCD, class CNT>
+struct RsFinArgs {
+    const u32 *snap;
+    const uint8_t *unsn;
+    u32 *bitmap;
+    u32 *counters;
+    u64 gmask, rmask;
+    int lo, gshift;
+    u32 G;
+};
+struct RsNoFin {};
+
+__global__ __launch_bounds__(256) void k_rs_snap(const u64 *__restrict__ keys, int64_t n, u32 nt, u32 S, u32 W, int gshift, u64 rmask,
+                                                 u32 *__restrict__ snap, uint8_t *__restrict__ unsn, u32 *__restrict__ counters) {
+    const u32 t = blockIdx.x * 4 + (threadIdx.x >> 6), lane = threadIdx.x & 63;
+    if (t > nt) return;
+    if (t == 0 || t == nt) { if (lane == 0) { snap[t] = t ? (u32)n : 0u; unsn[t] = 0; } return; }
+    const int64_t b = (int64_t)S * t;
+    for (u32 o = 0; o <= W; o += 64) {
+        const int64_t i = b + o + lane;
+        bool hit = false;
+        if (o + lane <= W && i <= n) hit = i == n || ((keys[i] >> gshift) & rmask) != ((keys[i - 1] >> gshift) & rmask);
+        const u64 m = __ballot(hit);
+        if (m) { if (lane == 0) { snap[t] = (u32)(b + o + (u32)__builtin_ctzll(m)); unsn[t] = 0; } return; }
+    }
+    if (lane == 0) { snap[t] = (u32)b; unsn[t] = 1; atomicAdd(&counters[1], 1u); }
+}
+
+template <bool XCD>
+__global__ __launch_bounds__(RS_THREADS) void k_rs_hist_snap(const u64 *__restrict__ keys, const uint8_t *__restrict__ digits, const u32 *__restrict__ snap,
+                                                             int shift, u32 dmask, u32 *__restrict__ blockhist, u32 nblocks) {
+    static_assert(RS_THREADS == 256, "a bin per thread");
+    __shared__ u32 h[256];
+    const u32 tile = rs_tile_of<XCD>(nblocks);
+    if (tile >= nblocks) return;
+    h[threadIdx.x] = 0;
+    __syncthreads();
+    const int64_t lo = snap[tile], hi = snap[tile + 1];
+    if (digits) {
+        for (int64_t c = (lo >> 4) + threadIdx.x; (c << 4) < hi; c += RS_THREADS) {
+            const uint4 v = *reinterpret_cast<const uint4 *>(digits + (c << 4));
+            const u32 w[4] = {v.x, v.y, v.z, v.w};
+#pragma unroll
+            for (int k = 0; k < 4; k++)
+#pragma unroll
+                for (int b = 0; b < 4; b++) {
+                    const int64_t i = (c << 4) + 4 * k + b;
+                    if (i >= lo && i < hi) atomicAdd(&h[(w[k] >> (8 * b)) & 255u], 1u);
+                }
+        }
+    } else {
+        for (int64_t i = lo + threadIdx.x; i < hi; i += RS_THREADS) atomicAdd(&h[(u32)(keys[i] >> shift) & dmask], 1u);
+    }
+    __syncthreads();
+    blockhist[(size_t)threadIdx.x * nblocks + tile] = h[threadIdx.x];
+}
+
+template <class V, int BITS, bool XCD, class CNT, bool FIN = false>
 __global__ __launch_bounds__(RS_THREADS) void k_rs_scatter(const u64 *__restrict__ kin, const V *__restrict__ vin,
-                                                            u64 *__restrict__ kout, V *__restrict__ vout, int64_t n, int shift, u32 dmask,
-                                                            const u32 *__restrict__ blockoff, u32 nblocks, uint8_t *__restrict__ dnext, int nshift, u32 nmask) {
+                                                            u64 *__restrict__ kout, V *__restrict__ vout, int64_t n_all, int shift, u32 dmask,
+                                                            const u32 *__restrict__ blockoff, u32 nblocks, uint8_t *__restrict__ dnext, int nshift, u32 nmask,
+                                                            typename std::conditional<FIN, RsFinArgs, RsNoFin>::type fin) {
     constexpr int NB = 1 << BITS;
     constexpr int BPT = NB / RS_THREADS;
     static_assert(NB % RS_THREADS == 0 && RS_TILE < 65536, "bins per thread, 16-bit counters");
@@ -213,7 +271,9 @@
     for (int k = threadIdx.x; k < NB; k += RS_THREADS) gbase[k] = blockoff[(size_t)k * nblocks + tile];
     __syncthreads();
 
-    const int64_t wbase = (int64_t)tile * RS_TILE + (int64_t)w * (64 * RS_ITEMS);
+    int64_t tbase = (int64_t)tile * RS_TILE, n = n_all;
+    if constexpr (FIN) { tbase = fin.snap[tile]; n = fin.snap[tile + 1]; }
+    const int64_t wbase = tbase + (int64_t)w * (64 * RS_ITEMS);
     u64 key[RS_ITEMS];
     V val[RS_ITEMS];
     u32 rnk[RS_ITEMS];
@@ -281,8 +341,48 @@
         }
     }
     __syncthreads();
-    const int64_t tbase = (int64_t)tile * RS_TILE;
     const u32 nvalid = (u32)((n - tbase) < (int64_t)RS_TILE ? (n - tbase) : (int64_t)RS_TILE);
+    u32 defm = 0;
+    if constexpr (FIN) {
+        const bool ul = fin.unsn[tile] != 0, ur = fin.unsn[tile + 1] != 0;
+        const u64 rl = ul ? (kin[tbase] >> fin.gshift) & fin.rmask : 0ull, rr = ur ? (kin[n] >> fin.gshift) & fin.rmask : 0ull;
+#pragma unroll
+        for (int r = 0; r < RS_ITEMS; r++) {
+            const u32 li = threadIdx.x + (u32)r * RS_THREADS;
+            u32 ns = li;
+            if (li < nvalid) {
+                const u64 k = skey[li];
+                const u64 g = (k >> fin.gshift) & fin.gmask;
+                const u32 d0 = (u32)(k >> fin.lo) & 255u;
+                u32 a = li, b = li, steps = 0, ahead = 0;
+                bool big = false;
+                while (a > 0) {
+                    const u64 o = skey[a - 1];
+                    if (((o >> fin.gshift) & fin.gmask) != g) break;
+                    if (++steps >= fin.G) { big = true; break; }
+                    ahead += ((u32)(o >> fin.lo) & 255u) <= d0; a--;
+                }
+                while (!big && b + 1 < nvalid) {
+                    const u64 o = skey[b + 1];
+                    if (((o >> fin.gshift) & fin.gmask) != g) break;
+                    if (++steps >= fin.G) { big = true; break; }
+                    ahead += ((u32)(o >> fin.lo) & 255u) < d0; b++;
+                }
+                const u64 run = g & fin.rmask;
+                if (big || (ul && run == rl) || (ur && run == rr)) defm |= 1u << r;
+                else ns = a + ahead;
+                key[r] = k; val[r] = sval[li];
+            }
+            rnk[r] = ns;
+        }
+        __syncthreads();
+#pragma unroll
+        for (int r = 0; r < RS_ITEMS; r++) {
+            const u32 li = threadIdx.x + (u32)r * RS_THREADS;
+            if (li < nvalid && rnk[r] != li) { skey[rnk[r]] = key[r]; sval[rnk[r]] = val[r]; }
+        }
+        __syncthreads();
+    }
     for (u32 li = threadIdx.x; li < nvalid; li += RS_THREADS) {
         const u64 k = skey[li];
         const u32 d = (u32)(k >> shift) & dmask;
@@ -290,6 +390,13 @@
         kout[dst] = k;
         vout[dst] = sval[li];
         if (dnext) dnext[dst] = (uint8_t)((u32)(k >> nshift) & nmask);
+        if constexpr (FIN) { if ((defm >> (li / RS_THREADS)) & 1u) atomicOr(&fin.bitmap[dst >> 5], 1u << (dst & 31)); }
+    }
+    if constexpr (FIN) {
+        u32 c = (u32)__popc(defm);
+#pragma unroll
+        for (int dd = 32; dd >= 1; dd >>= 1) c += __shfl_xor(c, dd, 64);
+        if (lane == 0 && c) atomicAdd(&fin.counters[0], c);
     }
 }
 
@@ -297,7 +404,63 @@
 static void rs_scatter_launch(hipStream_t q, u32 nb, const u64 *ki, const V *vi, u64 *ko, V *vo, int64_t n, int shift, u32 dmask, const u32 *bh,
                               uint8_t *dnext, int nshift, u32 nmask) {
     const u32 grid = XCD ? RS_XCDS * ((nb + RS_XCDS - 1) / RS_XCDS) : nb;
-    hipLaunchKernelGGL((k_rs_scatter<V, BITS, XCD, CNT>), dim3(grid), dim3(RS_THREADS), 0, q, ki, vi, ko, vo, n, shift, dmask, bh, nb, dnext, nshift, nmask);
+    hipLaunchKernelGGL((k_rs_scatter<V, BITS, XCD, CNT>), dim3(grid), dim3(RS_THREADS), 0, q, ki, vi, ko, vo, n, shift, dmask, bh, nb, dnext, nshift, nmask, RsNoFin());
+}
+template <class V, bool XCD, class CNT>
+static void rs_scatter_fin_launch(hipStream_t q, u32 nt, const u64 *ki, const V *vi, u64 *ko, V *vo, int64_t n, int shift, u32 dmask, const u32 *bh, const RsFinArgs &fin) {
+    const u32 grid = XCD ? RS_XCDS * ((nt + RS_XCDS - 1) / RS_XCDS) : nt;
+    if constexpr (sizeof(V) == 4)
+        hipLaunchKernelGGL((k_rs_scatter<V, 8, XCD, CNT, true>), dim3(grid), dim3(RS_THREADS), 0, q, ki, vi, ko, vo, n, shift, dmask, bh, nt, (uint8_t *)nullptr, 0, 0u, fin);
+}
+
+constexpr int FD_TB = 256;
+__global__ __launch_bounds__(FD_TB) void k_fin_count(const u32 *__restrict__ bitmap, int64_t nwords, u32 *__restrict__ bc) {
+    __shared__ u32 wt[FD_TB / 64];
+    const int64_t i = (int64_t)blockIdx.x * FD_TB + threadIdx.x;
+    u32 c = i < nwords ? (u32)__popc(bitmap[i]) : 0u;
+#pragma unroll
+    for (int dd = 32; dd >= 1; dd >>= 1) c += __shfl_xor(c, dd, 64);
+    if ((threadIdx.x & 63) == 0) wt[threadIdx.x >> 6] = c;
+    __syncthreads();
+    if (threadIdx.x == 0) { u32 t = 0; for (int k = 0; k < FD_TB / 64; k++) t += wt[k]; bc[blockIdx.x] = t; }
+}
+template <class V>
+__global__ __launch_bounds__(FD_TB) void k_fin_gather(const u32 *__restrict__ bitmap, int64_t nwords, const u32 *__restrict__ boff, const u64 *__restrict__ keys, const V *__restrict__ vals,
+                                                      u32 *__restrict__ gslot, u64 *__restrict__ gkey, V *__restrict__ gval, u32 m) {
+    __shared__ u32 wt[FD_TB / 64];
+    const int64_t i = (int64_t)blockIdx.x * FD_TB + threadIdx.x;
+    u32 bits = i < nwords ? bitmap[i] : 0u;
+    const u32 c = (u32)__popc(bits), inc = rv_wave_incl_sum_u32(c);
+    if ((threadIdx.x & 63) == 63) wt[threadIdx.x >> 6] = inc;
+    __syncthreads();
+    u32 pos = boff[blockIdx.x] + inc - c;
+    for (u32 k = 0; k < (threadIdx.x >> 6); k++) pos += wt[k];
+    while (bits) {
+        const u32 b = (u32)__builtin_ctz(bits); bits &= bits - 1u;
+        const u32 slot = (u32)(i * 32 + b);
+        if (pos < m) { gslot[pos] = slot; gkey[pos] = keys[slot]; gval[pos] = vals[slot]; }
+        pos++;
+    }
+}
+__global__ __launch_bounds__(FD_TB) void k_fin_heads(const u64 *__restrict__ gkey, u32 m, int gshift, u64 gmask, u32 *__restrict__ head) {
+    const u32 i = blockIdx.x * FD_TB + threadIdx.x;
+    if (i >= m) return;
+    head[i] = (i == 0 || ((gkey[i] >> gshift) & gmask) != ((gkey[i - 1] >> gshift) & gmask)) ? 1u : 0u;
+}
+__global__ __launch_bounds__(FD_TB) void k_fin_sortkeys(const u64 *__restrict__ gkey, const u32 *__restrict__ head, const u32 *__restrict__ before, u32 m, int lo,
+                                                        u64 *__restrict__ sk, u32 *__restrict__ sv) {
+    const u32 i = blockIdx.x * FD_TB + threadIdx.x;
+    if (i >= m) return;
+    sk[i] = ((u64)(before[i] + head[i]) << 8) | ((gkey[i] >> lo) & 255ull);
+    sv[i] = i;
+}
+template <class V>
+__global__ __launch_bounds__(FD_TB) void k_fin_put(const u32 *__restrict__ order, const u32 *__restrict__ gslot, const u64 *__restrict__ gkey, const V *__restrict__ gval, u32 m,
+                                                   u64 *__restrict__ keys, V *__restrict__ vals) {
+    const u32 i = blockIdx.x * FD_TB + threadIdx.x;
+    if (i >= m) return;
+    const u32 j = order[i], slot = gslot[i];
+    keys[slot] = gkey[j]; vals[slot] = gval[j];
 }
 
 }
@@ -310,35 +473,104 @@
 static bool rs_digit_bytes(const Workspace &ws, int64_t n, int bit_lo, int bit_hi) {
     return ws.opt.rs_bits != 10 && !ws.opt.rs_no_digit_bytes && n > 1 && n >= ((int64_t)1 << 20) && n < ((int64_t)1 << 32) && bit_hi - bit_lo > 8;
 }
-uint8_t *rv_radix_first_digits(Workspace &ws, int64_t n, int bit_lo, int bit_hi) {
-    if (!rs_digit_bytes(ws, n, bit_lo, bit_hi) || ws.rs_digits.reserve((size_t)n + 64)) return nullptr;
+static bool rs_finish_low(const Workspace &ws, int64_t n, int bit_lo, int bit_hi, size_t vbytes) {
+    const int64_t S = ws.opt.rs_fin_stride, W = ws.opt.rs_fin_window;
+    return ws.opt.rs_bits != 10 && !ws.opt.rs_no_finish_low && vbytes == 4 && bit_hi - bit_lo > 16 && n > 1 && n >= ws.opt.rs_fin_min_n && n < ((int64_t)1 << 32)
+           && S >= 64 && W >= 1 && W <= S && S + W <= RS_TILE && ws.opt.rs_fin_group >= 1;
+}
+uint8_t *rv_radix_first_digits(Workspace &ws, int64_t n, int bit_lo, int bit_hi, bool finish_low, int vbytes, int *digit_shift) {
+    const int lo = finish_low && rs_finish_low(ws, n, bit_lo, bit_hi, (size_t)vbytes) ? bit_lo + 8 : bit_lo;
+    if (digit_shift) *digit_shift = lo;
+    if (!rs_digit_bytes(ws, n, lo, bit_hi) || ws.rs_digits.reserve((size_t)n + 64)) return nullptr;
     return ws.rs_digits.as<uint8_t>();
 }
 
 template <class V>
-int rv_radix_sort_pairs(Workspace &ws, u64 *k0, V *v0, u64 *k1, V *v1, int64_t n, int bit_lo, int bit_hi, int *result_in_1, bool first_digits) {
+static int rs_finish_deferred(Workspace &ws, u64 *keys, V *vals, int64_t n, u32 m, const u32 *bitmap, int lo, int gshift, u64 gmask) {
+    const int64_t nwords = ceil_div(n, 32), nbk = ceil_div(nwords, FD_TB);
+    const u32 gm = (u32)ceil_div((int64_t)m, FD_TB);
+    DBuf &bcnt = ws.rs_fin[2], &blist = ws.rs_fin[3];
+    RV_TRY(bcnt.reserve((size_t)(nbk + 1) * 4));
+    const size_t m8 = ((size_t)m * 8 + 63) & ~(size_t)63, m4 = ((size_t)m * 4 + 63) & ~(size_t)63, mv = ((size_t)m * sizeof(V) + 63) & ~(size_t)63;
+    RV_TRY(blist.reserve(3 * m8 + 5 * m4 + mv));
+    uint8_t *p = blist.as<uint8_t>();
+    u64 *gkey = (u64 *)p, *sk0 = (u64 *)(p + m8), *sk1 = (u64 *)(p + 2 * m8); p += 3 * m8;
+    u32 *gslot = (u32 *)p, *head = (u32 *)(p + m4), *before = (u32 *)(p + 2 * m4), *sv0 = (u32 *)(p + 3 * m4), *sv1 = (u32 *)(p + 4 * m4); p += 5 * m4;
+    V *gval = (V *)p;
+    u32 *bc = bcnt.as<u32>();
+    hipLaunchKernelGGL(k_fin_count, dim3((unsigned)nbk), dim3(FD_TB), 0, ws.stream, bitmap, nwords, bc);
+    RV_LAUNCH_CHECK();
+    RV_TRY(rv_exclusive_sum_u32(ws, bc, bc, nbk));
+    hipLaunchKernelGGL((k_fin_gather<V>), dim3((unsigned)nbk), dim3(FD_TB), 0, ws.stream, bitmap, nwords, (const u32 *)bc, (const u64 *)keys, (const V *)vals, gslot, gkey, gval, m);
+    RV_LAUNCH_CHECK();
+    hipLaunchKernelGGL(k_fin_heads, dim3(gm), dim3(FD_TB), 0, ws.stream, (const u64 *)gkey, m, gshift, gmask, head);
+    RV_LAUNCH_CHECK();
+    RV_TRY(rv_exclusive_sum_u32(ws, head, before, (int64_t)m));
+    hipLaunchKernelGGL(k_fin_sortkeys, dim3(gm), dim3(FD_TB), 0, ws.stream, (const u64 *)gkey, (const u32 *)head, (const u32 *)before, m, lo, sk0, sv0);
+    RV_LAUNCH_CHECK();
+    int gbits = 1;
+    while (gbits < 32 && ((u64)m >> gbits)) gbits++;
+    int in1 = 0;
+    RV_TRY(rv_radix_sort_pairs<u32>(ws, sk0, sv0, sk1, sv1, (int64_t)m, 0, 8 + gbits, &in1));
+    hipLaunchKernelGGL((k_fin_put<V>), dim3(gm), dim3(FD_TB), 0, ws.stream, (const u32 *)(in1 ? sv1 : sv0), (const u32 *)gslot, (const u64 *)gkey, (const V *)gval, m, keys, vals);
+    RV_LAUNCH_CHECK();
+    return 0;
+}
+
+template <class V>
+int rv_radix_sort_pairs(Workspace &ws, u64 *k0, V *v0, u64 *k1, V *v1, int64_t n, int bit_lo, int bit_hi, int *result_in_1, bool first_digits, bool finish_low) {
     *result_in_1 = 0;
+    ws.rs_info[0] = ws.rs_info[1] = ws.rs_info[2] = ws.rs_info[3] = 0;
     if (n <= 1 || bit_hi <= bit_lo) return 0;
     if (n >= ((int64_t)1 << 32)) { rv_set_error("radix sort: n >= 2^32 not supported"); return -1; }
     const int width = ws.opt.rs_bits == 10 ? 10 : 8;
     const bool xcd = ws.opt.rs_xcd != 0, c16 = ws.opt.rs_cnt16 != 0;
     const u32 nb = (u32)ceil_div(n, RS_TILE);
-    RV_TRY(ws.rs_hist.reserve(((size_t)1 << width) * nb * sizeof(u32)));
+    const bool fin = finish_low && rs_finish_low(ws, n, bit_lo, bit_hi, sizeof(V));
+    const int pass_lo = fin ? bit_lo + 8 : bit_lo;
+    const u32 fS = (u32)ws.opt.rs_fin_stride, fW = (u32)ws.opt.rs_fin_window;
+    const u32 nt = fin ? (u32)ceil_div(n, (int64_t)fS) : 0u;
+    RV_TRY(ws.rs_hist.reserve(((size_t)1 << width) * (nb > nt ? nb : nt) * sizeof(u32)));
     u32 *bh = ws.rs_hist.as<u32>();
-    const bool bytes = rs_digit_bytes(ws, n, bit_lo, bit_hi);
+    const bool bytes = rs_digit_bytes(ws, n, pass_lo, bit_hi);
     if (first_digits && (!bytes || ws.rs_digits.cap < (size_t)n + 64)) { rv_set_error("radix sort: first digits announced but the byte path is off"); return -1; }
     if (bytes) RV_TRY(ws.rs_digits.reserve((size_t)n + 64));
     uint8_t *dig = bytes ? ws.rs_digits.as<uint8_t>() : nullptr;
+    RsFinArgs fa; memset(&fa, 0, sizeof fa);
+    if (fin) {
+        const size_t snap_bytes = (((size_t)nt + 1) * 4 + 63) & ~(size_t)63;
+        RV_TRY(ws.rs_fin[0].reserve(64 + snap_bytes + (size_t)nt + 1));
+        RV_TRY(ws.rs_fin[1].reserve((size_t)ceil_div(n, 32) * 4));
+        uint8_t *p = ws.rs_fin[0].as<uint8_t>();
+        fa.counters = (u32 *)p; fa.snap = (const u32 *)(p + 64); fa.unsn = p + 64 + snap_bytes;
+        fa.bitmap = ws.rs_fin[1].as<u32>();
+        fa.lo = bit_lo; fa.gshift = bit_lo + 8; fa.G = (u32)std::min<int64_t>(ws.opt.rs_fin_group, RS_TILE);
+        fa.gmask = (bit_hi - fa.gshift >= 64) ? ~0ull : ((1ull << (bit_hi - fa.gshift)) - 1ull);
+        RV_HIP(hipMemsetAsync(fa.counters, 0, 64, ws.stream));
+        RV_HIP(hipMemsetAsync(fa.bitmap, 0, (size_t)ceil_div(n, 32) * 4, ws.stream));
+    }
     bool have_digits = first_digits;
     u64 *ki = k0, *ko = k1;
     V *vi = v0, *vo = v1;
     int flip = 0;
-    for (int shift = bit_lo; shift < bit_hi; shift += width) {
+    for (int shift = pass_lo; shift < bit_hi; shift += width) {
         const int wbits = bit_hi - shift < width ? bit_hi - shift : width;
         const u32 dmask = (1u << wbits) - 1u;
+        const int nshift = shift + width;
+        const bool more = nshift < bit_hi;
+        const bool finpass = fin && !more;
+        const u32 ntiles = finpass ? nt : nb;
         int pid = ws.prof_begin(8 , (have_digits ? 1.0 : 8.0) * (double)n);
-        const u32 hgrid = xcd ? RS_XCDS * ((nb + RS_XCDS - 1) / RS_XCDS) : nb;
-        if (have_digits) {
+        const u32 hgrid = xcd ? RS_XCDS * ((ntiles + RS_XCDS - 1) / RS_XCDS) : ntiles;
+        if (finpass) {
+            fa.rmask = (1ull << (shift - fa.gshift)) - 1ull;
+            hipLaunchKernelGGL(k_rs_snap, dim3((nt + 1 + 3) / 4), dim3(256), 0, ws.stream, (const u64 *)ki, n, nt, fS, fW, fa.gshift, fa.rmask,
+                               const_cast<u32 *>(fa.snap), const_cast<uint8_t *>(fa.unsn), fa.counters);
+            RV_LAUNCH_CHECK();
+            const uint8_t *hd = have_digits ? dig : nullptr;
+            if (xcd) hipLaunchKernelGGL((k_rs_hist_snap<true>), dim3(hgrid), dim3(RS_THREADS), 0, ws.stream, (const u64 *)ki, hd, fa.snap, shift, dmask, bh, nt);
+            else hipLaunchKernelGGL((k_rs_hist_snap<false>), dim3(hgrid), dim3(RS_THREADS), 0, ws.stream, (const u64 *)ki, hd, fa.snap, shift, dmask, bh, nt);
+        } else if (have_digits) {
             if (xcd) hipLaunchKernelGGL((k_rs_hist_bytes<true>), dim3(hgrid), dim3(RS_THREADS), 0, ws.stream, (const uint8_t *)dig, n, bh, nb);
             else hipLaunchKernelGGL((k_rs_hist_bytes<false>), dim3(hgrid), dim3(RS_THREADS), 0, ws.stream, (const uint8_t *)dig, n, bh, nb);
         } else if (width == 10) { if (xcd) hipLaunchKernelGGL((k_rs_hist<10, true>), dim3(hgrid), dim3(RS_THREADS), 0, ws.stream, (const u64 *)ki, n, shift, dmask, bh, nb);
@@ -347,15 +579,16 @@
                            else hipLaunchKernelGGL((k_rs_hist<8, false>), dim3(hgrid), dim3(RS_THREADS), 0, ws.stream, (const u64 *)ki, n, shift, dmask, bh, nb); }
         RV_LAUNCH_CHECK();
         ws.prof_end(pid);
-        RV_TRY(rv_exclusive_sum_u32(ws, bh, bh, ((int64_t)1 << width) * nb));
-        const int nshift = shift + width;
-        const bool more = nshift < bit_hi;
+        RV_TRY(rv_exclusive_sum_u32(ws, bh, bh, ((int64_t)1 << width) * ntiles));
         const u32 nmask = more ? ((1u << (bit_hi - nshift < width ? bit_hi - nshift : width)) - 1u) : 0u;
         uint8_t *dn = (bytes && more) ? dig : nullptr;
         pid = ws.prof_begin(7 , (2.0 * (8.0 + sizeof(V)) + (dn ? 1.0 : 0.0)) * (double)n);
 #define RS_GO(B_, X_, C_) rs_scatter_launch<V, B_, X_, C_>(ws.stream, nb, (const u64 *)ki, (const V *)vi, ko, vo, n, shift, dmask, (const u32 *)bh, dn, nshift, nmask)
-        if (width == 10) { if (xcd) { if (c16) RS_GO(10, true, uint16_t); else RS_GO(10, true, u32); } else { if (c16) RS_GO(10, false, uint16_t); else RS_GO(10, false, u32); } }
+#define RS_FIN(X_, C_) rs_scatter_fin_launch<V, X_, C_>(ws.stream, nt, (const u64 *)ki, (const V *)vi, ko, vo, n, shift, dmask, (const u32 *)bh, fa)
+        if (finpass)     { if (xcd) { if (c16) RS_FIN(true, uint16_t); else RS_FIN(true, u32); } else { if (c16) RS_FIN(false, uint16_t); else RS_FIN(false, u32); } }
+        else if (width == 10) { if (xcd) { if (c16) RS_GO(10, true, uint16_t); else RS_GO(10, true, u32); } else { if (c16) RS_GO(10, false, uint16_t); else RS_GO(10, false, u32); } }
         else             { if (xcd) { if (c16) RS_GO(8, true, uint16_t); else RS_GO(8, true, u32); } else { if (c16) RS_GO(8, false, uint16_t); else RS_GO(8, false, u32); } }
+#undef RS_FIN
 #undef RS_GO
         RV_LAUNCH_CHECK();
         ws.prof_end(pid);
@@ -363,6 +596,24 @@
         u64 *tk = ki; ki = ko; ko = tk;
         V *tv = vi; vi = vo; vo = tv;
         flip ^= 1;
+        ws.rs_info[0]++;
+    }
+    if (fin) {
+        u32 cnt[2] = {0, 0};
+        RV_TRY(rv_read_back(ws, cnt, fa.counters, 8));
+        int64_t info[4] = {ws.rs_info[0], (int64_t)cnt[1], (int64_t)cnt[0], 0};
+        if (cnt[0]) {
+            const int64_t share = ws.opt.rs_fin_share;
+            if (share > 0 && (int64_t)cnt[0] * share > n) {
+                int in1 = 0;
+                RV_TRY(rv_radix_sort_pairs<V>(ws, ki, vi, ko, vo, n, bit_lo, bit_hi, &in1));
+                flip ^= in1;
+                info[0] += ws.rs_info[0]; info[3] = 1;
+            } else {
+                RV_TRY(rs_finish_deferred<V>(ws, ki, vi, n, cnt[0], fa.bitmap, fa.lo, fa.gshift, fa.gmask));
+            }
+        }
+        for (int k = 0; k < 4; k++) ws.rs_info[k] = info[k];
     }
     *result_in_1 = flip;
     return 0;
@@ -406,5 +657,5 @@
     return 0;
 }
 
-template int rv_radix_sort_pairs<u32>(Workspace &, u64 *, u32 *, u64 *, u32 *, int64_t, int, int, int *, bool);
-template int rv_radix_sort_pairs<u64>(Workspace &, u64 *, u64 *, u64 *, u64 *, int64_t, int, int, int *, bool);
+template int rv_radix_sort_pairs<u32>(Workspace &, u64 *, u32 *, u64 *, u32 *, int64_t, int, int, int *, bool, bool);
+template int rv_radix_sort_pairs<u64>(Workspace &, u64 *, u64 *, u64 *, u64 *, int64_t, int, int, int *, bool, bool);
```

New measurement: 23220. -7.8%, worse.
